# shepherdvovkes/sparse-matrix-multiplication-benchmark

Hardware: AMD Instinct MI355X
Metric: TCSC SpMM: effective G-add-ops/s + achieved HBM GB/s vs roofline, 1/2/4/8 GPU (higher is better)
Workload: dtype f32; 1 GPU; cfg4: M=4096 K=16384 N=16384, 98% ternary sparsity, fp32, tcsc_gemm_prelu; M=4096, K=16384, N=16384, variant=prelu_basic, columns_per_gpu=16384, nnz_per_gpu=5369271, parallelism=column-shard x1 (strong), no collective, rows_per_gpu=4096

## Files before the change

include/tcsc_gpu.h:

```cpp
#ifndef TCSC_AMD_TCSC_GPU_H
#define TCSC_AMD_TCSC_GPU_H

#include <stddef.h>
#include "sparse/tcsc.h"

#ifdef __cplusplus
extern "C" {
#endif

enum tcsc_variant {
    TCSC_VARIANT_BASIC = 0,
    TCSC_VARIANT_OPTIMIZED = 1,
    TCSC_VARIANT_PRELU_BASIC = 2,
    TCSC_VARIANT_PRELU_SEPARATE = 3,
    TCSC_VARIANT_PRELU_ONTHEGO = 4,
    TCSC_VARIANT_SPARSE_GEMM = 5
};

enum tcsc_status {
    TCSC_OK = 0,
    TCSC_E_ARG = 1,
    TCSC_E_HIP = 2,
    TCSC_E_NOMEM = 3,
    TCSC_E_NODEV = 4
};

enum tcsc_order {
    TCSC_ORDER_FAST = 0,
    TCSC_ORDER_REFERENCE = 1
};

typedef struct tcsc_gpu_plan tcsc_gpu_plan;

typedef struct {
    int device;
    int rows;
    int cols;
    int col_begin;
    long long nnz;
    long long n_pos, n_neg;
    int chunk_k;
    int n_chunks;
    size_t device_bytes;
    int order;
    int mfma_min_M;
} tcsc_gpu_plan_info;

int tcsc_gpu_device_count(void);

void tcsc_gpu_set_order(int order);
int tcsc_gpu_get_order(void);

int tcsc_gpu_plan_create(const tcsc_t *W, int col_begin, int col_end,
                         int device, void *stream, tcsc_gpu_plan **out);

int tcsc_gpu_plan_create_device(int rows, int cols,
                                const int *d_col_start_pos,
                                const int *d_col_start_neg,
                                const int *d_row_index_pos,
                                const int *d_row_index_neg,
                                int col_begin, int col_end, int device,
                                void *stream, tcsc_gpu_plan **out);

int tcsc_gpu_plan_get_info(const tcsc_gpu_plan *plan, tcsc_gpu_plan_info *info);

enum tcsc_path {
    TCSC_PATH_GATHER = 0,
    TCSC_PATH_FUSED = 1,
    TCSC_PATH_MFMA = 2,
    TCSC_PATH_SMALL = 3,
    TCSC_PATH_DECODE = 4
};
int tcsc_gpu_launch_info(const tcsc_gpu_plan *plan, int M, int *path, int *slices);

int tcsc_gpu_launch_combine(const tcsc_gpu_plan *plan, int M, int *in_launch);

int tcsc_gpu_launch_geometry(const tcsc_gpu_plan *plan, int M, int *cols_per_wave);
int tcsc_gpu_wide_pays(int M, int ncols, int num_cus);
int tcsc_gpu_plan_wide_stats(const tcsc_gpu_plan *plan, long long stats[4], unsigned short *map,
                             size_t map_entries);

int tcsc_gpu_plan_reserve(tcsc_gpu_plan *plan, int max_M);
void tcsc_gpu_plan_destroy(tcsc_gpu_plan *plan);

#define TCSC_PATH_AUTO (-1)
int tcsc_gpu_plan_workspace(const tcsc_gpu_plan *plan, int M, int path, size_t *need, size_t *reserved);

int tcsc_gpu_sgemm(const tcsc_gpu_plan *plan, const float *dX, const float *dB,
                   float *dY, int M, int ldy, int variant, float a,
                   void *stream);

int tcsc_gpu_prepare_x(const tcsc_gpu_plan *plan, const float *dX, int M, void *stream);
int tcsc_gpu_sgemm_prepared(const tcsc_gpu_plan *plan, const float *dB, float *dY, int M, int ldy,
                            int variant, float a, void *stream);

int tcsc_gpu_sgemm_bf16(const tcsc_gpu_plan *plan, const void *dX_bf16, const float *dB,
                        float *dY, int M, int ldy, int variant, float a, void *stream);
int tcsc_gpu_launch_info_bf16(const tcsc_gpu_plan *plan, int M, int *path, int *slices);

int tcsc_gpu_plan_enable_i8(tcsc_gpu_plan *plan, void *stream);
int tcsc_gpu_plan_has_i8(const tcsc_gpu_plan *plan);
int tcsc_gpu_sgemm_i8(const tcsc_gpu_plan *plan, const void *dXq, const float *dScale,
                      const float *dB, float *dY, int M, int ldy, int variant, float a, void *stream);
int tcsc_gpu_launch_info_i8(const tcsc_gpu_plan *plan, int M, int *path, int *slices);
int tcsc_gpu_quantize_rows_i8(const float *dX, int M, int K, void *dXq, float *dScale, void *stream);
int tcsc_gpu_workspace_bound_i8(int M, int K, int N, size_t *i8_bytes, size_t *f32_bytes);

int tcsc_gpu_plan_enable_w2(tcsc_gpu_plan *plan, void *stream);
int tcsc_gpu_plan_has_w2(const tcsc_gpu_plan *plan);
int tcsc_gpu_w2_image_bytes(int K, int N, size_t *bytes);
int tcsc_gpu_decode_pays(int M, int K, int N, long long nnz);

int tcsc_gpu_plan_create_packed(const tcsc_t *W, int col_begin, int col_end,
                                int device, void *stream, tcsc_gpu_plan **out);
int tcsc_gpu_plan_create_packed_device(int rows, int cols,
                                       const int *d_col_start_pos,
                                       const int *d_col_start_neg,
                                       const int *d_row_index_pos,
                                       const int *d_row_index_neg,
                                       int col_begin, int col_end, int device,
                                       void *stream, tcsc_gpu_plan **out);
int tcsc_gpu_plan_is_packed(const tcsc_gpu_plan *plan);
int tcsc_gpu_plan_copy_w2(const tcsc_gpu_plan *plan, void *d_dst, size_t bytes, void *stream);

int tcsc_gpu_plan_create_packed_image(const void *image, size_t bytes, int rows, int cols,
                                      int col_begin, int device, void *stream, tcsc_gpu_plan **out);
int tcsc_gpu_plan_create_packed_image_device(const void *d_image, size_t bytes, int rows, int cols,
                                             int col_begin, int device, void *stream, tcsc_gpu_plan **out);
int tcsc_gpu_w2_to_tcsc(const void *d_image, size_t bytes, int rows, int cols,
                        int *d_col_start_pos, int *d_col_start_neg,
                        int *d_row_index_pos, int *d_row_index_neg,
                        int *n_pos, int *n_neg, void *stream);
int tcsc_gpu_w2_from_tcsc_host(const tcsc_t *W, int col_begin, int col_end, void *image, size_t bytes);
tcsc_t *tcsc_gpu_w2_to_tcsc_host(const void *image, size_t bytes, int rows, int cols);

enum tcsc_xtype { TCSC_X_F32 = 0, TCSC_X_BF16 = 1 };
int tcsc_gpu_quantize_rows_i8_bf16(const void *dX_bf16, int M, int K, void *dXq, float *dScale, void *stream);
int tcsc_gpu_sgemm_q8(const tcsc_gpu_plan *plan, const void *dX, int xtype, void *dXq, float *dScale,
                      const float *dB, float *dY, int M, int ldy, int variant, float a, void *stream);
int tcsc_gpu_launch_info_q8(const tcsc_gpu_plan *plan, int M, int xtype, int *path, int *slices, int *fused);
int tcsc_gpu_quant_fuse_pays(int M, int K, int N, int xtype);

enum tcsc_ytype { TCSC_Y_F32 = 0, TCSC_Y_BF16 = 1 };
int tcsc_gpu_sgemm_i8_out(const tcsc_gpu_plan *plan, const void *dXq, const float *dScale,
                          const float *dColScale, const float *dB, void *dY, int ytype,
                          int M, int ldy, int variant, float a, void *stream);
int tcsc_gpu_sgemm_q8_out(const tcsc_gpu_plan *plan, const void *dX, int xtype, void *dXq,
                          float *dScale, const float *dColScale, const float *dB, void *dY,
                          int ytype, int M, int ldy, int variant, float a, void *stream);

int tcsc_gpu_from_dense(const float *d_dense, int rows, int cols,
                        int *d_col_start_pos, int *d_col_start_neg,
                        int *d_row_index_pos, int *d_row_index_neg,
                        int *n_pos, int *n_neg, void *stream);

int tcsc_gpu_dense_sgemm(const float *dX, const float *dW, const float *dB,
                         float *dY, int M, int N, int K, int ldy, int variant,
                         float a, void *stream);


int tcsc_gpu_transpose_index(int rows, int cols,
                             const int *d_col_start_pos, const int *d_col_start_neg,
                             const int *d_row_index_pos, const int *d_row_index_neg,
                             int col_begin, int col_end,
                             int *d_t_col_start_pos, int *d_t_col_start_neg,
                             int *d_t_row_index_pos, int *d_t_row_index_neg,
                             void *stream);

int tcsc_gpu_plan_create_transposed(const tcsc_t *W, int col_begin, int col_end,
                                    int device, void *stream, tcsc_gpu_plan **out);

int tcsc_gpu_plan_create_transposed_device(int rows, int cols,
                                           const int *d_col_start_pos,
                                           const int *d_col_start_neg,
                                           const int *d_row_index_pos,
                                           const int *d_row_index_neg,
                                           int col_begin, int col_end, int device,
                                           void *stream, tcsc_gpu_plan **out);

int tcsc_gpu_sgemm_t(const tcsc_gpu_plan *tplan, const float *dG, float *dDX,
                     int M, int ldx, void *stream);

int tcsc_gpu_prelu_backward(const float *dG, int ldg, const float *dY, int ldy, float a,
                            float *dDZ, int lddz, float *dDB, int M, int N, void *stream);

const char *tcsc_gpu_last_error(void);

void tcsc_gpu_cache_clear(void);

int tcsc_gpu_num_shards(void);
void tcsc_gpu_set_num_shards(int shards);


int tcsc_gpu_build_flags(void);

#ifdef __cplusplus
}
#endif

#endif
```

sparse-matrix-multiplication-benchmark_amd/csrc/tcsc_api.cpp:

```cpp
#include <hip/hip_runtime.h>
#include <rocblas/rocblas.h>

#include <algorithm>
#include <cstdarg>
#include <cstdint>
#include <cstdio>
#include <cstdlib>
#include <cstring>
#include <memory>
#include <mutex>
#include <string>
#include <unordered_map>
#include <vector>

#include "../../include/sparse/tcsc.h"
#include "../../include/tcsc_gpu.h"
#include "tcsc_plan.h"

struct tcsc_gpu_plan {
    int device = 0;
    int rows = 0, cols = 0, col_begin = 0;
    long long n_pos = 0, n_neg = 0;
    int n_chunks = 0, n_groups = 0;
    long long n_entries = 0;
// ... 319 lines not shown
              bool allow_mfma, hipStream_t st) {
    if (p->cols == 0 || p->rows >= (1 << 27) - 4) return TCSC_OK;
    if (!tcsc::small_m_fits(1, p->rows) && !mfma_wanted(p, allow_mfma)) return TCSC_OK;
    const int nc = p->cols, ng = tcsc::csc_groups(nc);
    size_t tb = 0;
    DevBuf tcp, tcn, trp, trn, gq, tmp;
    if (tcsc::plan_scan_tmp_bytes(ng + 1, &tb) != hipSuccess || hipMalloc(&p->ccq, (size_t)(ng + 1) * sizeof(int)) != hipSuccess ||
        tcp.alloc((size_t)(nc + 1) * sizeof(int)) != hipSuccess || tcn.alloc((size_t)(nc + 1) * sizeof(int)) != hipSuccess ||
        gq.alloc((size_t)(ng + 1) * sizeof(int)) != hipSuccess || tmp.alloc(tb) != hipSuccess ||
        trp.alloc((size_t)(p->n_pos > 0 ? p->n_pos : 1) * sizeof(int)) != hipSuccess ||
        trn.alloc((size_t)(p->n_neg > 0 ? p->n_neg : 1) * sizeof(int)) != hipSuccess) {
        (void)hipGetLastError();
        free_csc(p);
        return TCSC_OK;
    }
    HIP_TRY(tcsc::csc_prepare(csp, csn, rip, rin, col_begin, nc, p->n_pos, p->n_neg, tcp.as<int>(), tcn.as<int>(),
                              trp.as<int>(), trn.as<int>(), gq.as<int>(), tmp.p, tb, p->ccq, st));
    int quads = 0;
    HIP_TRY(hipMemcpyAsync(&quads, p->ccq + ng, sizeof(int), hipMemcpyDeviceToHost, st));
    HIP_TRY(hipStreamSynchronize(st));
    const size_t ent = tcsc::csc_quad_entries(quads);
    const double nnz = (double)(p->n_pos + p->n_neg);
    if ((double)ent > kCscMaxPad * nnz + (double)tcsc::csc_quad_entries(16LL * ng)) {
        free_csc(p);
        return TCSC_OK;
    }
    if (hipMalloc(&p->crq, ent * sizeof(int)) != hipSuccess) {
        (void)hipGetLastError();
        free_csc(p);
        return TCSC_OK;
    }
    p->csc_bytes = (size_t)(ng + 1) * sizeof(int) + ent * sizeof(int);
    HIP_TRY(tcsc::csc_fill(tcp.as<int>(), tcn.as<int>(), trp.as<int>(), trn.as<int>(), p->ccq, nc, p->rows, p->crq,
                           ent, st));
    HIP_TRY(hipStreamSynchronize(st));
    return TCSC_OK;
}

constexpr int kSmallMaxM = 4;
int small_max_m() {
    const char* e = std::getenv("TCSC_SMALL_M");
    if (!e) return kSmallMaxM;
    return std::max(0, std::min(kSmallMaxM, std::atoi(e)));
}

bool has_small(const tcsc_gpu_plan* p, int M) {
    return p->crq && p->rows > 0 && M >= 1 && M <= small_max_m() && tcsc::small_m_fits(M, p->rows);
}
bool use_small(const tcsc_gpu_plan* p, int M, int dt = kF32) { return has_small(p, M) && !use_mfma(p, M, dt); }

bool decode_pays(int M, int K, int N, long long nnz) {
    if (M < 1 || M > tcsc::kDecodeMaxM) return false;
    return M > kSmallMaxM || !tcsc::small_m_fits(M, K) || 16 * nnz > (long long)K * N;
}
int decode_knob() {
    const char* e = std::getenv("TCSC_DECODE");
    if (!e || !*e) return -1;
    return std::atoi(e) != 0 ? 1 : 0;
}
bool w2gemm_knob() {
    const char* e = std::getenv("TCSC_W2GEMM");
    return e && std::atoi(e) != 0;
}
bool has_decode(const tcsc_gpu_plan* p, int M, int dt) {
    return dt == kI8 && p->w2 && M >= 1 && M <= tcsc::kDecodeMaxM;
}
bool use_decode(const tcsc_gpu_plan* p, int M, int dt) {
    if (!has_decode(p, M, dt)) return false;
    if (p->packed) return true;
    const int knob = decode_knob();
    return knob >= 0 ? knob == 1 : decode_pays(M, p->rows, p->cols, p->n_pos + p->n_neg);
}

int maybe_build_mfma(tcsc_gpu_plan* p, const int* csp, const int* csn, const int* rip, const int* rin, int col_begin,
                     bool allow_mfma, hipStream_t st) {
    const int mode = path_mode();
    if (!mfma_wanted(p, allow_mfma)) return TCSC_OK;
    if (!p->crq) return TCSC_OK;
    const size_t n = (size_t)p->rows * p->cols;
    DevBuf wf, bad;
    if (wf.alloc(n * sizeof(float)) != hipSuccess || bad.alloc(sizeof(int)) != hipSuccess) {
        (void)hipGetLastError();
        return TCSC_OK;
    }
    const int ldw = tcsc::mfma_ldw(p->rows);
    const size_t wtb = (size_t)p->cols * ldw * sizeof(uint16_t);
    if (hipMalloc(&p->wt, wtb) != hipSuccess) {
        (void)hipGetLastError();
        free_mfma(p);
        return TCSC_OK;
    }
    p->mfma_bytes = wtb;
    HIP_TRY(hipMemsetAsync(bad.p, 0, sizeof(int), st));
    HIP_TRY(tcsc::mfma_build_wt(csp, csn, rip, rin, col_begin, p->rows, p->cols, wf.as<float>(), p->wt, ldw,
                                p->n_pos, p->n_neg, bad.as<int>(), st));
    int hbad = 0;
    HIP_TRY(hipMemcpyAsync(&hbad, bad.p, sizeof(int), hipMemcpyDeviceToHost, st));
    HIP_TRY(hipStreamSynchronize(st));
    if (hbad) free_mfma(p);
    p->mfma_min_M = mode == 2 ? 1 : kMfmaMinM;
    return TCSC_OK;
}

int build_plan_ordered(int rows, int col_begin, int ncols, long long n_pos, long long n_neg, const int* csp,
                       const int* csn, const int* rip, const int* rin, int device, hipStream_t st, int order,
                       tcsc_gpu_plan** out, bool allow_mfma = true) {
    int rc = build_plan(rows, col_begin, ncols, n_pos, n_neg, csp, csn, rip, rin, device, st, out);
    if (rc != TCSC_OK) return rc;
    if (order != TCSC_ORDER_REFERENCE) {
        rc = build_csc(*out, csp, csn, rip, rin, col_begin, allow_mfma, st);
        if (rc == TCSC_OK) rc = maybe_build_mfma(*out, csp, csn, rip, rin, col_begin, allow_mfma, st);
        if (rc != TCSC_OK) {
            tcsc_gpu_plan_destroy(*out);
            *out = nullptr;
        }
        return rc;
    }
    tcsc_gpu_plan* p = *out;
    p->order = order;
    DevBuf zeros;
    const size_t zb = (size_t)(col_begin + ncols + 1) * sizeof(int);
    if (zeros.alloc(zb) != hipSuccess || hipMemsetAsync(zeros.p, 0, zb, st) != hipSuccess) {
        tcsc_gpu_plan_destroy(p);
        *out = nullptr;
        set_error("tcsc_gpu_plan_create: cannot allocate the reference-order chains");
        return TCSC_E_HIP;
    }
    rc = build_plan(rows, col_begin, ncols, n_pos, 0, csp, zeros.as<int>(), rip, rip, device, st, &p->chain_pos);
    if (rc == TCSC_OK)
        rc = build_plan(rows, col_begin, ncols, 0, n_neg, zeros.as<int>(), csn, rin, rin, device, st, &p->chain_neg);
    if (rc != TCSC_OK) {
        tcsc_gpu_plan_destroy(p);
        *out = nullptr;
    }
    return rc;
}

int slices_override() {
    const char* s = std::getenv("TCSC_SLICES");
    return s ? std::atoi(s) : 0;
}

int combine_giveup_knob() {
    const char* s = std::getenv("TCSC_COMBINE_GIVEUP");
    return s && std::atoi(s) != 0 ? 1 : 0;
}

size_t path_ws_bytes(const tcsc_gpu_plan* p, int M, int path) {
    if (M <= 0 || p->cols == 0) return 0;
    RoutePins pin;
    pin.path = path;
    return route_call(p, M, p->packed ? kI8 : kF32, kUnbounded, pin).ws_bytes;
}

int launch_path(const tcsc_gpu_plan* p, int M, int dt = kF32) {
    if (use_decode(p, M, dt)) return TCSC_PATH_DECODE;
    return use_mfma(p, M, dt) ? TCSC_PATH_MFMA : use_small(p, M, dt) ? TCSC_PATH_SMALL : TCSC_PATH_GATHER;
}

size_t wanted_workspace(const tcsc_gpu_plan* p, int M, int dt = kF32) {
    if (M <= 0 || p->cols == 0) return 0;
    return route_call(p, M, dt, kUnbounded, RoutePins()).ws_bytes;
}

constexpr long long kNoSplitBase = 40 * 256;
size_t reserve_bytes(const tcsc_gpu_plan* p, int max_M) {
    if (max_M <= 0 || p->cols == 0) return 0;
    if (p->packed) {
        const int top = std::min(max_M, kMaxLaunchRows);
        size_t want = path_ws_bytes(p, top, TCSC_PATH_MFMA);
        for (int M = 64; M < top; M += 64) want = std::max(want, path_ws_bytes(p, M, TCSC_PATH_MFMA));
        return want;
    }
    const long long cb = std::max(1, (p->n_groups + tcsc::kWaves - 1) / tcsc::kWaves);
    const int every = (int)std::min<long long>(max_M, (kNoSplitBase + cb - 1) / cb * tcsc::kTM);
    size_t want = 0;
    auto all_paths = [&](int M) {
        for (int path : {TCSC_PATH_GATHER, TCSC_PATH_MFMA, TCSC_PATH_SMALL})
            want = std::max(want, path_ws_bytes(p, M, path));
    };
    for (int M = 1; M <= every; ++M) all_paths(M);
    if (p->wt)
        for (long long M = ((long long)every / 64 + 1) * 64; M < max_M; M += 64)
            want = std::max(want, path_ws_bytes(p, (int)M, TCSC_PATH_MFMA));
    all_paths(max_M);
    return want;
}

int check_index_host(const int* cs, const int* ri, int c0, int c1, int rows, int n_elem, const char* sign,
                     std::vector<int>& sorted) {
    sorted.clear();
    bool in_order = true;
    for (int j = c0; j < c1; ++j) {
        const int a = cs[j], b = cs[j + 1];
        if (a < 0 || b < a || b > n_elem) {
            set_error("tcsc_gpu_plan_create: col_start_%s[%d..%d] = %d, %d is not a range inside [0, %d]", sign, j,
                      j + 1, a, b, n_elem);
            return TCSC_E_ARG;
        }
        for (int i = a; i < b; ++i) {
            const int k = ri[i];
            if (k < 0 || k >= rows) {
                set_error("tcsc_gpu_plan_create: row_index_%s[%d] = %d outside [0, %d) (column %d)", sign, i, k, rows,
                          j);
                return TCSC_E_ARG;
            }
            if (i > a && k < ri[i - 1]) in_order = false;
        }
    }
    if (in_order) return TCSC_OK;
    const int base = cs[c0];
    sorted.assign(ri + base, ri + cs[c1]);
    for (int j = c0; j < c1; ++j) std::sort(sorted.begin() + (cs[j] - base), sorted.begin() + (cs[j + 1] - base));
    return TCSC_OK;
}

}

namespace tcsc {

uint64_t fmix64(uint64_t h) {
    h ^= h >> 33;
    h *= 0xff51afd7ed558ccdull;
    h ^= h >> 33;
    h *= 0xc4ceb9fe1a85ec53ull;
    return h ^ (h >> 33);
}

constexpr uint32_t kHashA[4] = {0x9e3779b9u, 0x85ebca6bu, 0xc2b2ae35u, 0x27d4eb2fu};
constexpr uint32_t kHashB[4] = {0x165667b1u, 0xd3a2646cu, 0xfd7046c5u, 0xb55a4f09u};

void hash_groups(const uint32_t* u, long long i0, long long i1, uint64_t acc[4]) {
    for (long long i = i0; i < i1; i += 8) {
        const uint32_t pos = (uint32_t)i;
        for (int j = 0; j < 4; ++j)
            acc[j] += (uint64_t)(u[i + 2 * j] + kHashA[j] + pos) * (uint64_t)(u[i + 2 * j + 1] + kHashB[j]);
    }
}

uint64_t hash_finish(const uint32_t* u, long long n, uint64_t h, uint64_t acc[4]) {
    for (long long i = n & ~7LL; i < n; ++i)
        acc[i & 3] += (uint64_t)(u[i] + kHashA[i & 3] + (uint32_t)i) * (uint64_t)(kHashB[i & 3] | 1u);
    for (int j = 0; j < 4; ++j) h = fmix64(h ^ acc[j]) + (uint64_t)j;
    return h;
}

uint64_t hash_ints(const int* p, long long n, uint64_t h) {
    h = fmix64(h ^ (uint64_t)n);
    if (!p || n <= 0) return h;
    const uint32_t* u = reinterpret_cast<const uint32_t*>(p);
    uint64_t acc[4] = {0, 0, 0, 0};
    hash_groups(u, 0, n & ~7LL, acc);
    return hash_finish(u, n, h, acc);
}

uint64_t tcsc_fingerprint(const tcsc_t* W) {
    uint64_t h = fmix64(((uint64_t)(uint32_t)W->rows << 32) | (uint32_t)W->cols);
    h = hash_ints(W->col_start_pos, (long long)W->cols + 1, h);
    h = hash_ints(W->col_start_neg, (long long)W->cols + 1, h);
    h = hash_ints(W->row_index_pos, W->n_elem_pos, h);
    return hash_ints(W->row_index_neg, W->n_elem_neg, h);
}

}

namespace {

constexpr double kWideAlpha = 0.92;
bool wide_pays(int M, int ncols, int num_cus) {
    if (M <= 0 || ncols <= 0 || num_cus <= 0) return false;
    const long long rt = ((long long)M + tcsc::kTM - 1) / tcsc::kTM;
    auto rounds = [&](int w) { return (rt * ((ncols + w - 1) / w) + num_cus - 1) / num_cus; };
    return (double)(rounds(tcsc::kWideWgCols) * tcsc::kWideWgCols) * kWideAlpha <
           (double)(rounds(tcsc::kWgCols) * tcsc::kWgCols);
}

int geo_override() {
    const char* s = std::getenv("TCSC_GEO");
    const int v = s ? std::atoi(s) : 0;
    return v == tcsc::kCW || v == tcsc::kWideCW ? v : 0;
}

bool wide_wanted(const tcsc_gpu_plan* p, int max_M) {
    if (p->order != TCSC_ORDER_FAST || p->tbias || p->rows <= 0 || p->cols <= 0 || max_M <= 0 || !p->ent || !p->sptr)
        return false;
    const int f = geo_override();
    if (f == tcsc::kWideCW) return true;
    if (f == tcsc::kCW) return false;
    const int top = std::min(max_M, kMaxLaunchRows);
    for (long long M = tcsc::kTM; M < top + tcsc::kTM; M += tcsc::kTM)
        if (wide_pays((int)std::min<long long>(M, top), p->cols, p->num_cus)) return true;
    return false;
}

int build_wide(tcsc_gpu_plan* p) {
    if (p->ent_w) return TCSC_OK;
    DeviceGuard dg(p->device);
    hipStream_t st = nullptr;
    const int nch = p->n_chunks, G = p->n_groups, ncols = p->cols, Gw = tcsc::wide_groups_for(ncols);
    const long long nc = (long long)nch * ncols, ng = (long long)nch * Gw;
    if (nch <= 0 || ng + 1 > 0x7fffffffLL) return TCSC_OK;
    const char* bal_s = std::getenv("TCSC_WIDE_BALANCE");
    const int balance = bal_s && std::atoi(bal_s) == 0 ? 0 : 1;
    const size_t nmap = (size_t)tcsc::wide_blocks_for(ncols) * tcsc::kWideWgCols;
    DevBuf cnt, cptr, gcnt, tmp, loads, winv, wstats;
    size_t tb1 = 0, tb2 = 0;
    HIP_TRY(tcsc::plan_scan_tmp_bytes(nc + 1, &tb1));
    HIP_TRY(tcsc::plan_scan_tmp_bytes(ng + 1, &tb2));
    const size_t tb = std::max(tb1, tb2);
    int* sptr_w = nullptr;
    unsigned short* wperm = nullptr;
    if (cnt.alloc((size_t)(nc + 1) * sizeof(int)) != hipSuccess || cptr.alloc((size_t)(nc + 1) * sizeof(int)) != hipSuccess ||
        gcnt.alloc((size_t)(ng + 1) * sizeof(int)) != hipSuccess || tmp.alloc(tb) != hipSuccess ||
        loads.alloc(nmap / tcsc::kWideCW * nch * sizeof(int)) != hipSuccess ||
        winv.alloc((size_t)ncols * sizeof(unsigned short)) != hipSuccess ||
        wstats.alloc(4 * sizeof(unsigned long long)) != hipSuccess ||
        hipMalloc(&sptr_w, (size_t)(ng + 1) * sizeof(int)) != hipSuccess) {
        (void)hipGetLastError();
        return TCSC_OK;
    }
    std::unique_ptr<int, void (*)(int*)> sptr_guard(sptr_w, [](int* q) { (void)hipFree(q); });
    if (hipMalloc(&wperm, nmap * sizeof(unsigned short)) != hipSuccess) {
        (void)hipGetLastError();
        return TCSC_OK;
    }
    std::unique_ptr<unsigned short, void (*)(unsigned short*)> wperm_guard(wperm, [](unsigned short* q) { (void)hipFree(q); });
    HIP_TRY(hipDeviceSynchronize());
    HIP_TRY(tcsc::wide_counts(p->ent, p->sptr, G, nch, ncols, Gw, balance, cnt.as<int>(), cptr.as<int>(), gcnt.as<int>(),
                              sptr_w, loads.as<int>(), wperm, winv.as<unsigned short>(), wstats.as<unsigned long long>(),
                              tmp.p, tb, st));
    int total = 0;
    unsigned long long stats[4] = {0, 0, 0, 0};
    HIP_TRY(hipMemcpyAsync(&total, sptr_w + ng, sizeof(int), hipMemcpyDeviceToHost, st));
    HIP_TRY(hipMemcpyAsync(stats, wstats.p, sizeof stats, hipMemcpyDeviceToHost, st));
    HIP_TRY(hipStreamSynchronize(st));
    int2* ent_w = nullptr;
    if (hipMalloc(&ent_w, (size_t)(total + tcsc::kEntGuard) * sizeof(int2)) != hipSuccess) {
        (void)hipGetLastError();
        return TCSC_OK;
    }
    hipError_t e = tcsc::wide_fill(p->ent, p->sptr, G, nch, ncols, Gw, cptr.as<int>(), winv.as<unsigned short>(), sptr_w,
                                   ent_w, total, st);
    if (e == hipSuccess) e = hipStreamSynchronize(st);
    if (e != hipSuccess) {
        (void)hipFree(ent_w);
        return hip_fail(e, "build_wide");
    }
    p->ent_w = ent_w;
    p->sptr_w = sptr_guard.release();
    p->wperm = wperm_guard.release();
    for (int i = 0; i < 4; ++i) p->wide_stats[i] = (long long)stats[i];
    p->n_entries_w = total;
    p->n_groups_w = Gw;
    p->wide_bytes = (size_t)(ng + 1) * sizeof(int) + (size_t)(total + tcsc::kEntGuard) * sizeof(int2) +
                    nmap * sizeof(unsigned short);
    return TCSC_OK;
}

int launch_geo(const tcsc_gpu_plan* p, int M, int slices, int forced_slices, const char* who) {
    const int f = geo_override();
    if (f == tcsc::kWideCW) {
        if (p->order != TCSC_ORDER_FAST || forced_slices > 1) {
            if (who)
                set_error("%s: TCSC_GEO=22 needs the fast order and an unsplit K (order %s, %d slices forced)", who,
                          p->order == TCSC_ORDER_FAST ? "fast" : "reference", forced_slices);
            return -1;
        }
        if (p->rows <= 0) return tcsc::kCW;
        if (!p->ent_w) {
            if (who)
                set_error("%s: TCSC_GEO=22 but the plan has no wide streams (tcsc_gpu_plan_reserve builds them)", who);
            return -1;
        }
        return tcsc::kWideCW;
    }
    if (f == tcsc::kCW || !p->ent_w || p->order != TCSC_ORDER_FAST) return tcsc::kCW;
    if (slices != 1) return tcsc::kCW;
    return wide_pays(M, p->cols, p->num_cus) ? tcsc::kWideCW : tcsc::kCW;
}

}

Route tcsc::route_call(const tcsc_gpu_plan* p, int M, int dt, size_t ws_avail, const RoutePins& pin, const char* who) {
    const XType& d = kXTypes[dt];
    const int K = p->rows, N = p->cols;
    Route r;
    r.path = pin.path != TCSC_PATH_AUTO ? pin.path : launch_path(p, M, dt);
    r.rows = std::min(M, kMaxLaunchRows);
    if (p->packed) {
        if (pin.path == TCSC_PATH_AUTO) r.path = M <= tcsc::kDecodeMaxM ? TCSC_PATH_DECODE : TCSC_PATH_MFMA;
        if (r.path != TCSC_PATH_MFMA || !has_mfma(p, r.rows, dt)) return r;
        r.slices = d.slices(r.rows, N, K);
        r.ws_bytes = mfma_ws(dt, r.rows, K, N).bytes;
        return r;
    }
    if (r.path == TCSC_PATH_MFMA) {
        if (!has_mfma(p, M, dt)) return r;
        r.slices = d.slices(M, N, K);
        r.ws_bytes = mfma_ws(dt, M, K, N).bytes;
        return r;
    }
    if (r.path == TCSC_PATH_DECODE) return r;
    if (r.path == TCSC_PATH_SMALL) {
        if (has_small(p, M) && dt == kF32) r.ws_bytes = align256((size_t)M * K * sizeof(float));
        return r;
    }
    const size_t xtb = tcsc::xt_bytes(r.rows, K);
    const int force = pin.slices > 0 ? pin.slices : M > kMaxLaunchRows ? 1 : slices_override();
    int chosen = 1;
    if (p->order != TCSC_ORDER_REFERENCE)
        chosen = tcsc::choose_slices(r.rows, N, K, p->n_pos + p->n_neg, p->n_groups, ws_avail > xtb ? ws_avail - xtb : 0,
                                     force);
    r.slices = tcsc::normalized_slices(K, chosen);
    r.ws_bytes = xtb + tcsc::workspace_bytes(r.rows, N, chosen);
    r.geo = launch_geo(p, r.rows, r.slices, force, who);
    if (r.slices > 1) {
        const long long cb = (p->n_groups + tcsc::kWaves - 1) / tcsc::kWaves, rt = (r.rows + tcsc::kTM - 1) / tcsc::kTM;
        const bool words = pin.plan_ws && p->csync != nullptr;
        r.combine = tcsc::combine_mode(r.slices, cb * rt * r.slices, cb * rt, (long long)r.rows * N,
                                       words ? p->num_cus : 0, words, pin.vec && N % 4 == 0);
    }
    return r;
}

namespace {
int sgemm_mfma(const tcsc_gpu_plan* p, const void* dX, int dt, const float* dScale, const float* dB, const YOut& y,
               int M, int ldy, int variant, float a, void* stream, float* ws, size_t ws_bytes, int stage) {
    const XType& d = kXTypes[dt];
    float* dY = static_cast<float*>(y.Y);
    const int K = p->rows, N = p->cols, ldx = d.ldx(K), ldw = d.ldw(K);
    const MfmaWs w = mfma_ws(dt, M, K, N);
    if (!ws || ws_bytes < w.bytes) {
        set_error("%s: workspace of %zu bytes < %zu needed for M=%d", d.sgemm, ws ? ws_bytes : (size_t)0, w.bytes, M);
        return TCSC_E_ARG;
    }
    hipStream_t st = static_cast<hipStream_t>(stream);
    char* base = reinterpret_cast<char*>(ws);
    uint16_t* xp = reinterpret_cast<uint16_t*>(base);
    int* flags = reinterpret_cast<int*>(base + w.flags_off);
    void* slabs = base + w.slabs_off;
    const size_t slab_bytes = ws_bytes - w.slabs_off;
    const bool prelu = is_prelu(variant);
    switch (dt) {
        case kF32:
            if (stage != 2) HIP_TRY(tcsc::mfma_split_x(static_cast<const float*>(dX), M, K, xp, ldx, flags, st));
            if (stage == 1) return TCSC_OK;
            HIP_TRY(tcsc::mfma_gemm3(xp, ldx, p->wt, ldw, K, M, N, dB, dY, ldy, prelu, a, static_cast<float*>(slabs),
                                     slab_bytes, flags, p->ccq, p->crq, st));
            break;
        case kBf16:
            HIP_TRY(tcsc::mfma_pack_x(static_cast<const uint16_t*>(dX), M, K, xp, ldx, flags, st));
            HIP_TRY(tcsc::mfma_gemm1(xp, ldx, p->wt, ldw, K, M, N, dB, dY, ldy, prelu, a, static_cast<float*>(slabs),
                                     slab_bytes, flags, p->ccq, p->crq, st));
            break;
        case kI8:
            HIP_TRY(tcsc::mfma8_pack_x(static_cast<const int8_t*>(dX), M, K, reinterpret_cast<int8_t*>(base), ldx, st));
            if (p->packed || (p->w2 && w2gemm_knob()))
                HIP_TRY(tcsc::mfma8_gemm_w2(reinterpret_cast<const int8_t*>(base), p->w2, ldx, K, M, N, dScale, dB, y,
                                            ldy, prelu, a, static_cast<int*>(slabs), slab_bytes, st));
            else
                HIP_TRY(tcsc::mfma8_gemm(reinterpret_cast<const int8_t*>(base), p->w8, ldx, K, M, N, dScale, dB, y,
                                         ldy, prelu, a, static_cast<int*>(slabs), slab_bytes, st));
            break;
    }
    if (d.flags && d.slices(M, N, K) <= 1) {
        const auto fixup = dt == kF32 ? tcsc::mfma_fixup : tcsc::mfma_fixup1;
        HIP_TRY(fixup(xp, M, K, ldx, p->ccq, p->crq, N, dB, dY, ldy, false, prelu, a, flags, st));
    }
    return TCSC_OK;
}

}

static const char* path_name(int path) {
    switch (path) {
        case TCSC_PATH_GATHER: return "gather";
        case TCSC_PATH_MFMA: return "MFMA";
        case TCSC_PATH_SMALL: return "small-M";
        case TCSC_PATH_DECODE: return "decode";
        default: return "unknown";
    }
}
static bool refuse_out(const char* who, int path, const YOut& y, int M) {
    if (y.plain() || path == TCSC_PATH_DECODE || path == TCSC_PATH_MFMA) return false;
    set_error("%s: %s%s%s needs the decode or the MFMA path, and M=%d routes to the %s path (%d), which writes an fp32 Y "
              "without column scales", who, y.ytype == kYBf16 ? "a bf16 Y" : "", y.ytype == kYBf16 && y.cscale ? " with " : "",
              y.cscale ? "a column scale" : "", M, path_name(path), path);
    return true;
}

int tcsc::sgemm_ws(const tcsc_gpu_plan* p, const void* dX, const float* dB, float* dY, int M, int ldy, int variant,
                   float a, void* stream, float* ws, size_t ws_bytes, int stage, const RoutePins& pin, Route* ran,
                   int dt, const float* dScale, const YOut* out, const char* as) {
    const XType& d = kXTypes[dt];
    const char* who = as ? as : d.sgemm;
    const YOut y = out ? *out : YOut{dY, kYF32, nullptr};
    if (out) dY = y.plain() ? static_cast<float*>(y.Y) : nullptr;
    if (dt != kI8 && !y.plain()) {
        set_error("%s: only the int8 call has a typed Y and column scales", who);
        return TCSC_E_ARG;
    }
    if (dt != kF32 && stage != 0) {
        set_error("%s: no staged form", who);
        return TCSC_E_ARG;
    }
    if (!p || M < 0 || (stage != 1 && (ldy < p->cols || !valid_variant(variant)))) {
        set_error("%s: bad arguments (M=%d ldy=%d variant=%d)", who, M, ldy, variant);
        return TCSC_E_ARG;
    }
    if (p->packed && dt != kI8) {
        set_error("%s: a packed plan holds the 2-bit image only and runs tcsc_gpu_sgemm_i8 alone", who);
        return TCSC_E_ARG;
    }
    if (M == 0 || p->cols == 0) return TCSC_OK;
    if ((stage != 1 && (!y.Y || !dB)) || (stage != 2 && !dX && p->rows > 0)) {
        set_error("%s: NULL device pointer", who);
        return TCSC_E_ARG;
    }
    if (p->packed && M > kMaxLaunchRows) {
        for (int r0 = 0; r0 < M; r0 += kMaxLaunchRows) {
            const YOut piece = y.rows_on((size_t)r0, ldy);
            const int rc = sgemm_ws(p, static_cast<const char*>(dX) + (size_t)r0 * p->rows * d.elem, dB, nullptr,
                                    std::min(kMaxLaunchRows, M - r0), ldy, variant, a, stream, ws, ws_bytes, 0, pin,
                                    nullptr, dt, dScale ? dScale + r0 : nullptr, &piece, as);
            if (rc != TCSC_OK) return rc;
        }
        if (ran) *ran = route_call(p, M, dt, ws ? ws_bytes : 0, pin);
        return TCSC_OK;
    }
    const size_t xtb = tcsc::xt_bytes(std::min(M, kMaxLaunchRows), p->rows);
    tcsc::GemmArgs g;
    g.ncols = p->cols;
    g.B = dB;
    g.Y = dY;
    g.ldy = ldy;
    g.ws = (ws && ws_bytes > xtb) ? reinterpret_cast<float*>(reinterpret_cast<char*>(ws) + xtb) : nullptr;
    g.ws_bytes = g.ws ? ws_bytes - xtb : 0;
    RoutePins pins = pin;
    pins.plan_ws = ws == p->ws;
    pins.vec = tcsc::stores16(g);
    const Route r = route_call(p, M, dt, ws ? ws_bytes : 0, pins, stage != 1 ? who : nullptr);
    if (ran) *ran = r;
    if ((r.path == TCSC_PATH_MFMA && !has_mfma(p, M, dt)) || (r.path == TCSC_PATH_SMALL && !has_small(p, M)) ||
        (r.path == TCSC_PATH_DECODE && !has_decode(p, M, dt)) ||
        (p->packed && r.path != TCSC_PATH_MFMA && r.path != TCSC_PATH_DECODE)) {
        set_error("%s: the plan cannot run M=%d on the pinned path %d", who, M, r.path);
        return TCSC_E_ARG;
    }
    if (refuse_out(who, r.path, y, M)) return TCSC_E_ARG;
    if (r.path == TCSC_PATH_DECODE) {
        HIP_TRY(tcsc::decode_gemm(static_cast<const int8_t*>(dX), p->w2, p->rows, M, p->cols, dScale, dB, y, ldy,
                                  is_prelu(variant), a, p->num_cus, static_cast<hipStream_t>(stream)));
        return TCSC_OK;
    }
    if (r.path == TCSC_PATH_MFMA)
        return sgemm_mfma(p, dX, dt, dScale, dB, y, M, ldy, variant, a, stream, ws, ws_bytes, stage);
    if (r.path == TCSC_PATH_SMALL) {
        hipStream_t st = static_cast<hipStream_t>(stream);
        const size_t xb = (size_t)M * p->rows * sizeof(float);
        if (stage != 0 && (!ws || ws_bytes < xb)) {
            set_error("tcsc_gpu_sgemm: workspace of %zu bytes < %zu needed for M=%d", ws ? ws_bytes : (size_t)0, xb,
                      M);
            return TCSC_E_ARG;
        }
        if (stage == 1) {
            HIP_TRY(hipMemcpyAsync(ws, dX, xb, hipMemcpyDeviceToDevice, st));
            return TCSC_OK;
        }
        HIP_TRY(tcsc::launch_small_m(stage == 2 ? ws : dX, dt, dScale, M, p->rows, p->ccq, p->crq, p->cols, dB, dY, ldy,
                                     false, is_prelu(variant), a, st));
        return TCSC_OK;
    }
    if (M > kMaxLaunchRows) {
        if (stage != 0) {
            set_error("tcsc_gpu_sgemm: M=%d rows staged at once (at most %d; split the rows)", M, kMaxLaunchRows);
            return TCSC_E_ARG;
        }
        RoutePins piece = pin;
        piece.path = TCSC_PATH_GATHER;
        piece.slices = r.slices;
        for (int r0 = 0; r0 < M; r0 += kMaxLaunchRows) {
            const int rows = std::min(kMaxLaunchRows, M - r0);
            const void* xr = static_cast<const char*>(dX) + (size_t)r0 * p->rows * d.elem;
            const int rc = sgemm_ws(p, xr, dB, dY + (size_t)r0 * ldy, rows, ldy, variant, a, stream, ws, ws_bytes, 0,
                                    piece, nullptr, dt, dScale ? dScale + r0 : nullptr, nullptr, as);
            if (rc != TCSC_OK) return rc;
        }
        return TCSC_OK;
    }
    if (p->rows > 0 && (!ws || ws_bytes < xtb)) {
        set_error("%s: workspace of %zu bytes < %zu needed for M=%d", who, ws ? ws_bytes : (size_t)0, xtb, M);
        return TCSC_E_ARG;
    }
    g.X = dX;
    g.xtype = dt;
    g.Xscale = dScale;
    g.XT = p->rows > 0 ? ws : nullptr;
    g.M = M;
    g.K = p->rows;
    g.ent = p->ent;
    g.sptr = p->sptr;
    g.n_entries = p->n_entries;
    if (p->order == TCSC_ORDER_REFERENCE && p->chain_pos && p->chain_neg) {
        g.order = (variant == TCSC_VARIANT_BASIC || variant == TCSC_VARIANT_PRELU_BASIC ||
                   variant == TCSC_VARIANT_SPARSE_GEMM)
                      ? 1
                      : 2;
        g.ent = p->chain_pos->ent;
        g.sptr = p->chain_pos->sptr;
        g.n_entries = p->chain_pos->n_entries;
        g.ent2 = p->chain_neg->ent;
        g.sptr2 = p->chain_neg->sptr;
        g.n_entries2 = p->chain_neg->n_entries;
    }
    g.n_groups = p->n_groups;
    g.a = a;
    g.slices = r.slices;
    g.combine = r.combine;
    g.stage = stage;
    if (stage != 1) {
        if (r.geo < 0) return TCSC_E_ARG;
        if (r.geo == tcsc::kWideCW) {
            g.geo = r.geo;
            g.ent = p->ent_w;
            g.sptr = p->sptr_w;
            g.wperm = p->wperm;
            g.n_entries = p->n_entries_w;
            g.n_groups = p->n_groups_w;
            g.slices = 1;
            g.combine = 0;
        }
    }
    if (pins.plan_ws && p->csync) {
        if (p->csync_dirty) {
            HIP_TRY(hipMemsetAsync(p->csync, 0, tcsc::kCombineBytes, static_cast<hipStream_t>(stream)));
            p->csync_dirty = false;
        }
        g.ccnt = p->csync;
        g.combine_giveup = combine_giveup_knob();
    }
    g.bias_first = (g.order == 1 && variant == TCSC_VARIANT_BASIC);
    g.prelu = is_prelu(variant);
    hipError_t e = tcsc::launch_gemm(g, static_cast<hipStream_t>(stream));
    if (e != hipSuccess) {
        if (g.ccnt) p->csync_dirty = true;
// ... 266 lines not shown
int tcsc_gpu_plan_create_packed(const tcsc_t* W, int col_begin, int col_end, int device, void* stream,
                                tcsc_gpu_plan** out) {
    const char* who = "tcsc_gpu_plan_create_packed";
    if (!W || !out || col_begin < 0 || col_end > W->cols || col_begin > col_end) {
        set_error("%s: bad arguments", who);
        return TCSC_E_ARG;
    }
    *out = nullptr;
    int rc = packed_args_ok(who, W->rows);
    if (rc != TCSC_OK) return rc;
    std::vector<int> unused;
    rc = check_index_host(W->col_start_pos, W->row_index_pos, col_begin, col_end, W->rows, W->n_elem_pos, "pos", unused);
    if (rc == TCSC_OK)
        rc = check_index_host(W->col_start_neg, W->row_index_neg, col_begin, col_end, W->rows, W->n_elem_neg, "neg",
                              unused);
    if (rc != TCSC_OK) return rc;
    DeviceGuard dg(device);
    if (!dg.ok()) {
        set_error("%s: cannot select device %d", who, device);
        return TCSC_E_NODEV;
    }
    hipStream_t st = static_cast<hipStream_t>(stream);
    const int nc = col_end - col_begin;
    const int p0 = W->col_start_pos[col_begin], p1 = W->col_start_pos[col_end];
    const int q0 = W->col_start_neg[col_begin], q1 = W->col_start_neg[col_end];
    std::vector<int> csp(nc + 1), csn(nc + 1);
    for (int j = 0; j <= nc; ++j) {
        csp[j] = W->col_start_pos[col_begin + j] - p0;
        csn[j] = W->col_start_neg[col_begin + j] - q0;
    }
    DevBuf dcsp, dcsn, drip, drin;
    HIP_TRY(dcsp.alloc((nc + 1) * sizeof(int)));
    HIP_TRY(dcsn.alloc((nc + 1) * sizeof(int)));
    HIP_TRY(drip.alloc((size_t)(p1 - p0) * sizeof(int)));
    HIP_TRY(drin.alloc((size_t)(q1 - q0) * sizeof(int)));
    HIP_TRY(hipMemcpyAsync(dcsp.p, csp.data(), (nc + 1) * sizeof(int), hipMemcpyHostToDevice, st));
    HIP_TRY(hipMemcpyAsync(dcsn.p, csn.data(), (nc + 1) * sizeof(int), hipMemcpyHostToDevice, st));
    if (p1 > p0)
        HIP_TRY(hipMemcpyAsync(drip.p, W->row_index_pos + p0, (size_t)(p1 - p0) * sizeof(int), hipMemcpyHostToDevice, st));
    if (q1 > q0)
        HIP_TRY(hipMemcpyAsync(drin.p, W->row_index_neg + q0, (size_t)(q1 - q0) * sizeof(int), hipMemcpyHostToDevice, st));
    rc = build_packed(who, W->rows, 0, nc, p1 - p0, q1 - q0, dcsp.as<int>(), dcsn.as<int>(), drip.as<int>(),
                      drin.as<int>(), device, st, out);
    if (rc == TCSC_OK) (*out)->col_begin = col_begin;
    return rc;
}

int tcsc_gpu_plan_create_packed_device(int rows, int cols, const int* d_csp, const int* d_csn, const int* d_rip,
                                       const int* d_rin, int col_begin, int col_end, int device, void* stream,
                                       tcsc_gpu_plan** out) {
    const char* who = "tcsc_gpu_plan_create_packed_device";
    if (!out || !d_csp || !d_csn || col_begin < 0 || col_end > cols || col_begin > col_end) {
        set_error("%s: bad arguments", who);
        return TCSC_E_ARG;
    }
    *out = nullptr;
    const int rc = packed_args_ok(who, rows);
    if (rc != TCSC_OK) return rc;
    DeviceGuard dg(device);
    if (!dg.ok()) {
        set_error("%s: cannot select device %d", who, device);
        return TCSC_E_NODEV;
    }
    hipStream_t st = static_cast<hipStream_t>(stream);
    int ends[4];
    HIP_TRY(hipMemcpyAsync(&ends[0], d_csp + col_begin, sizeof(int), hipMemcpyDeviceToHost, st));
    HIP_TRY(hipMemcpyAsync(&ends[1], d_csp + col_end, sizeof(int), hipMemcpyDeviceToHost, st));
    HIP_TRY(hipMemcpyAsync(&ends[2], d_csn + col_begin, sizeof(int), hipMemcpyDeviceToHost, st));
    HIP_TRY(hipMemcpyAsync(&ends[3], d_csn + col_end, sizeof(int), hipMemcpyDeviceToHost, st));
    HIP_TRY(hipStreamSynchronize(st));
    const int nc = col_end - col_begin;
    DevBuf flag;
    HIP_TRY(flag.alloc(sizeof(int)));
    HIP_TRY(hipMemsetAsync(flag.p, 0, sizeof(int), st));
    HIP_TRY(tcsc::check_index_device(d_csp, d_rip, col_begin, nc, rows, ends[1], flag.as<int>(), st));
    HIP_TRY(tcsc::check_index_device(d_csn, d_rin, col_begin, nc, rows, ends[3], flag.as<int>(), st));
    int hflag = 0;
    HIP_TRY(hipMemcpyAsync(&hflag, flag.p, sizeof(int), hipMemcpyDeviceToHost, st));
    HIP_TRY(hipStreamSynchronize(st));
    if (hflag & 1) {
        set_error("%s: a col_start range or a row index outside [0, %d)", who, rows);
        return TCSC_E_ARG;
    }
    return build_packed(who, rows, col_begin, nc, ends[1] - ends[0], ends[3] - ends[2], d_csp, d_csn, d_rip, d_rin,
                        device, st, out);
}

int tcsc_gpu_plan_is_packed(const tcsc_gpu_plan* p) {
    if (!p) {
        set_error("tcsc_gpu_plan_is_packed: NULL plan");
        return 0;
    }
    return p->packed ? 1 : 0;
}

int tcsc_gpu_plan_copy_w2(const tcsc_gpu_plan* p, void* d_dst, size_t bytes, void* stream) {
    if (!p) {
        set_error("tcsc_gpu_plan_copy_w2: NULL plan");
        return TCSC_E_ARG;
    }
    if (!p->w2 || bytes != p->w2_bytes || !d_dst) {
        set_error("tcsc_gpu_plan_copy_w2: %s", !p->w2 ? "the plan has no 2-bit image"
                                                      : !d_dst ? "NULL destination" : "bytes is not the image's size");
        return TCSC_E_ARG;
    }
    DeviceGuard dg(p->device);
    HIP_TRY(hipMemcpyAsync(d_dst, p->w2, bytes, hipMemcpyDeviceToDevice, static_cast<hipStream_t>(stream)));
    return TCSC_OK;
}

int tcsc_gpu_plan_create_packed_image(const void* image, size_t bytes, int rows, int cols, int col_begin, int device,
                                      void* stream, tcsc_gpu_plan** out) {
    return packed_from_image("tcsc_gpu_plan_create_packed_image", image, hipMemcpyHostToDevice, bytes, rows, cols,
                             col_begin, device, stream, out);
}

int tcsc_gpu_plan_create_packed_image_device(const void* d_image, size_t bytes, int rows, int cols, int col_begin,
                                             int device, void* stream, tcsc_gpu_plan** out) {
    return packed_from_image("tcsc_gpu_plan_create_packed_image_device", d_image, hipMemcpyDeviceToDevice, bytes, rows,
                             cols, col_begin, device, stream, out);
}

int tcsc_gpu_w2_to_tcsc(const void* d_image, size_t bytes, int rows, int cols, int* d_csp, int* d_csn, int* d_rip,
                        int* d_rin, int* n_pos, int* n_neg, void* stream) {
    const char* who = "tcsc_gpu_w2_to_tcsc";
    if (!d_csp || !d_csn || !n_pos || !n_neg) {
        set_error("%s: NULL col_start or count pointer", who);
        return TCSC_E_ARG;
    }
    int rc = image_args_ok(who, d_image, bytes, rows, cols);
    if (rc != TCSC_OK) return rc;
    if (!tcsc::w2_unpack_fits(cols, rows)) {
        set_error("%s: %d columns x %d k blocks do not fit 32-bit counters", who, cols, tcsc::w2_kblocks(rows));
        return TCSC_E_ARG;
    }
    hipStream_t st = static_cast<hipStream_t>(stream);
    const uint32_t* w2 = static_cast<const uint32_t*>(d_image);
    long long np = 0, nn = 0;
    rc = check_image(who, w2, rows, cols, &np, &nn, st);
    if (rc != TCSC_OK) return rc;
    if (np > 0x7fffffffLL || nn > 0x7fffffffLL) {
        set_error("%s: %lld +1 and %lld -1 entries: tcsc_t offsets are int (each sign below 2^31)", who, np, nn);
        return TCSC_E_ARG;
    }
    const size_t n = (size_t)cols * tcsc::w2_kblocks(rows) + 1;
    size_t tb = 0;
    HIP_TRY(tcsc::plan_scan_tmp_bytes((long long)n, &tb));
    const size_t arr = align256(n * sizeof(int));
    DevBuf scratch;
    HIP_TRY(scratch.alloc(align256(tb) + 4 * arr));
    char* base = scratch.as<char>() + align256(tb);
    int *cntp = reinterpret_cast<int*>(base), *cntn = reinterpret_cast<int*>(base + arr);
    int *offp = reinterpret_cast<int*>(base + 2 * arr), *offn = reinterpret_cast<int*>(base + 3 * arr);
    HIP_TRY(hipMemsetAsync(cntp + (n - 1), 0, sizeof(int), st));
    HIP_TRY(hipMemsetAsync(cntn + (n - 1), 0, sizeof(int), st));
    HIP_TRY(tcsc::w2_unpack_counts(w2, cols, rows, cntp, cntn, st));
    HIP_TRY(tcsc::exclusive_scan_i32(cntp, offp, (int)n, scratch.p, tb, st));
    HIP_TRY(tcsc::exclusive_scan_i32(cntn, offn, (int)n, scratch.p, tb, st));
    HIP_TRY(tcsc::w2_unpack_col_start(offp, offn, cols, rows, d_csp, d_csn, st));
    if (d_rip && d_rin) HIP_TRY(tcsc::w2_unpack_fill(w2, cols, rows, offp, offn, d_rip, d_rin, st));
    HIP_TRY(hipStreamSynchronize(st));
    *n_pos = (int)np;
    *n_neg = (int)nn;
    return TCSC_OK;
}

int tcsc_gpu_plan_get_info(const tcsc_gpu_plan* p, tcsc_gpu_plan_info* info) {
    if (!p || !info) {
        set_error("tcsc_gpu_plan_get_info: NULL");
        return TCSC_E_ARG;
    }
    info->device = p->device;
    info->rows = p->rows;
    info->cols = p->cols;
    info->col_begin = p->col_begin;
    info->nnz = p->n_pos + p->n_neg;
    info->n_pos = p->n_pos;
    info->n_neg = p->n_neg;
    info->chunk_k = tcsc::kTK;
    info->n_chunks = p->n_chunks;
    info->device_bytes = p->bytes + p->ws_bytes + p->mfma_bytes + p->i8_bytes + p->w2_bytes + p->csc_bytes + p->tbias_bytes + p->wide_bytes +
                         (p->chain_pos ? p->chain_pos->bytes : 0) + (p->chain_neg ? p->chain_neg->bytes : 0);
    info->order = p->order;
    info->mfma_min_M = (p->wt || p->packed) ? p->mfma_min_M : 0;
    return TCSC_OK;
}

void tcsc_gpu_set_order(int order) {
    std::lock_guard<std::mutex> lk(g_order_mu);
    g_order = order == TCSC_ORDER_REFERENCE ? TCSC_ORDER_REFERENCE : TCSC_ORDER_FAST;
}

int tcsc_gpu_get_order(void) { return current_order(); }

void tcsc_gpu_plan_destroy(tcsc_gpu_plan* p) {
    if (!p) return;
    DeviceGuard dg(p->device);
    if (p->ent) (void)hipFree(p->ent);
    if (p->sptr) (void)hipFree(p->sptr);
    if (p->ws) (void)hipFree(p->ws);
    if (p->csync) (void)hipFree(p->csync);
    if (p->tbias) (void)hipFree(p->tbias);
    if (p->ent_w) (void)hipFree(p->ent_w);
    if (p->sptr_w) (void)hipFree(p->sptr_w);
    if (p->wperm) (void)hipFree(p->wperm);
    free_mfma(p);
    free_csc(p);
    tcsc_gpu_plan_destroy(p->chain_pos);
    tcsc_gpu_plan_destroy(p->chain_neg);
    delete p;
}

int tcsc_gpu_plan_reserve(tcsc_gpu_plan* p, int max_M) {
    if (!p || max_M < 0) {
        set_error("tcsc_gpu_plan_reserve: bad arguments");
        return TCSC_E_ARG;
    }
    const size_t want = reserve_bytes(p, max_M);
    if (!p->csync && p->rows > 0 && p->order == TCSC_ORDER_FAST && !p->packed) {
        DeviceGuard dg(p->device);
        HIP_TRY(hipMalloc(&p->csync, tcsc::kCombineBytes));
        HIP_TRY(hipMemset(p->csync, 0, tcsc::kCombineBytes));
        HIP_TRY(hipDeviceSynchronize());
        if (!p->num_cus) HIP_TRY(hipDeviceGetAttribute(&p->num_cus, hipDeviceAttributeMultiprocessorCount, p->device));
    }
    if (!p->ent_w && wide_wanted(p, max_M)) {
        const int rc = build_wide(p);
        if (rc != TCSC_OK) return rc;
    }
    if (want <= p->ws_bytes) return TCSC_OK;
    DeviceGuard dg(p->device);
    if (p->ws) {
        HIP_TRY(hipDeviceSynchronize());
        (void)hipFree(p->ws);
    }
    p->ws = nullptr;
    p->ws_bytes = 0;
    p->staged_M = -1;
    HIP_TRY(hipMalloc(&p->ws, want));
    p->ws_bytes = want;
    return TCSC_OK;
}

int tcsc_gpu_plan_workspace(const tcsc_gpu_plan* p, int M, int path, size_t* need, size_t* reserved) {
    if (!p || M < 0 || (path != TCSC_PATH_AUTO && path != TCSC_PATH_GATHER && path != TCSC_PATH_MFMA &&
                        path != TCSC_PATH_SMALL && path != TCSC_PATH_DECODE)) {
        set_error("tcsc_gpu_plan_workspace: bad arguments (M=%d path=%d)", M, path);
        return TCSC_E_ARG;
    }
    if (need) *need = path_ws_bytes(p, M, path);
    if (reserved) *reserved = p->ws_bytes;
    return TCSC_OK;
}

static Route plan_route(const tcsc_gpu_plan* p, int M, int dt, const char* who = nullptr) {
    return route_call(p, M, dt, p->ws_bytes, RoutePins(), who);
}

static int launch_info_impl(const char* who, const tcsc_gpu_plan* p, int M, int* path, int* slices, int dt) {
    if (!p || M < 0 || !path || !slices) {
        set_error("%s: bad arguments", who);
        return TCSC_E_ARG;
    }
    if (dt != kI8 && refuse_packed(p, who)) return TCSC_E_ARG;
    const Route r = plan_route(p, M, dt);
    *path = r.path;
    *slices = r.slices;
    return TCSC_OK;
}

int tcsc_gpu_launch_info(const tcsc_gpu_plan* p, int M, int* path, int* slices) {
    return launch_info_impl("tcsc_gpu_launch_info", p, M, path, slices, kF32);
}

int tcsc_gpu_launch_info_bf16(const tcsc_gpu_plan* p, int M, int* path, int* slices) {
    return launch_info_impl("tcsc_gpu_launch_info_bf16", p, M, path, slices, kBf16);
}

int tcsc_gpu_launch_info_i8(const tcsc_gpu_plan* p, int M, int* path, int* slices) {
    return launch_info_impl("tcsc_gpu_launch_info_i8", p, M, path, slices, kI8);
}

int tcsc_gpu_wide_pays(int M, int ncols, int num_cus) { return wide_pays(M, ncols, num_cus) ? 1 : 0; }

int tcsc_gpu_plan_wide_stats(const tcsc_gpu_plan* p, long long stats[4], unsigned short* map, size_t map_entries) {
    if (!p || (!stats && !map)) {
        set_error("tcsc_gpu_plan_wide_stats: bad arguments");
        return TCSC_E_ARG;
    }
    if (!p->ent_w || !p->wperm) {
        set_error("tcsc_gpu_plan_wide_stats: the plan has no wide streams (tcsc_gpu_plan_reserve builds them)");
        return TCSC_E_ARG;
    }
    if (stats)
        for (int i = 0; i < 4; ++i) stats[i] = p->wide_stats[i];
    if (map) {
        const size_t nmap = (size_t)tcsc::wide_blocks_for(p->cols) * tcsc::kWideWgCols;
        if (map_entries != nmap) {
            set_error("tcsc_gpu_plan_wide_stats: the map has %zu entries, not %zu", nmap, map_entries);
            return TCSC_E_ARG;
        }
        DeviceGuard dg(p->device);
        HIP_TRY(hipMemcpy(map, p->wperm, nmap * sizeof(unsigned short), hipMemcpyDeviceToHost));
    }
    return TCSC_OK;
}

int tcsc_gpu_launch_geometry(const tcsc_gpu_plan* p, int M, int* cols_per_wave) {
    if (!p || M < 0 || !cols_per_wave) {
        set_error("tcsc_gpu_launch_geometry: bad arguments");
        return TCSC_E_ARG;
    }
    if (refuse_packed(p, "tcsc_gpu_launch_geometry")) return TCSC_E_ARG;
    *cols_per_wave = 0;
    const Route r = plan_route(p, M, kF32, "tcsc_gpu_launch_geometry");
    if (r.path != TCSC_PATH_GATHER) return TCSC_OK;
    if (r.geo < 0) return TCSC_E_ARG;
    *cols_per_wave = r.geo;
    return TCSC_OK;
}

int tcsc_gpu_launch_combine(const tcsc_gpu_plan* p, int M, int* in_launch) {
    if (!p || M < 0 || !in_launch) {
        set_error("tcsc_gpu_launch_combine: bad arguments");
        return TCSC_E_ARG;
    }
    if (refuse_packed(p, "tcsc_gpu_launch_combine")) return TCSC_E_ARG;
    *in_launch = plan_route(p, M, kF32).combine;
    return TCSC_OK;
}

static int sgemm_entry(const tcsc_gpu_plan* p, const void* dX, int dt, const float* dScale, const float* dB, float* dY,
                       int M, int ldy, int variant, float a, void* stream, const YOut* out = nullptr,
                       const char* as = nullptr) {
    if (dt != kI8 && refuse_packed(p, kXTypes[dt].sgemm)) return TCSC_E_ARG;
    if (out && !out->plain() && p && M > 0 && p->cols > 0 &&
        refuse_out(as ? as : kXTypes[dt].sgemm, route_call(p, M, dt, p->ws_bytes, RoutePins()).path, *out, M))
        return TCSC_E_ARG;
    if (p && M > 0 && p->cols > 0 && p->ws_bytes < wanted_workspace(p, M, dt)) {
        const int rc = tcsc_gpu_plan_reserve(const_cast<tcsc_gpu_plan*>(p), M);
        if (rc != TCSC_OK) return rc;
    }
    if (p) const_cast<tcsc_gpu_plan*>(p)->staged_M = -1;
    return sgemm_ws(p, dX, dB, dY, M, ldy, variant, a, stream, p ? p->ws : nullptr, p ? p->ws_bytes : 0, 0, RoutePins(),
                    nullptr, dt, dScale, out, as);
}

int tcsc_gpu_sgemm(const tcsc_gpu_plan* p, const float* dX, const float* dB, float* dY, int M, int ldy,
                   int variant, float a, void* stream) {
    return sgemm_entry(p, dX, kF32, nullptr, dB, dY, M, ldy, variant, a, stream);
}

int tcsc_gpu_sgemm_bf16(const tcsc_gpu_plan* p, const void* dX_bf16, const float* dB, float* dY, int M, int ldy,
                        int variant, float a, void* stream) {
    return sgemm_entry(p, dX_bf16, kBf16, nullptr, dB, dY, M, ldy, variant, a, stream);
}

int tcsc_gpu_plan_enable_i8(tcsc_gpu_plan* p, void* stream) {
    if (!p) {
        set_error("tcsc_gpu_plan_enable_i8: NULL plan");
        return TCSC_E_ARG;
    }
    if (p->w8 || !p->wt || p->order == TCSC_ORDER_REFERENCE || p->rows <= 0 || p->cols <= 0) return TCSC_OK;
    DeviceGuard dg(p->device);
    hipStream_t st = static_cast<hipStream_t>(stream);
    const int ld8 = tcsc::mfma8_ldw(p->rows);
    const size_t bytes = (size_t)p->cols * ld8;
    DevBuf bad;
    if (bad.alloc(sizeof(int)) != hipSuccess || hipMalloc(&p->w8, bytes) != hipSuccess) {
        (void)hipGetLastError();
        p->w8 = nullptr;
        set_error("tcsc_gpu_plan_enable_i8: cannot allocate the int8 image (%zu bytes)", bytes);
        return TCSC_E_NOMEM;
    }
    p->i8_bytes = bytes;
    int hbad = 0, rc = TCSC_OK;
    hipError_t e = hipMemsetAsync(bad.p, 0, sizeof(int), st);
    if (e == hipSuccess)
        e = tcsc::mfma8_build_w8(p->wt, p->cols, p->rows, tcsc::mfma_ldw(p->rows), p->w8, ld8, bad.as<int>(), st);
    if (e == hipSuccess) e = hipMemcpyAsync(&hbad, bad.p, sizeof(int), hipMemcpyDeviceToHost, st);
    if (e == hipSuccess) e = hipStreamSynchronize(st);
    if (e != hipSuccess) rc = hip_fail(e, "tcsc_gpu_plan_enable_i8");
    if (rc != TCSC_OK || hbad) free_i8(p);
    return rc;
}

int tcsc_gpu_plan_has_i8(const tcsc_gpu_plan* p) {
    if (!p) {
        set_error("tcsc_gpu_plan_has_i8: NULL plan");
        return 0;
    }
    return p->w8 ? 1 : 0;
}

int tcsc_gpu_plan_enable_w2(tcsc_gpu_plan* p, void* stream) {
    if (!p) {
        set_error("tcsc_gpu_plan_enable_w2: NULL plan");
        return TCSC_E_ARG;
    }
    if (p->w2 || !p->w8 || p->rows <= 0 || p->rows >= tcsc::kDecodeMaxK || p->cols <= 0) return TCSC_OK;
    DeviceGuard dg(p->device);
    hipStream_t st = static_cast<hipStream_t>(stream);
    const size_t bytes = tcsc::w2_image_bytes(p->rows, p->cols);
    DevBuf bad;
    if (bad.alloc(sizeof(int)) != hipSuccess || hipMalloc(&p->w2, bytes) != hipSuccess) {
        (void)hipGetLastError();
        p->w2 = nullptr;
        set_error("tcsc_gpu_plan_enable_w2: cannot allocate the 2-bit image (%zu bytes)", bytes);
        return TCSC_E_NOMEM;
    }
    p->w2_bytes = bytes;
    int hbad = 0, rc = TCSC_OK;
    hipError_t e = hipMemsetAsync(bad.p, 0, sizeof(int), st);
    if (e == hipSuccess)
        e = tcsc::decode_build_w2(p->w8, p->cols, p->rows, tcsc::mfma8_ldw(p->rows), p->w2, bad.as<int>(), st);
    if (e == hipSuccess) e = hipMemcpyAsync(&hbad, bad.p, sizeof(int), hipMemcpyDeviceToHost, st);
    if (e == hipSuccess) e = hipStreamSynchronize(st);
    if (e == hipSuccess && !p->num_cus)
        e = hipDeviceGetAttribute(&p->num_cus, hipDeviceAttributeMultiprocessorCount, p->device);
    if (e != hipSuccess) rc = hip_fail(e, "tcsc_gpu_plan_enable_w2");
    if (rc != TCSC_OK || hbad) free_w2(p);
    return rc;
}

int tcsc_gpu_plan_has_w2(const tcsc_gpu_plan* p) {
    if (!p) {
        set_error("tcsc_gpu_plan_has_w2: NULL plan");
        return 0;
    }
    return p->w2 ? 1 : 0;
}

int tcsc_gpu_w2_image_bytes(int K, int N, size_t* bytes) {
    if (K < 0 || N < 0 || !bytes) {
        set_error("tcsc_gpu_w2_image_bytes: bad arguments (K=%d N=%d)", K, N);
        return TCSC_E_ARG;
    }
    *bytes = tcsc::w2_image_bytes(K, N);
    return TCSC_OK;
}

int tcsc_gpu_decode_pays(int M, int K, int N, long long nnz) { return decode_pays(M, K, N, nnz) ? 1 : 0; }

int tcsc_gpu_sgemm_i8(const tcsc_gpu_plan* p, const void* dXq, const float* dScale, const float* dB, float* dY, int M,
                      int ldy, int variant, float a, void* stream) {
    const YOut y{dY, kYF32, nullptr};
    return sgemm_entry(p, dXq, kI8, dScale, dB, nullptr, M, ldy, variant, a, stream, &y);
}

static int out_args(const char* who, const tcsc_gpu_plan* p, const float* dB, const void* dY, int ytype) {
    if (ytype != TCSC_Y_F32 && ytype != TCSC_Y_BF16) {
        set_error("%s: ytype=%d is neither TCSC_Y_F32 (0) nor TCSC_Y_BF16 (1)", who, ytype);
        return TCSC_E_ARG;
    }
    if (!p) {
        set_error("%s: NULL plan", who);
        return TCSC_E_ARG;
    }
    if (!dY || !dB) {
        set_error("%s: NULL %s", who, !dY ? "dY" : "dB");
        return TCSC_E_ARG;
    }
    return TCSC_OK;
}

int tcsc_gpu_sgemm_i8_out(const tcsc_gpu_plan* p, const void* dXq, const float* dScale, const float* dColScale,
                          const float* dB, void* dY, int ytype, int M, int ldy, int variant, float a, void* stream) {
    const char* who = "tcsc_gpu_sgemm_i8_out";
    const int rc = out_args(who, p, dB, dY, ytype);
    if (rc != TCSC_OK) return rc;
    const YOut y{dY, ytype == TCSC_Y_BF16 ? kYBf16 : kYF32, dColScale};
    return sgemm_entry(p, dXq, kI8, dScale, dB, nullptr, M, ldy, variant, a, stream, &y, who);
}

int tcsc_gpu_quantize_rows_i8(const float* dX, int M, int K, void* dXq, float* dScale, void* stream) {
    if (M < 0 || K < 0) {
        set_error("tcsc_gpu_quantize_rows_i8: bad arguments (M=%d K=%d)", M, K);
        return TCSC_E_ARG;
    }
    if (M == 0) return TCSC_OK;
    if (!dScale || (K > 0 && (!dX || !dXq))) {
        set_error("tcsc_gpu_quantize_rows_i8: NULL device pointer");
        return TCSC_E_ARG;
    }
    HIP_TRY(tcsc::quantize_rows_i8(dX, M, K, static_cast<int8_t*>(dXq), dScale, static_cast<hipStream_t>(stream)));
    return TCSC_OK;
}

int tcsc_gpu_quantize_rows_i8_bf16(const void* dX_bf16, int M, int K, void* dXq, float* dScale, void* stream) {
    if (M < 0 || K < 0) {
        set_error("tcsc_gpu_quantize_rows_i8_bf16: bad arguments (M=%d K=%d)", M, K);
        return TCSC_E_ARG;
    }
    if (M == 0) return TCSC_OK;
    if (!dScale || (K > 0 && (!dX_bf16 || !dXq))) {
        set_error("tcsc_gpu_quantize_rows_i8_bf16: NULL device pointer");
        return TCSC_E_ARG;
    }
    HIP_TRY(tcsc::quantize_rows_i8_bf16(static_cast<const uint16_t*>(dX_bf16), M, K, static_cast<int8_t*>(dXq), dScale,
                                        static_cast<hipStream_t>(stream)));
    return TCSC_OK;
}

static constexpr int kQFuseMaxM = 4;
static constexpr long long kQFuseValues = 1LL << 23;
static bool quant_fuse_pays(int M, int K, int N, int xtype) {
    if (M < 1 || M > kQFuseMaxM || K < 1 || N < 1 || (xtype != TCSC_X_F32 && xtype != TCSC_X_BF16)) return false;
    const int T = tcsc::decode_tiles_per_wg(M, N, 0);
    const long long wgs = (tcsc::w2_col_tiles(N) + T - 1) / T;
    return wgs * M * K <= kQFuseValues;
}
static int qfuse_knob() {
    const char* e = std::getenv("TCSC_QFUSE");
    if (!e || !*e) return -1;
    return std::atoi(e) != 0 ? 1 : 0;
}
static Route route_q8(const tcsc_gpu_plan* p, int M, int xtype, bool* fused) {
    const Route r = route_call(p, M, kI8, p->ws_bytes, RoutePins());
    *fused = false;
    if (r.path == TCSC_PATH_DECODE && has_decode(p, M, kI8)) {
        const int knob = qfuse_knob();
        *fused = knob >= 0 ? knob == 1 : quant_fuse_pays(M, p->rows, p->cols, xtype);
    }
    return r;
}

int tcsc_gpu_quant_fuse_pays(int M, int K, int N, int xtype) { return quant_fuse_pays(M, K, N, xtype) ? 1 : 0; }

int tcsc_gpu_launch_info_q8(const tcsc_gpu_plan* p, int M, int xtype, int* path, int* slices, int* fused) {
    if (!p || M < 0 || !path || !slices || !fused || (xtype != TCSC_X_F32 && xtype != TCSC_X_BF16)) {
        set_error("tcsc_gpu_launch_info_q8: bad arguments (M=%d xtype=%d)", M, xtype);
        return TCSC_E_ARG;
    }
    bool f = false;
    const Route r = route_q8(p, M, xtype, &f);
    *path = r.path;
    *slices = r.slices;
    *fused = f ? 1 : 0;
    return TCSC_OK;
}

static int sgemm_q8_impl(const char* who, const char* inner, const tcsc_gpu_plan* p, const void* dX, int xtype, void* dXq,
                         float* dScale, const float* dB, const YOut& y, int M, int ldy, int variant, float a,
                         void* stream) {
    void* dY = y.Y;
    if (!p || M < 0 || ldy < p->cols || !valid_variant(variant) || (xtype != TCSC_X_F32 && xtype != TCSC_X_BF16)) {
        set_error("%s: bad arguments (M=%d ldy=%d variant=%d xtype=%d)", who, M, ldy, variant, xtype);
        return TCSC_E_ARG;
    }
    if (M == 0) return TCSC_OK;
    if (!dScale || !dB || !dY || (!dX && p->rows > 0)) {
        set_error("%s: NULL device pointer", who);
        return TCSC_E_ARG;
    }
    bool fused = false;
    if (p->cols > 0 && refuse_out(who, route_q8(p, M, xtype, &fused).path, y, M)) return TCSC_E_ARG;
    if (!fused) {
        if (!dXq && p->rows > 0) {
            set_error("%s: NULL dXq on a route that is not fused (M=%d)", who, M);
            return TCSC_E_ARG;
        }
        const int rc = xtype == TCSC_X_F32
                           ? tcsc_gpu_quantize_rows_i8(static_cast<const float*>(dX), M, p->rows, dXq, dScale, stream)
                           : tcsc_gpu_quantize_rows_i8_bf16(dX, M, p->rows, dXq, dScale, stream);
        if (rc != TCSC_OK) return rc;
        return sgemm_entry(p, dXq, kI8, dScale, dB, nullptr, M, ldy, variant, a, stream, &y, inner);
    }
    const_cast<tcsc_gpu_plan*>(p)->staged_M = -1;
    HIP_TRY(tcsc::decode_gemm_q(dX, xtype == TCSC_X_BF16, p->w2, p->rows, M, p->cols, dScale, dB, y, ldy,
                                is_prelu(variant), a, p->num_cus, static_cast<hipStream_t>(stream)));
    return TCSC_OK;
}

int tcsc_gpu_sgemm_q8(const tcsc_gpu_plan* p, const void* dX, int xtype, void* dXq, float* dScale, const float* dB,
                      float* dY, int M, int ldy, int variant, float a, void* stream) {
    return sgemm_q8_impl("tcsc_gpu_sgemm_q8", nullptr, p, dX, xtype, dXq, dScale, dB, YOut{dY, kYF32, nullptr}, M, ldy,
                         variant, a, stream);
}

int tcsc_gpu_sgemm_q8_out(const tcsc_gpu_plan* p, const void* dX, int xtype, void* dXq, float* dScale,
                          const float* dColScale, const float* dB, void* dY, int ytype, int M, int ldy, int variant,
                          float a, void* stream) {
    const char* who = "tcsc_gpu_sgemm_q8_out";
    const int rc = out_args(who, p, dB, dY, ytype);
    if (rc != TCSC_OK) return rc;
    return sgemm_q8_impl(who, who, p, dX, xtype, dXq, dScale, dB, YOut{dY, ytype == TCSC_Y_BF16 ? kYBf16 : kYF32, dColScale},
                         M, ldy, variant, a, stream);
}

int tcsc_gpu_workspace_bound_i8(int M, int K, int N, size_t* i8_bytes, size_t* f32_bytes) {
    if (M < 0 || K < 1 || N < 0) {
        set_error("tcsc_gpu_workspace_bound_i8: bad arguments (M=%d K=%d N=%d)", M, K, N);
        return TCSC_E_ARG;
    }
    if (i8_bytes) *i8_bytes = mfma_ws(kI8, M, K, N).bytes;
    if (f32_bytes) *f32_bytes = mfma_ws(kF32, M, K, N).bytes;
    return TCSC_OK;
}

static int ensure_workspace(const tcsc_gpu_plan* p, int M) {
    if (p && M > 0 && p->cols > 0 && p->ws_bytes < wanted_workspace(p, M))
        return tcsc_gpu_plan_reserve(const_cast<tcsc_gpu_plan*>(p), M);
    return TCSC_OK;
}

int tcsc_gpu_prepare_x(const tcsc_gpu_plan* p, const float* dX, int M, void* stream) {
// ... 363 lines not shown
```

sparse-matrix-multiplication-benchmark_amd/csrc/tcsc_internal.h:

```cpp
#pragma once
#include <hip/hip_runtime.h>
#include <stddef.h>
#include <stdint.h>

namespace tcsc {

constexpr int kTM = 256;
#ifndef TCSC_TK
#define TCSC_TK 48
#endif
#ifndef TCSC_NBUF
#define TCSC_NBUF 3
#endif
constexpr int kTK = TCSC_TK;
constexpr int kNBuf = TCSC_NBUF;
constexpr int kRowBytes = kTM * 4;
constexpr int kBufRows = kTK + 1;
#ifndef TCSC_WAVES
#define TCSC_WAVES 16
#endif
#ifndef TCSC_CW
#define TCSC_CW 16
#endif
#ifndef TCSC_BATCH
#define TCSC_BATCH 4
#endif
constexpr int kWaves = TCSC_WAVES;
constexpr int kCW = TCSC_CW;
constexpr int kBatch = TCSC_BATCH;
constexpr int kWavesPerSimd = kWaves / 4;
static_assert(kWaves % 4 == 0 && kWaves <= 16, "whole waves per SIMD");

#ifndef TCSC_WIDTHS
#define TCSC_WIDTHS 16, 16, 16, 16
#endif
struct ColLayout {
    int w[kWavesPerSimd];
};
constexpr ColLayout kRankCols{{TCSC_WIDTHS}};
__host__ __device__ constexpr int wave_cols(int w) { return kRankCols.w[w >> 2]; }
__host__ __device__ constexpr int wave_col0(int w) {
    int s = 0;
    for (int r = 0; r < (w >> 2); ++r) s += 4 * kRankCols.w[r];
    return s + (w & 3) * kRankCols.w[w >> 2];
}
constexpr int wg_cols() {
    int s = 0;
    for (int r = 0; r < kWavesPerSimd; ++r) s += 4 * kRankCols.w[r];
    return s;
}
constexpr int kWgCols = wg_cols();
constexpr bool widths_ok() {
    for (int r = 0; r < kWavesPerSimd; ++r)
        if (kRankCols.w[r] <= 0 || kRankCols.w[r] > kCW || kRankCols.w[r] % 4) return false;
    return true;
}
static_assert(widths_ok(), "TCSC_WIDTHS: one width per rank, multiples of 4, at most TCSC_CW");
__host__ __device__ constexpr int group_col0(int g) { return (g / kWaves) * kWgCols + wave_col0(g % kWaves); }
__host__ __device__ constexpr int group_cols(int g) { return wave_cols(g % kWaves); }
__host__ __device__ constexpr int groups_for(int ncols) {
    int g = (ncols / kWgCols) * kWaves;
    while (group_col0(g) < ncols) ++g;
    return g;
}
#ifndef TCSC_PF_S
#define TCSC_PF_S 1
#endif
constexpr bool kPfS = TCSC_PF_S != 0;
constexpr int kPfWindow = 1792;
constexpr int kEntGuard = kPfS ? kPfWindow / 8 + 8 : 64;
static_assert(kEntGuard <= 256, "k_fill_headers writes the guard with one block");
constexpr int kHdr = 2;
constexpr int kRingBytes = kNBuf * kBufRows * kRowBytes;
constexpr int kPfScratch = kPfS ? kWaves * 256 : 0;
constexpr int kEpiMinBytes = kWaves * 64 * (kCW * 4 + 16) + 64 * kRowBytes + 16;
constexpr int kLdsBytes = (kRingBytes + kPfScratch) > kEpiMinBytes ? (kRingBytes + kPfScratch) : kEpiMinBytes;
#ifndef TCSC_DMA_WAVES
#define TCSC_DMA_WAVES (TCSC_WAVES / 4)
#endif
#ifndef TCSC_DMA_EARLY
#define TCSC_DMA_EARLY 1
#endif
constexpr int kDmaWaves = TCSC_DMA_WAVES;
constexpr bool kDmaEarly = TCSC_DMA_EARLY != 0;
constexpr int kDmaPerWave = kTK / kDmaWaves;
static_assert(kDmaWaves <= kWaves && kTK % kDmaWaves == 0, "each DMA wave moves the same number of rows");
static_assert(kLdsBytes <= 160 * 1024, "LDS");
static_assert(kNBuf >= 2 && kNBuf <= 5, "ring of 2 (DMA(c+1) before gather(c)) or n >= 3 (DMA(c+n-1) after it)");

static_assert(4 * kCW <= 255, "slot index must fit the 8-bit gpr_idx field");
static_assert(64 * 16 <= 1024, "lane byte offset (16*lane) must fit the 10 low address bits");

constexpr int kWideCW = 22;
constexpr int kWideBatch = 3;
constexpr int kWideWgCols = kWaves * kWideCW;
__host__ __device__ constexpr int wide_group_col0(int g) { return (g / kWaves) * kWideWgCols + (g % kWaves) * kWideCW; }
__host__ __device__ constexpr int wide_groups_for(int ncols) {
    return (ncols / kWideWgCols) * kWaves + (ncols % kWideWgCols + kWideCW - 1) / kWideCW;
}
__host__ __device__ constexpr int wide_blocks_for(int ncols) { return (ncols + kWideWgCols - 1) / kWideWgCols; }

struct PlanDev {
    int rows = 0;
    int ncols = 0;
    int col_begin = 0;
    long long n_pos = 0, n_neg = 0;
    const int* csp = nullptr;
    const int* csn = nullptr;
    const int* rip = nullptr;
    const int* rin = nullptr;
};

struct PlanOut {
    int n_chunks = 0;
    int n_groups = 0;
    long long n_entries = 0;
    int2* ent = nullptr;
    int* sptr = nullptr;
    int* lbp = nullptr;
    int* lbn = nullptr;
    int* cnt = nullptr;
    int* cptr = nullptr;
    int* gcnt = nullptr;
    void* scan_tmp = nullptr;
    size_t scan_tmp_bytes = 0;
};

constexpr int kCombineTiles = 4096;
constexpr int kCombineWords = 32;
constexpr size_t kCombineBytes = (size_t)kCombineTiles * kCombineWords * 4;

enum { kF32 = 0, kBf16 = 1, kI8 = 2 };

enum { kYF32 = 0, kYBf16 = 1 };
struct YOut {
    void* Y = nullptr;
    int ytype = kYF32;
    const float* cscale = nullptr;
    size_t elem() const { return ytype == kYBf16 ? 2 : 4; }
    bool plain() const { return ytype == kYF32 && !cscale; }
    YOut rows_on(size_t r0, int ldy) const { return YOut{static_cast<char*>(Y) + r0 * ldy * elem(), ytype, cscale}; }
};

struct GemmArgs {
    const void* X = nullptr;
    int xtype = kF32;
    const float* Xscale = nullptr;
    float* XT = nullptr;
    int M = 0, K = 0;
    const int2* ent = nullptr;
    const int* sptr = nullptr;
    long long n_entries = 0;
    int order = 0;
    const int2* ent2 = nullptr;
    const int* sptr2 = nullptr;
    long long n_entries2 = 0;
    int n_groups = 0;
    int geo = kCW;
    const unsigned short* wperm = nullptr;
    int ncols = 0;
    const float* B = nullptr;
    float* Y = nullptr;
    int ldy = 0;
    float a = 0.f;
    bool bias_first = false;
    bool prelu = false;
    float* ws = nullptr;
    size_t ws_bytes = 0;
    int slices = 1;
    int combine = 0;
    int stage = 0;
    unsigned* ccnt = nullptr;
    int combine_giveup = 0;
};
inline bool stores16(const GemmArgs& g) {
    return g.ncols % 4 == 0 && g.ldy % 4 == 0 &&
           ((reinterpret_cast<uintptr_t>(g.Y) | reinterpret_cast<uintptr_t>(g.ws) | reinterpret_cast<uintptr_t>(g.B)) & 15) == 0;
}
constexpr int kMaxLaunchRows = 1 << 22;

hipError_t plan_scan_tmp_bytes(long long n, size_t* bytes);
hipError_t plan_counts(const PlanDev& in, PlanOut& out, hipStream_t st);
hipError_t plan_fill(const PlanDev& in, PlanOut& out, hipStream_t st);
int choose_slices(int M, int ncols, int K, long long nnz, int n_groups, size_t ws_bytes, int force);
int combine_mode(int slices, long long wgs, long long tiles, long long slab_floats, int num_cus, bool have_words,
                 bool vec);
int normalized_slices(int K, int slices);
void pf_stream_params(long long n_entries, int n_groups, int n_chunks, int* dist, int* lines);
size_t workspace_bytes(int M, int ncols, int slices);
size_t xt_bytes(int M, int K);
hipError_t launch_gemm(const GemmArgs& g, hipStream_t st);
hipError_t wide_counts(const int2* ent, const int* sptr, int G, int nch, int ncols, int Gw, int balance, int* cnt,
                       int* cptr, int* gcnt, int* sptr_w, int* loads, unsigned short* wperm, unsigned short* winv,
                       unsigned long long* wstats, void* tmp, size_t tmp_bytes, hipStream_t st);
hipError_t wide_fill(const int2* ent, const int* sptr, int G, int nch, int ncols, int Gw, const int* cptr,
                     const unsigned short* winv, const int* sptr_w, int2* ent_w, long long n_entries, hipStream_t st);
hipError_t launch_stream_wide(const GemmArgs& g, hipStream_t st);
int dense_tile_rows(int rows);
hipError_t dense_to_tcsc_counts(const float* D, int rows, int cols, int* cp, int* cn, int* totp, int* totn,
                                hipStream_t st);
hipError_t dense_to_tcsc_fill(const float* D, int rows, int cols, const int* csp, const int* csn, const int* op,
                              const int* on, int* rip, int* rin, hipStream_t st);
hipError_t launch_bias_act(float* Y, int M, int N, int ldy, const float* B, bool prelu, float a, hipStream_t st);
hipError_t exclusive_scan_i32(const int* in, int* out, int n, void* tmp, size_t tmp_bytes, hipStream_t st);
hipError_t check_index_device(const int* cs, const int* ri, int col_begin, int ncols, int rows, int n_total,
                              int* d_flag, hipStream_t st);
hipError_t rebase_offsets(const int* cs, int col_begin, int ncols, int* out, hipStream_t st);
hipError_t sort_columns_tmp_bytes(int n, int ncols, size_t* bytes);
hipError_t sort_columns(const int* in, int* out, int n, int ncols, const int* off, void* tmp, size_t tmp_bytes,
                        hipStream_t st);
int ldxt_for(int M);
hipError_t launch_transpose(const void* X, int M, int K, float* XT, int ldxt, hipStream_t st, int xtype = kF32,
                            const float* scale = nullptr);

constexpr int kCscGroup = 64;
constexpr int kCscGuardQuads = 48;
__host__ __device__ inline int csc_half(int K) { return (K + 4) & ~3; }
__host__ __device__ inline int csc_neg_base(int K) { return 4 * csc_half(K); }
__host__ __device__ inline int csc_groups(int ncols) { return (ncols + kCscGroup - 1) / kCscGroup; }
inline size_t csc_quad_entries(long long quads) { return (size_t)(quads + kCscGuardQuads) * kCscGroup * 4; }
hipError_t csc_prepare(const int* csp, const int* csn, const int* rip, const int* rin, int col_begin, int ncols,
                       long long n_pos, long long n_neg, int* cp, int* cn, int* crp, int* crn, int* gq, void* scan_tmp,
                       size_t scan_tmp_bytes, int* cq, hipStream_t st);
hipError_t csc_fill(const int* cp, const int* cn, const int* crp, const int* crn, const int* cq, int ncols, int rows,
                    int* crq, size_t crq_entries, hipStream_t st);
__host__ __device__ inline size_t csc_entry(const int* cq, int j, int i) {
    const int g = j / kCscGroup, l = j % kCscGroup;
    return ((size_t)(cq[g] + i / 4) * kCscGroup + l) * 4 + (i & 3);
}

constexpr int kMfmaBlk = 64;
__host__ __device__ inline int mfma_nblk(int K) { return (K + kMfmaBlk - 1) / kMfmaBlk; }
__host__ __device__ inline int mfma_ldk(int K) { return 3 * kMfmaBlk * mfma_nblk(K); }
__host__ __device__ inline int mfma_ldw(int K) { return kMfmaBlk * mfma_nblk(K); }
__host__ __device__ inline int x3_index(int k, int part) {
    return (k / kMfmaBlk) * (3 * kMfmaBlk) + part * kMfmaBlk + k % kMfmaBlk;
}
hipError_t mfma_build_wt(const int* csp, const int* csn, const int* rip, const int* rin, int col_begin, int rows,
                         int ncols, float* wf, uint16_t* wt, int ldw, long long n_pos, long long n_neg, int* bad,
                         hipStream_t st);
constexpr size_t small_m_lds_bytes_max() { return 160 * 1024; }
inline size_t small_m_lds_bytes(int M, int K) { return (size_t)M * 2 * (size_t)csc_half(K) * 4; }
inline bool small_m_fits(int M, int K) { return M >= 1 && M <= 4 && small_m_lds_bytes(M, K) <= small_m_lds_bytes_max(); }
hipError_t launch_small_m(const void* X, int xtype, const float* scale, int M, int K, const int* cq, const int* crq,
                          int ncols, const float* B, float* Y, int ldy, bool bias_first, bool prelu, float a,
                          hipStream_t st);
hipError_t mfma_split_x(const float* X, int M, int K, uint16_t* x3, int ldk, int* flags, hipStream_t st);
bool mfma_big_tiles(int M, int N);
bool mfma_narrow_tiles(int M, int N);
long long mfma_tiles(int M, int N);
int mfma_slices(int M, int N, int K);
size_t mfma_slab_bytes(int M, int N, int K);
hipError_t mfma_gemm3(const uint16_t* x3, int ldk, const uint16_t* wt, int ldw, int K, int M, int N, const float* B,
                      float* Y, int ldy, bool prelu, float a, float* slabs, size_t slab_bytes, const int* flags,
                      const int* cq, const int* crq, hipStream_t st);

hipError_t mfma_pack_x(const uint16_t* X, int M, int K, uint16_t* x1, int ldw, int* flags, hipStream_t st);
hipError_t mfma_gemm1(const uint16_t* x1, int ldk, const uint16_t* wt, int ldw, int K, int M, int N, const float* B,
                      float* Y, int ldy, bool prelu, float a, float* slabs, size_t slab_bytes, const int* flags,
                      const int* cq, const int* crq, hipStream_t st);
hipError_t mfma_fixup1(const uint16_t* x1, int M, int K, int ldk, const int* cq, const int* crq, int ncols,
                       const float* B, float* Y, int ldy, bool bias_first, bool prelu, float a, const int* flags,
                       hipStream_t st);

constexpr int kMfma8Blk = 128;
__host__ __device__ inline int mfma8_nblk(int K) { return (K + kMfma8Blk - 1) / kMfma8Blk; }
__host__ __device__ inline int mfma8_ldw(int K) { return kMfma8Blk * mfma8_nblk(K); }
int mfma8_slices(int M, int N, int K);
size_t mfma8_slab_bytes(int M, int N, int K);
hipError_t mfma8_pack_x(const int8_t* X, int M, int K, int8_t* x8, int ld8, hipStream_t st);
hipError_t mfma8_build_w8(const uint16_t* wt, int ncols, int K, int ldw, int8_t* w8, int ld8, int* bad,
                          hipStream_t st);
hipError_t mfma8_gemm(const int8_t* x8, const int8_t* w8, int ld8, int K, int M, int N, const float* scale,
                      const float* B, const YOut& y, int ldy, bool prelu, float a, int* slabs, size_t slab_bytes,
                      hipStream_t st);
hipError_t quantize_rows_i8(const float* X, int M, int K, int8_t* Xq, float* scale, hipStream_t st);
hipError_t quantize_rows_i8_bf16(const uint16_t* X, int M, int K, int8_t* Xq, float* scale, hipStream_t st);

constexpr int kW2Cols = 16;
constexpr int kW2Blk = 256;
constexpr int kW2TileBytes = 1024;
constexpr int kDecodeMaxM = 16;
constexpr int kDecodeMaxK = 1 << 22;
__host__ __device__ inline int w2_col_tiles(int N) { return (N + kW2Cols - 1) / kW2Cols; }
__host__ __device__ inline int w2_kblocks(int K) { return (K + kW2Blk - 1) / kW2Blk; }
inline size_t w2_image_bytes(int K, int N) { return (size_t)w2_col_tiles(N) * w2_kblocks(K) * kW2TileBytes; }
hipError_t decode_build_w2(const int8_t* w8, int ncols, int K, int ld8, uint32_t* w2, int* bad, hipStream_t st);
hipError_t w2_from_tcsc(const int* csp, const int* csn, const int* rip, const int* rin, int col_begin, int ncols, int K,
                        uint32_t* w2, int* bad, hipStream_t st);
constexpr int kW2BadCode = 1, kW2BadPad = 2;
hipError_t w2_check(const uint32_t* w2, int ncols, int K, unsigned long long* counts, int* bad, hipStream_t st);
bool w2_unpack_fits(int ncols, int K);
hipError_t w2_unpack_counts(const uint32_t* w2, int ncols, int K, int* cntp, int* cntn, hipStream_t st);
hipError_t w2_unpack_col_start(const int* offp, const int* offn, int ncols, int K, int* csp, int* csn, hipStream_t st);
hipError_t w2_unpack_fill(const uint32_t* w2, int ncols, int K, const int* offp, const int* offn, int* rip, int* rin,
                          hipStream_t st);
hipError_t mfma8_gemm_w2(const int8_t* x8, const uint32_t* w2, int ld8, int K, int M, int N, const float* scale,
                         const float* B, const YOut& y, int ldy, bool prelu, float a, int* slabs, size_t slab_bytes,
                         hipStream_t st);
int decode_tiles_per_wg(int M, int N, int num_cus);
hipError_t decode_gemm(const int8_t* X, const uint32_t* w2, int K, int M, int N, const float* scale, const float* B,
                       const YOut& y, int ldy, bool prelu, float a, int num_cus, hipStream_t st);
hipError_t decode_gemm_q(const void* X, bool bf16, const uint32_t* w2, int K, int M, int N, float* scale_out,
                         const float* B, const YOut& y, int ldy, bool prelu, float a, int num_cus, hipStream_t st);

hipError_t mfma_fixup(const uint16_t* x3, int M, int K, int ldk, const int* cq, const int* crq, int ncols,
                      const float* B, float* Y, int ldy, bool bias_first, bool prelu, float a, const int* flags,
                      hipStream_t st);

hipError_t transpose_sign(const int* cs, const int* ri, int col_begin, int ncols, int rows, int e0, int n, int* cnt,
                          int* cursor, int* unsorted, void* tmp, size_t tmp_bytes, int* t_cs, int* t_ri,
                          hipStream_t st);
hipError_t launch_prelu_bwd(const float* G, int ldg, const float* Y, int ldy, float a, float* DZ, int lddz, float* DB,
                            int M, int N, hipStream_t st);

void set_error_msg(const char* msg);
const char* error_msg();
void report_status(int rc);

struct BcsrArgs {
    const float* XT = nullptr;
    int ldxt = 0, M = 0, N = 0, ldy = 0;
    const int* colptr = nullptr;
    const int2* ent = nullptr;
    const float* vals = nullptr;
    int r = 1, c = 1, nbc = 0;
    const float* B = nullptr;
    float* Y = nullptr;
    float a = 0.f;
    bool fma = false;
    bool prelu = false;
};
hipError_t launch_bcsr(const BcsrArgs& g, hipStream_t st);

}
```

sparse-matrix-multiplication-benchmark_amd/csrc/tcsc_wide.hip:

```cpp
#include <hip/hip_runtime.h>
#include <hipcub/hipcub.hpp>
#include <stdint.h>

#include "tcsc_internal.h"

namespace tcsc {

#include "gather_asm_w22.inc"

static_assert(TCSCW_GEN_CW == kWideCW && TCSCW_GEN_BATCH == kWideBatch, "generated loop geometry");
static_assert(TCSCW_GEN_CAP + kHdr <= kEntGuard, "stream prefetch stays inside the entry guard");
static_assert(TCSCW_GEN_HDR == 2 * kHdr, "generated loop and plan agree on the chunk header");
static_assert(TCSCW_GEN_BUDGET == (512 / kWavesPerSimd) / 8 * 8, "generated loop VGPR budget");
static_assert(TCSCW_GEN_TAIL == 1, "the wide streams are unpadded");
static_assert(TCSCW_GEN_TOUCH == 0 && TCSCW_GEN_PF == 0, "no scalar-cache touches in the wide loop");
static_assert(4 * kWideCW <= 255, "slot index must fit the 8-bit gpr_idx field");
static_assert(kWaves == 16 && kTK % 16 == 0 && kNBuf >= 3, "the wide kernel's DMA split and ring");

namespace {

typedef float f32x32_t __attribute__((ext_vector_type(32)));
typedef float f32x16_t __attribute__((ext_vector_type(16)));
typedef float f32x8_t __attribute__((ext_vector_type(8)));
constexpr int kAccWidths[] = {TCSCW_ACC_WIDTHS};
static_assert(sizeof(kAccWidths) == 4 * sizeof(int) && kAccWidths[0] == 32 && kAccWidths[1] == 32 &&
                  kAccWidths[2] == 16 && kAccWidths[3] == 8,
              "AccW mirrors the generated operand tuples");
struct AccW {
    f32x32_t v0, v1;
    f32x16_t v2;
    f32x8_t v3;
};
__device__ __forceinline__ float acc_get(const AccW& a, int i) {
    return i < 32 ? a.v0[i] : i < 64 ? a.v1[i - 32] : i < 80 ? a.v2[i - 64] : a.v3[i - 80];
}
__device__ __forceinline__ void acc_set(AccW& a, int i, float v) {
    if (i < 32) a.v0[i] = v;
    else if (i < 64) a.v1[i - 32] = v;
    else if (i < 80) a.v2[i - 64] = v;
    else a.v3[i - 80] = v;
}
__device__ __forceinline__ void acc_zero(AccW& a) {
#pragma unroll
    for (int i = 0; i < 4 * kWideCW; ++i) acc_set(a, i, 0.f);
}

typedef int i32x16 __attribute__((ext_vector_type(16)));
typedef __attribute__((address_space(4))) const i32x16 const_i32x16;
typedef int sbuf_tail_t __attribute__((ext_vector_type(TCSCW_SBUF_TAIL ? TCSCW_SBUF_TAIL : 4)));
typedef __attribute__((address_space(4))) const sbuf_tail_t const_sbuf_tail;

__device__ __forceinline__ void gather_stream_w(i32x16 (&sb)[TCSCW_SBUF_VECS], sbuf_tail_t& sbt,
                                                unsigned long long& ptr, unsigned lane16, unsigned mask, AccW& acc) {
    (void)sbt;
    unsigned m0sv;
    asm volatile(TCSCW_GATHER_ASM
                 : TCSCW_ACC_OPERANDS(acc), TCSCW_SBUF_OPERANDS(sb, sbt), TCSCW_PTR_OPERAND(ptr), [m0sv] "=&s"(m0sv)
                 : [lane] "v"(lane16), [mask] "v"(mask)
                 : TCSCW_GATHER_CLOBBERS);
}

__device__ __forceinline__ void load_stream_w(i32x16 (&sb)[TCSCW_SBUF_VECS], sbuf_tail_t& sbt, const char* p) {
    const_i32x16* q = reinterpret_cast<const_i32x16*>(reinterpret_cast<uintptr_t>(p));
#pragma unroll
    for (int i = 0; i < TCSCW_SBUF_VECS; ++i) sb[i] = q[i];
#if TCSCW_SBUF_TAIL
    sbt = *reinterpret_cast<const_sbuf_tail*>(reinterpret_cast<uintptr_t>(p + 64 * TCSCW_SBUF_VECS));
#endif
}

struct DmaW {
    const char* next;
    unsigned lds_wave;
    unsigned chunk_bytes;
    unsigned row_bytes;
};
static_assert(kDmaPerWave % 2 == 0, "whole pairs of DMA rows");

__device__ __forceinline__ void dma_next_chunk_w(DmaW& d, int buf, unsigned lane16) {
    const unsigned m0base = d.lds_wave + (unsigned)(buf * (kBufRows * kRowBytes));
    const char* row = d.next;
#pragma unroll
    for (int i0 = 0; i0 < kDmaPerWave; i0 += 2) {
        const char* s0 = row;
        const char* s1 = row + (d.row_bytes - 1 * kRowBytes);
        unsigned sv;
        asm volatile("s_mov_b32 %[sv], m0\n\ts_mov_b32 m0, %1\n\ts_nop 0\n\tglobal_load_lds_dwordx4 %2, %3\n\t"
                     "global_load_lds_dwordx4 %2, %4 offset:1024\n\ts_mov_b32 m0, %[sv]"
                     : [sv] "=&s"(sv)
                     : "s"(m0base + i0 * kRowBytes), "v"(lane16), "s"(s0), "s"(s1)
                     : "memory");
        row += 2u * d.row_bytes;
    }
    d.next += d.chunk_bytes;
}
static_assert(kRowBytes == 1024, "the DMA's instruction offsets are whole 1-KiB rows");

__device__ __forceinline__ void pf_touch_w(unsigned m0, unsigned voff, const char* base) {
    unsigned sv;
    asm volatile("s_mov_b32 %[sv], m0\n\ts_mov_b32 m0, %1\n\ts_nop 0\n\tglobal_load_lds_dword %2, %3\n\t"
                 "s_mov_b32 m0, %[sv]"
                 : [sv] "=&s"(sv)
                 : "s"(m0), "v"(voff), "s"(base)
                 : "memory");
}

__device__ __forceinline__ void xcd_tile_w(int bx, int by, int ncb, int nrt, int& cb, int& rt) {
    const int T = ncb * nrt;
    const int L = bx + ncb * by;
    const int q = T >> 3, r = T & 7, x = L & 7;
    const int Lg = (x < r ? x * (q + 1) : r * (q + 1) + (x - r) * q) + (L >> 3);
    cb = Lg % ncb;
    rt = Lg / ncb;
}

constexpr int kEpiRowsW = 64;
constexpr int kStrideW = kWideWgCols * 4 + 16;
constexpr int kLdsBytesW = kRingBytes + kPfScratch;
static_assert(kEpiRowsW * kStrideW <= kRingBytes, "the epilogue staging fits below the ring's end");
static_assert(kLdsBytesW <= 160 * 1024, "LDS");
static_assert(kWideCW <= 64 && kWideWgCols <= 65535, "one lane per slot reads its 16-bit column position");
static_assert(kWideWgCols % 4 == 0 && kWideWgCols / 4 > 64 && kWideWgCols / 4 <= 128,
              "a tile row is 64 quads plus a second, partial set");

}

struct WideArgs {
    const float* XT;
    const int2* ent;
    const int* sptr;
    const float* Bias;
    float* Y;
    const unsigned short* wperm;
    long long n_entries;
    int ldxt, M, G, ncols, nch, ldy;
    float a;
    int pf_dist, pf_lines;
};

template <bool BIAS_FIRST, bool PRELU>
__global__ void __launch_bounds__(kWaves * 64, kWavesPerSimd)
k_stream_w(const float* __restrict__ XT, const int2* __restrict__ ent, const int* __restrict__ sptr,
           const float* __restrict__ Bias0, float* __restrict__ Y0, const unsigned short* __restrict__ wperm0,
           long long n_entries, int ldxt, int M0, int G, int ncols0, int nch, int ldy0, float a0, int pf_dist,
           int pf_lines) {
    __shared__ __attribute__((aligned(16))) char lds[kLdsBytesW];
    const int lane = threadIdx.x & 63;
    const unsigned lane16 = 16u * lane;
    const int wave = __builtin_amdgcn_readfirstlane(threadIdx.x >> 6);
    int tcb, trt;
    xcd_tile_w(blockIdx.x, blockIdx.y, gridDim.x, gridDim.y, tcb, trt);
    const int g = tcb * kWaves + wave;
    const int m0 = trt * kTM;
    const bool active = g < G;

    AccW acc;
    acc_zero(acc);
    if (BIAS_FIRST && active) {
        const int cb = lane < kWideCW ? tcb * kWideWgCols + wperm0[tcb * kWideWgCols + wave * kWideCW + lane] : ncols0;
        const float bv = cb < ncols0 ? Bias0[cb] : 0.f;
#pragma unroll
        for (int j = 0; j < kWideCW; ++j) {
            const float b = __shfl(bv, j);
#pragma unroll
            for (int r = 0; r < 4; ++r) acc_set(acc, 4 * j + r, b);
        }
    }

    if (threadIdx.x < 64 * kNBuf) {
        const int b = threadIdx.x >> 6;
        reinterpret_cast<float4*>(lds + (b * kBufRows + kTK) * kRowBytes)[lane] = make_float4(-0.f, -0.f, -0.f, -0.f);
    }

    if (nch > 0) {
        DmaW dma;
        dma.row_bytes = (unsigned)ldxt * 4u;
        dma.chunk_bytes = (unsigned)kTK * (unsigned)ldxt * 4u;
        dma.next = reinterpret_cast<const char*>(XT + m0) + (size_t)(wave * kDmaPerWave) * dma.row_bytes;
        dma.lds_wave = (unsigned)reinterpret_cast<uintptr_t>(lds) + (unsigned)(wave * kDmaPerWave * kRowBytes);
        const bool dma_wave = wave < kDmaWaves;
        const unsigned pf_m0 = (unsigned)reinterpret_cast<uintptr_t>(lds) + kRingBytes + 256u * wave;
        const unsigned pf_s_off = (unsigned)pf_dist + 128u * (unsigned)(lane * pf_lines >> 6);
        auto pf_issue = [&](unsigned long long p) {
            if (kPfS) pf_touch_w(pf_m0, pf_s_off, reinterpret_cast<const char*>(p));
        };
        if (dma_wave) dma_next_chunk_w(dma, 0, lane16);
        unsigned long long cur =
            reinterpret_cast<unsigned long long>(ent + (active ? (long long)sptr[(long long)g * nch] : n_entries));
        i32x16 sb[TCSCW_SBUF_VECS];
        sbuf_tail_t sbt;
        load_stream_w(sb, sbt, reinterpret_cast<const char*>(cur));
        pf_issue(cur);
#pragma unroll
        for (int i = 1; i + 1 < kNBuf; ++i) {
            if (dma_wave) dma_next_chunk_w(dma, i % kNBuf, lane16);
            pf_issue(cur);
        }
        asm volatile("s_waitcnt lgkmcnt(0)" ::: "memory");
        const unsigned mask = 0x3ffu;
        int dbuf = kNBuf - 1;
        for (int c = 0; c < nch; ++c) {
            asm volatile("s_waitcnt vmcnt(%0)" ::"n"((kNBuf - 2) * kDmaPerWave + (kPfS ? 2 : 0)) : "memory");
            __builtin_amdgcn_s_barrier();
            if (dma_wave) dma_next_chunk_w(dma, dbuf, lane16);
            gather_stream_w(sb, sbt, cur, lane16, mask, acc);
            load_stream_w(sb, sbt, reinterpret_cast<const char*>(cur));
            pf_issue(cur);
            dbuf = dbuf == kNBuf - 1 ? 0 : dbuf + 1;
        }
        asm volatile("s_waitcnt vmcnt(0) lgkmcnt(0)" ::: "memory");
    }

    __syncthreads();
    typedef __attribute__((address_space(4))) const WideArgs const_args;
    const_args* E = reinterpret_cast<const_args*>(reinterpret_cast<uintptr_t>(__builtin_amdgcn_kernarg_segment_ptr()));
    asm volatile("" : "+s"(E)::"memory");
    const float* __restrict__ Bias = E->Bias;
    float* __restrict__ Y = E->Y;
    const int M = E->M, ncols = E->ncols, ldy = E->ldy;
    const float a = E->a;
    int bx = blockIdx.x, by = blockIdx.y, gx = gridDim.x, gy = gridDim.y;
    asm volatile("" : "+s"(bx), "+s"(by), "+s"(gx), "+s"(gy));
    const int wave_e = __builtin_amdgcn_readfirstlane(threadIdx.x >> 6);
    int tcb_e, trt_e;
    xcd_tile_w(bx, by, gx, gy, tcb_e, trt_e);
    const bool active_e = tcb_e * kWaves + wave_e < E->G;
    const int m0_e = trt_e * kTM;
    static_assert(kEpiRowsW == 64 && kTM == 4 * kEpiRowsW, "a pass parks one of each lane's four rows");
    constexpr int kQuads = kWideWgCols / 4;
    const unsigned short* __restrict__ wperm = E->wperm;
    const int posv = lane < kWideCW ? wperm[tcb_e * kWideWgCols + wave_e * kWideCW + lane] : 0;
    int pos[kWideCW];
#pragma unroll
    for (int j = 0; j < kWideCW; ++j) pos[j] = __builtin_amdgcn_readlane(posv, j);
    const bool vec_ok = (ldy & 3) == 0 && ((reinterpret_cast<uintptr_t>(Y) & 15) == 0);
    float4 bq[2];
#pragma unroll
    for (int s = 0; s < 2; ++s) {
        const int col = tcb_e * kWideWgCols + 4 * (lane + 64 * s);
        const bool in = lane + 64 * s < kQuads;
        bq[s].x = (!BIAS_FIRST && in && col + 0 < ncols) ? Bias[col + 0] : 0.f;
        bq[s].y = (!BIAS_FIRST && in && col + 1 < ncols) ? Bias[col + 1] : 0.f;
        bq[s].z = (!BIAS_FIRST && in && col + 2 < ncols) ? Bias[col + 2] : 0.f;
        bq[s].w = (!BIAS_FIRST && in && col + 3 < ncols) ? Bias[col + 3] : 0.f;
    }
#pragma unroll
    for (int h = 0; h < kTM / kEpiRowsW; ++h) {
        if (active_e) {
#pragma unroll
            for (int j = 0; j < kWideCW; ++j)
                *reinterpret_cast<float*>(lds + lane * kStrideW + pos[j] * 4) = acc_get(acc, 4 * j + h);
        }
        __syncthreads();
#pragma unroll
        for (int i = 0; i < kEpiRowsW / kWaves; ++i) {
            const int R = wave_e + kWaves * i;
            const int row = m0_e + 4 * R + h;
#pragma unroll
            for (int s = 0; s < 2; ++s) {
                const int q = lane + 64 * s;
                const int col = tcb_e * kWideWgCols + 4 * q;
                if (q < kQuads && row < M && col < ncols) {
                    float4 v = *reinterpret_cast<const float4*>(lds + R * kStrideW + q * 16);
                    if (!BIAS_FIRST) {
                        v.x += bq[s].x;
                        v.y += bq[s].y;
                        v.z += bq[s].z;
                        v.w += bq[s].w;
                    }
                    if (PRELU) {
                        v.x = (v.x < 0.0f) ? a * v.x : v.x;
                        v.y = (v.y < 0.0f) ? a * v.y : v.y;
                        v.z = (v.z < 0.0f) ? a * v.z : v.z;
                        v.w = (v.w < 0.0f) ? a * v.w : v.w;
                    }
                    float* dst = Y + (size_t)row * ldy + col;
                    if (vec_ok && col + 3 < ncols) {
                        typedef float nt4 __attribute__((ext_vector_type(4)));
                        nt4 w = {v.x, v.y, v.z, v.w};
                        __builtin_nontemporal_store(w, reinterpret_cast<nt4*>(dst));
                    } else {
                        dst[0] = v.x;
                        if (col + 1 < ncols) dst[1] = v.y;
                        if (col + 2 < ncols) dst[2] = v.z;
                        if (col + 3 < ncols) dst[3] = v.w;
                    }
                }
            }
        }
        if (h + 1 < kTM / kEpiRowsW) __syncthreads();
    }
}


namespace {

__device__ __forceinline__ int stream_range(const int* __restrict__ sptr, long long i, int* first) {
    const int s0 = sptr[i], s1 = sptr[i + 1];
    *first = s0 + kHdr;
    return s1 - s0 - kHdr;
}
__device__ __forceinline__ bool is_pad(int word) { return ((word >> 10) % kBufRows) == kTK; }

__global__ void k_wide_col_counts(const int2* __restrict__ ent, const int* __restrict__ sptr, int G, int nch, int ncols,
                                  int* __restrict__ cnt) {
    const long long total = (long long)G * nch;
    for (long long i = blockIdx.x * (long long)blockDim.x + threadIdx.x; i < total;
         i += (long long)gridDim.x * blockDim.x) {
        const int g = (int)(i / nch), c = (int)(i % nch);
        int first;
        const int n = stream_range(sptr, i, &first);
        const int n0 = group_col0(g);
        int run = 0, slot = -1;
        for (int e = 0; e < n; ++e) {
            const int w = ent[first + e].y;
            if (is_pad(w)) continue;
            const int s = (w & 0x3ff) >> 2;
            if (s != slot) {
                if (run) cnt[(long long)c * ncols + n0 + slot] = run;
                slot = s;
                run = 0;
            }
            ++run;
        }
        if (run) cnt[(long long)c * ncols + n0 + slot] = run;
    }
}

template <typename T>
__device__ __forceinline__ T wave_sum(T v) {
#pragma unroll
    for (int o = 32; o > 0; o >>= 1) v += __shfl_xor(v, o);
    return v;
}

__global__ void __launch_bounds__(kWaves * 64)
k_wide_balance(const int* __restrict__ cnt, int ncols, int nch, int balance, int* L0, unsigned short* __restrict__ wperm,
               unsigned short* __restrict__ winv) {
    __shared__ int tot[kWideWgCols];
    __shared__ unsigned short order[kWideWgCols], cand[kWideWgCols];
    __shared__ int nslot[kWaves];
    __shared__ unsigned long long score[kWaves], red[2][kWaves];
    __shared__ int best_s, keep_s;
    const int tid = threadIdx.x, nt = blockDim.x, lane = tid & 63, wave = tid >> 6;
    const int c0 = blockIdx.x * kWideWgCols;
    unsigned short* perm = wperm + (size_t)blockIdx.x * kWideWgCols;
    if (!balance || c0 + kWideWgCols > ncols) {
        for (int i = tid; i < kWideWgCols; i += nt) {
            perm[i] = (unsigned short)i;
            if (c0 + i < ncols) winv[c0 + i] = (unsigned short)i;
        }
        return;
    }
    const int* blk = cnt + c0;
    int* L = L0 + (size_t)blockIdx.x * kWaves * nch;
    for (int col = tid; col < kWideWgCols; col += nt) {
        int s = 0;
        for (int c = 0; c < nch; ++c) s += blk[(size_t)c * ncols + col];
        tot[col] = s;
    }
    for (int i = tid; i < kWaves * nch; i += nt) L[i] = 0;
    if (tid < kWaves) nslot[tid] = 0;
    __syncthreads();
    for (int i = tid; i < kWideWgCols; i += nt) {
        int r = 0;
        for (int j = 0; j < kWideWgCols; ++j) r += (tot[j] > tot[i] || (tot[j] == tot[i] && j < i)) ? 1 : 0;
        order[r] = (unsigned short)i;
    }
    __syncthreads();
    for (int step = 0; step < kWideWgCols; ++step) {
        const int col = order[step];
        const int* cc = blk + col;
        unsigned long long s = 0;
        if (nslot[wave] < kWideCW)
            for (int c = lane; c < nch; c += 64)
                s += (unsigned long long)L[(size_t)wave * nch + c] * (unsigned long long)cc[(size_t)c * ncols];
        s = wave_sum(s);
        if (lane == 0) score[wave] = s;
        __syncthreads();
        if (tid == 0) {
            int best = -1;
            for (int w = 0; w < kWaves; ++w)
                if (nslot[w] < kWideCW && (best < 0 || score[w] < score[best])) best = w;
            cand[best * kWideCW + nslot[best]++] = (unsigned short)col;
            best_s = best;
        }
        __syncthreads();
        const int bw = best_s;
        for (int c = tid; c < nch; c += nt) L[(size_t)bw * nch + c] += cc[(size_t)c * ncols];
        __syncthreads();
    }
    unsigned long long sg = 0, si = 0;
    for (int c = tid; c < nch; c += nt) {
        int mg = 0, mi = 0;
        for (int w = 0; w < kWaves; ++w) {
            mg = max(mg, L[(size_t)w * nch + c]);
            int s = 0;
            for (int j = 0; j < kWideCW; ++j) s += blk[(size_t)c * ncols + w * kWideCW + j];
            mi = max(mi, s);
        }
        sg += (unsigned long long)mg;
        si += (unsigned long long)mi;
    }
    sg = wave_sum(sg);
    si = wave_sum(si);
    if (lane == 0) {
        red[0][wave] = sg;
        red[1][wave] = si;
    }
    __syncthreads();
    if (tid == 0) {
        unsigned long long g = 0, i = 0;
        for (int w = 0; w < kWaves; ++w) {
            g += red[0][w];
            i += red[1][w];
        }
        keep_s = g < i ? 1 : 0;
    }
    __syncthreads();
    const bool keep = keep_s != 0;
    for (int i = tid; i < kWideWgCols; i += nt) {
        const int v = keep ? cand[i] : i;
        perm[i] = (unsigned short)v;
        winv[c0 + v] = (unsigned short)i;
    }
}

__global__ void k_wide_permute_counts(const int* __restrict__ cnt, const unsigned short* __restrict__ wperm, int ncols,
                                      int nch, int* __restrict__ cntp) {
    const long long total = (long long)nch * ncols;
    for (long long i = blockIdx.x * (long long)blockDim.x + threadIdx.x; i <= total;
         i += (long long)gridDim.x * blockDim.x) {
        if (i == total) {
            cntp[i] = 0;
            continue;
        }
        const int q = (int)(i % ncols), b0 = q / kWideWgCols * kWideWgCols;
        cntp[i] = cnt[i - q + b0 + wperm[q]];
    }
}

__global__ void k_wide_stats(const int* __restrict__ cnt, const unsigned short* __restrict__ wperm, int ncols, int nch,
                             unsigned long long* __restrict__ st) {
    const int c0 = blockIdx.x * kWideWgCols;
    const unsigned short* perm = wperm + (size_t)blockIdx.x * kWideWgCols;
    unsigned long long v[4] = {0, 0, 0, 0};
    for (int c = threadIdx.x; c < nch; c += blockDim.x) {
        const int* row = cnt + (size_t)c * ncols + c0;
        int mi = 0, mp = 0;
        for (int w = 0; w < kWaves; ++w) {
            int si = 0, sp = 0;
            for (int j = 0; j < kWideCW; ++j) {
                const int ci = w * kWideCW + j, cp = perm[ci];
                si += c0 + ci < ncols ? row[ci] : 0;
                sp += c0 + cp < ncols ? row[cp] : 0;
            }
            mi = max(mi, si);
            mp = max(mp, sp);
            v[2] += si > TCSCW_GEN_CAP ? 1 : 0;
            v[3] += sp > TCSCW_GEN_CAP ? 1 : 0;
        }
        v[0] += (unsigned long long)mi;
        v[1] += (unsigned long long)mp;
    }
#pragma unroll
    for (int k = 0; k < 4; ++k) {
        const unsigned long long s = wave_sum(v[k]);
        if ((threadIdx.x & 63) == 0 && s) atomicAdd(st + k, s);
    }
}

__global__ void k_wide_group_counts(const int* __restrict__ cptr, int ncols, int nch, int Gw, int* __restrict__ gcnt) {
    const long long total = (long long)nch * Gw;
    for (long long i = blockIdx.x * (long long)blockDim.x + threadIdx.x; i < total;
         i += (long long)gridDim.x * blockDim.x) {
        const int g = (int)(i / nch), c = (int)(i % nch);
        const int n0 = wide_group_col0(g), n1 = min(n0 + kWideCW, ncols);
        gcnt[i] = kHdr + cptr[(long long)c * ncols + n1] - cptr[(long long)c * ncols + n0];
    }
}

__global__ void k_wide_scatter(const int2* __restrict__ ent, const int* __restrict__ sptr, int G, int nch, int ncols,
                               const int* __restrict__ cptr, const unsigned short* __restrict__ winv,
                               const int* __restrict__ sptr_w, int2* __restrict__ ent_w) {
    const long long total = (long long)G * nch;
    for (long long i = blockIdx.x * (long long)blockDim.x + threadIdx.x; i < total;
         i += (long long)gridDim.x * blockDim.x) {
        const int g = (int)(i / nch), c = (int)(i % nch);
        int first;
        const int n = stream_range(sptr, i, &first);
        const int n0 = group_col0(g);
        int rank = 0, slot = -1, base = 0, jw = 0;
        for (int e = 0; e < n; ++e) {
            const int2 v = ent[first + e];
            if (is_pad(v.y)) continue;
            const int s = (v.y & 0x3ff) >> 2;
            if (s != slot) {
                slot = s;
                rank = 0;
                const int col = n0 + s;
                const int p = col / kWideWgCols * kWideWgCols + winv[col];
                const int gw = (p / kWideWgCols) * kWaves + (p % kWideWgCols) / kWideCW;
                jw = p - wide_group_col0(gw);
                base = sptr_w[(long long)gw * nch + c] + kHdr +
                       (cptr[(long long)c * ncols + p] - cptr[(long long)c * ncols + wide_group_col0(gw)]);
            }
            ent_w[base + rank++] = make_int2(v.x, (v.y & ~0x3ff) | (4 * jw));
        }
    }
}

__global__ void k_wide_headers(const int* __restrict__ sptr_w, int nch, int Gw, int2* __restrict__ ent_w,
                               long long n_entries) {
    const long long total = (long long)nch * Gw;
    for (long long i = blockIdx.x * (long long)blockDim.x + threadIdx.x; i < total;
         i += (long long)gridDim.x * blockDim.x) {
        const int s0 = sptr_w[i], s1 = sptr_w[i + 1];
        const int n = s1 - s0 - kHdr;
        ent_w[s0] = make_int2(n / kWideBatch, n % kWideBatch);
        ent_w[s0 + 1] = make_int2((s1 - s0) * (int)sizeof(int2), 0);
    }
    if (blockIdx.x == 0)
        for (int i = threadIdx.x; i < kEntGuard; i += blockDim.x)
            ent_w[n_entries + i] = i < kHdr ? make_int2(0, 0) : make_int2(0x3f800000, kTK << 10);
}

inline int grid_for(long long n, int block) {
    long long g = (n + block - 1) / block;
    if (g < 1) g = 1;
    if (g > 65535LL * 16) g = 65535LL * 16;
    return (int)g;
}

}

hipError_t wide_counts(const int2* ent, const int* sptr, int G, int nch, int ncols, int Gw, int balance, int* cnt,
                       int* cptr, int* gcnt, int* sptr_w, int* loads, unsigned short* wperm, unsigned short* winv,
                       unsigned long long* wstats, void* tmp, size_t tmp_bytes, hipStream_t st) {
    hipError_t e;
    const long long nc = (long long)nch * ncols, ng = (long long)nch * Gw;
    const int nblk = wide_blocks_for(ncols);
    if ((e = hipMemsetAsync(cnt, 0, (size_t)(nc + 1) * sizeof(int), st)) != hipSuccess) return e;
    if ((e = hipMemsetAsync(gcnt + ng, 0, sizeof(int), st)) != hipSuccess) return e;
    if ((e = hipMemsetAsync(wstats, 0, 4 * sizeof(unsigned long long), st)) != hipSuccess) return e;
    hipLaunchKernelGGL(k_wide_col_counts, dim3(grid_for((long long)G * nch, 128)), dim3(128), 0, st, ent, sptr, G, nch,
                       ncols, cnt);
    if ((e = hipGetLastError()) != hipSuccess) return e;
    hipLaunchKernelGGL(k_wide_balance, dim3(nblk), dim3(kWaves * 64), 0, st, cnt, ncols, nch, balance, loads, wperm,
                       winv);
    if ((e = hipGetLastError()) != hipSuccess) return e;
    hipLaunchKernelGGL(k_wide_stats, dim3(nblk), dim3(256), 0, st, cnt, wperm, ncols, nch, wstats);
    if ((e = hipGetLastError()) != hipSuccess) return e;
    hipLaunchKernelGGL(k_wide_permute_counts, dim3(grid_for(nc + 1, 256)), dim3(256), 0, st, cnt, wperm, ncols, nch,
                       cptr);
    if ((e = hipGetLastError()) != hipSuccess) return e;
    size_t tb = tmp_bytes;
    if ((e = hipcub::DeviceScan::ExclusiveSum(tmp, tb, cptr, cptr, (int)(nc + 1), st)) != hipSuccess) return e;
    hipLaunchKernelGGL(k_wide_group_counts, dim3(grid_for(ng, 256)), dim3(256), 0, st, cptr, ncols, nch, Gw, gcnt);
    if ((e = hipGetLastError()) != hipSuccess) return e;
    tb = tmp_bytes;
    return hipcub::DeviceScan::ExclusiveSum(tmp, tb, gcnt, sptr_w, (int)(ng + 1), st);
}

hipError_t wide_fill(const int2* ent, const int* sptr, int G, int nch, int ncols, int Gw, const int* cptr,
                     const unsigned short* winv, const int* sptr_w, int2* ent_w, long long n_entries, hipStream_t st) {
    hipLaunchKernelGGL(k_wide_scatter, dim3(grid_for((long long)G * nch, 128)), dim3(128), 0, st, ent, sptr, G, nch,
                       ncols, cptr, winv, sptr_w, ent_w);
    hipError_t e = hipGetLastError();
    if (e != hipSuccess) return e;
    hipLaunchKernelGGL(k_wide_headers, dim3(grid_for((long long)nch * Gw, 256)), dim3(256), 0, st, sptr_w, nch, Gw,
                       ent_w, n_entries);
    return hipGetLastError();
}

hipError_t launch_stream_wide(const GemmArgs& g, hipStream_t st) {
    if (g.order != 0 || g.ent == nullptr || g.wperm == nullptr) return hipErrorInvalidValue;
    const int nch = (g.K + kTK - 1) / kTK;
    const int ldxt = ldxt_for(g.M);
    dim3 grid((g.n_groups + kWaves - 1) / kWaves, (g.M + kTM - 1) / kTM, 1);
    dim3 block(kWaves * 64);
    int pfd = 0, pfl = 1;
    pf_stream_params(g.n_entries, g.n_groups, nch, &pfd, &pfl);
#define TCSC_LAUNCH_W(BF, PR)                                                                                \
    hipLaunchKernelGGL((k_stream_w<BF, PR>), grid, block, 0, st, g.XT, g.ent, g.sptr, g.B, g.Y, g.wperm, g.n_entries, \
                       ldxt, g.M, g.n_groups, g.ncols, nch, g.ldy, g.a, pfd, pfl)
    if (g.bias_first) {
        if (g.prelu) TCSC_LAUNCH_W(true, true);
        else TCSC_LAUNCH_W(true, false);
    } else {
        if (g.prelu) TCSC_LAUNCH_W(false, true);
        else TCSC_LAUNCH_W(false, false);
    }
#undef TCSC_LAUNCH_W
    return hipGetLastError();
}

}
```

sparse-matrix-multiplication-benchmark_amd/tcsc_amd/__init__.py:

```python
from __future__ import annotations

import ctypes as C
import os
import subprocess

import numpy as np

PKG_DIR = os.path.dirname(os.path.dirname(os.path.abspath(__file__)))
LIB_PATH = os.environ.get("TCSC_AMD_LIB") or os.path.join(PKG_DIR, "lib", "libtcsc_amd.so")

VARIANTS = ("basic", "optimized", "prelu_basic", "prelu_separate", "prelu_onthego")
VARIANT_ID = {v: i for i, v in enumerate(VARIANTS)}
VARIANT_ID["sparse_gemm"] = 5
PRELU_VARIANTS = frozenset(VARIANTS[2:])

EXPORTED_SYMBOLS = (
    "tcsc_from_dense", "tcsc_sgemm_basic", "tcsc_sgemm_optimized", "tcsc_sgemm_prelu_basic",
    "tcsc_sgemm_prelu_optimized_separate", "tcsc_sgemm_prelu_optimized_onthego", "tcsc_free",
    "dense_random", "init_rand_dense", "init_rand_sparse", "compare", "gemm_basic", "gemm_prelu_basic",
    "tcsc_set_seed",
    "tcsc_gpu_device_count", "tcsc_gpu_plan_create", "tcsc_gpu_plan_create_device", "tcsc_gpu_plan_get_info",
    "tcsc_gpu_plan_reserve", "tcsc_gpu_plan_destroy", "tcsc_gpu_sgemm", "tcsc_gpu_prepare_x",
    "tcsc_gpu_sgemm_prepared", "tcsc_gpu_from_dense", "tcsc_gpu_dense_sgemm", "tcsc_gpu_last_error",
    "tcsc_gpu_cache_clear", "tcsc_gpu_num_shards", "tcsc_gpu_set_num_shards", "tcsc_gpu_set_order",
    "tcsc_gpu_get_order", "tcsc_gpu_launch_info", "tcsc_gpu_launch_combine", "tcsc_gpu_build_flags",
    "tcsc_gpu_plan_workspace", "tcsc_gpu_transpose_index", "tcsc_gpu_plan_create_transposed",
    "tcsc_gpu_plan_create_transposed_device", "tcsc_gpu_sgemm_t", "tcsc_gpu_prelu_backward",
    "tcsc_gpu_sgemm_bf16", "tcsc_gpu_launch_info_bf16",
    "tcsc_gpu_plan_enable_i8", "tcsc_gpu_plan_has_i8", "tcsc_gpu_sgemm_i8", "tcsc_gpu_launch_info_i8",
    "tcsc_gpu_quantize_rows_i8", "tcsc_gpu_workspace_bound_i8",
    "tcsc_gpu_plan_enable_w2", "tcsc_gpu_plan_has_w2", "tcsc_gpu_w2_image_bytes", "tcsc_gpu_decode_pays",
    "tcsc_gpu_launch_geometry", "tcsc_gpu_wide_pays", "tcsc_gpu_plan_wide_stats",
    "tcsc_gpu_plan_create_packed", "tcsc_gpu_plan_create_packed_device", "tcsc_gpu_plan_is_packed",
    "tcsc_gpu_plan_copy_w2",
    "tcsc_gpu_plan_create_packed_image", "tcsc_gpu_plan_create_packed_image_device", "tcsc_gpu_w2_to_tcsc",
    "tcsc_gpu_w2_from_tcsc_host", "tcsc_gpu_w2_to_tcsc_host",
    "tcsc_gpu_quantize_rows_i8_bf16", "tcsc_gpu_sgemm_q8", "tcsc_gpu_launch_info_q8", "tcsc_gpu_quant_fuse_pays",
    "tcsc_gpu_sgemm_i8_out", "tcsc_gpu_sgemm_q8_out",
    "bcsr_from_dense", "bcsr_sgemm_basic", "bcsr_sgemm_prelu_basic", "bcsr_sgemm_avx", "bcsr_sgemm_prelu_avx",
    "bcsr_sgemm_avx2", "bcsr_free",
    "bcsr_gpu_plan_create", "bcsr_gpu_plan_stats", "bcsr_gpu_plan_reserve", "bcsr_gpu_plan_destroy",
    "bcsr_gpu_sgemm", "bcsr_gpu_prepare_x", "bcsr_gpu_sgemm_prepared",
    "tcsc_sparse_format", "tcsc_sparse_gemm", "tcsc_sparse_gemm_prelu", "tcsc_dense_gemm", "tcsc_dense_gemm_prelu",
)


class TcscError(RuntimeError):
    pass


class tcsc_t(C.Structure):

    _fields_ = [
        ("rows", C.c_int), ("cols", C.c_int), ("n_elem_pos", C.c_int), ("n_elem_neg", C.c_int),
        ("col_start_pos", C.POINTER(C.c_int)), ("col_start_neg", C.POINTER(C.c_int)),
        ("row_index_pos", C.POINTER(C.c_int)), ("row_index_neg", C.POINTER(C.c_int)),
    ]


class plan_info_t(C.Structure):
    _fields_ = [
        ("device", C.c_int), ("rows", C.c_int), ("cols", C.c_int), ("col_begin", C.c_int),
        ("nnz", C.c_longlong), ("n_pos", C.c_longlong), ("n_neg", C.c_longlong),
        ("chunk_k", C.c_int), ("n_chunks", C.c_int), ("device_bytes", C.c_size_t), ("order", C.c_int),
        ("mfma_min_M", C.c_int),
    ]


_f32p = np.ctypeslib.ndpointer(dtype=np.float32, flags="C_CONTIGUOUS")
_i32p = np.ctypeslib.ndpointer(dtype=np.int32, flags="C_CONTIGUOUS")
_lib = None


def build(force: bool = False) -> str:
    if force or not os.path.exists(LIB_PATH):
        subprocess.check_call(["make", "-s", "-C", PKG_DIR, "-j8"])
    return LIB_PATH


def lib():
    global _lib
    if _lib is not None:
        return _lib
    if not os.path.exists(LIB_PATH):
        raise TcscError(f"{LIB_PATH} missing: build it with `make -C {PKG_DIR}`")
    try:
        import torch
    except ImportError:
        pass
    L = C.CDLL(LIB_PATH)
    L.tcsc_gpu_build_flags.restype = C.c_int
    flags = int(L.tcsc_gpu_build_flags())
    if flags and os.environ.get("TCSC_ALLOW_DIAG") != "1":
        raise TcscError(f"{LIB_PATH} is a diagnostic build (flags {flags:#x}: ablation/no-DMA/stamps/trace, "
                        "results wrong by design); set TCSC_ALLOW_DIAG=1 to load it anyway")
    vp, i, f = C.c_void_p, C.c_int, C.c_float
    P = C.POINTER(tcsc_t)
    L.tcsc_from_dense.argtypes = [_f32p, i, i]
    L.tcsc_from_dense.restype = P
    for n in ("tcsc_sgemm_basic", "tcsc_sgemm_optimized"):
        getattr(L, n).argtypes = [_f32p, P, _f32p, _f32p, i, i, i]
        getattr(L, n).restype = None
    for n in ("tcsc_sgemm_prelu_basic", "tcsc_sgemm_prelu_optimized_separate",
              "tcsc_sgemm_prelu_optimized_onthego"):
        getattr(L, n).argtypes = [_f32p, P, _f32p, f, _f32p, i, i, i]
        getattr(L, n).restype = None
    L.tcsc_free.argtypes = [P]
    L.tcsc_free.restype = None
    L.tcsc_set_seed.argtypes = [C.c_ulonglong]
    L.tcsc_gpu_device_count.restype = i
    L.tcsc_gpu_last_error.restype = C.c_char_p
    L.tcsc_gpu_plan_create.argtypes = [P, i, i, i, vp, C.POINTER(vp)]
    L.tcsc_gpu_plan_create_device.argtypes = [i, i, vp, vp, vp, vp, i, i, i, vp, C.POINTER(vp)]
    L.tcsc_gpu_plan_get_info.argtypes = [vp, C.POINTER(plan_info_t)]
    L.tcsc_gpu_launch_info.argtypes = [vp, i, C.POINTER(i), C.POINTER(i)]
    L.tcsc_gpu_launch_combine.argtypes = [vp, i, C.POINTER(i)]
    L.tcsc_gpu_launch_geometry.argtypes = [vp, i, C.POINTER(i)]
    L.tcsc_gpu_wide_pays.argtypes = [i, i, i]
    L.tcsc_gpu_plan_wide_stats.argtypes = [vp, C.POINTER(C.c_longlong), vp, C.c_size_t]
    L.tcsc_gpu_plan_reserve.argtypes = [vp, i]
    L.tcsc_gpu_plan_workspace.argtypes = [vp, i, i, C.POINTER(C.c_size_t), C.POINTER(C.c_size_t)]
    L.tcsc_gpu_plan_destroy.argtypes = [vp]
    L.tcsc_gpu_plan_destroy.restype = None
    L.tcsc_gpu_sgemm.argtypes = [vp, vp, vp, vp, i, i, i, f, vp]
    L.tcsc_gpu_sgemm_bf16.argtypes = [vp, vp, vp, vp, i, i, i, f, vp]
    L.tcsc_gpu_launch_info_bf16.argtypes = [vp, i, C.POINTER(i), C.POINTER(i)]
    L.tcsc_gpu_plan_enable_i8.argtypes = [vp, vp]
    L.tcsc_gpu_plan_has_i8.argtypes = [vp]
    L.tcsc_gpu_sgemm_i8.argtypes = [vp, vp, vp, vp, vp, i, i, i, f, vp]
    L.tcsc_gpu_launch_info_i8.argtypes = [vp, i, C.POINTER(i), C.POINTER(i)]
    L.tcsc_gpu_quantize_rows_i8.argtypes = [vp, i, i, vp, vp, vp]
    L.tcsc_gpu_workspace_bound_i8.argtypes = [i, i, i, C.POINTER(C.c_size_t), C.POINTER(C.c_size_t)]
    L.tcsc_gpu_plan_enable_w2.argtypes = [vp, vp]
    L.tcsc_gpu_plan_has_w2.argtypes = [vp]
    L.tcsc_gpu_w2_image_bytes.argtypes = [i, i, C.POINTER(C.c_size_t)]
    L.tcsc_gpu_decode_pays.argtypes = [i, i, i, C.c_longlong]
    L.tcsc_gpu_plan_create_packed.argtypes = [P, i, i, i, vp, C.POINTER(vp)]
    L.tcsc_gpu_plan_create_packed_device.argtypes = [i, i, vp, vp, vp, vp, i, i, i, vp, C.POINTER(vp)]
    L.tcsc_gpu_plan_is_packed.argtypes = [vp]
    L.tcsc_gpu_plan_copy_w2.argtypes = [vp, vp, C.c_size_t, vp]
    L.tcsc_gpu_plan_create_packed_image.argtypes = [vp, C.c_size_t, i, i, i, i, vp, C.POINTER(vp)]
    L.tcsc_gpu_plan_create_packed_image_device.argtypes = [vp, C.c_size_t, i, i, i, i, vp, C.POINTER(vp)]
    L.tcsc_gpu_w2_to_tcsc.argtypes = [vp, C.c_size_t, i, i, vp, vp, vp, vp, C.POINTER(i), C.POINTER(i), vp]
    L.tcsc_gpu_w2_from_tcsc_host.argtypes = [P, i, i, vp, C.c_size_t]
    L.tcsc_gpu_w2_to_tcsc_host.argtypes = [vp, C.c_size_t, i, i]
    L.tcsc_gpu_w2_to_tcsc_host.restype = P
    L.tcsc_gpu_quantize_rows_i8_bf16.argtypes = [vp, i, i, vp, vp, vp]
    L.tcsc_gpu_sgemm_q8.argtypes = [vp, vp, i, vp, vp, vp, vp, i, i, i, f, vp]
    L.tcsc_gpu_launch_info_q8.argtypes = [vp, i, i, C.POINTER(i), C.POINTER(i), C.POINTER(i)]
    L.tcsc_gpu_quant_fuse_pays.argtypes = [i, i, i, i]
    L.tcsc_gpu_sgemm_i8_out.argtypes = [vp, vp, vp, vp, vp, vp, i, i, i, i, f, vp]
    L.tcsc_gpu_sgemm_q8_out.argtypes = [vp, vp, i, vp, vp, vp, vp, vp, i, i, i, i, f, vp]
    L.tcsc_gpu_prepare_x.argtypes = [vp, vp, i, vp]
    L.tcsc_gpu_sgemm_prepared.argtypes = [vp, vp, vp, i, i, i, f, vp]
    L.tcsc_gpu_from_dense.argtypes = [vp, i, i, vp, vp, vp, vp, C.POINTER(i), C.POINTER(i), vp]
    L.tcsc_gpu_dense_sgemm.argtypes = [vp, vp, vp, vp, i, i, i, i, i, f, vp]
    L.tcsc_gpu_transpose_index.argtypes = [i, i, vp, vp, vp, vp, i, i, vp, vp, vp, vp, vp]
    L.tcsc_gpu_plan_create_transposed.argtypes = [P, i, i, i, vp, C.POINTER(vp)]
    L.tcsc_gpu_plan_create_transposed_device.argtypes = [i, i, vp, vp, vp, vp, i, i, i, vp, C.POINTER(vp)]
    L.tcsc_gpu_sgemm_t.argtypes = [vp, vp, vp, i, i, vp]
    L.tcsc_gpu_prelu_backward.argtypes = [vp, i, vp, i, f, vp, i, vp, i, i, vp]
    L.tcsc_gpu_num_shards.restype = i
    L.tcsc_gpu_set_num_shards.argtypes = [i]
    L.tcsc_gpu_set_num_shards.restype = None
    L.tcsc_gpu_cache_clear.restype = None
    L.tcsc_gpu_set_order.argtypes = [i]
    L.tcsc_gpu_set_order.restype = None
    L.tcsc_gpu_get_order.restype = i
    ip = C.POINTER(i)
    L.tcsc_sparse_format.argtypes = [_i32p, i, i, _i32p, _i32p, vp, vp, ip, ip]
    L.tcsc_sparse_format.restype = i
    L.tcsc_sparse_gemm.argtypes = [_f32p, _i32p, _i32p, _i32p, _i32p, _f32p, _f32p, i, i, i]
    L.tcsc_sparse_gemm.restype = None
    L.tcsc_sparse_gemm_prelu.argtypes = L.tcsc_sparse_gemm.argtypes + [f]
    L.tcsc_sparse_gemm_prelu.restype = None
    L.tcsc_dense_gemm.argtypes = [_f32p, _f32p, _f32p, _f32p, i, i, i]
    L.tcsc_dense_gemm.restype = None
    L.tcsc_dense_gemm_prelu.argtypes = L.tcsc_dense_gemm.argtypes + [f]
    L.tcsc_dense_gemm_prelu.restype = None
    from . import bcsr as _bcsr

    _bcsr.bind(L)
    _lib = L
    return L


def last_error() -> str:
    return lib().tcsc_gpu_last_error().decode(errors="replace")


def _check(rc: int, what: str) -> None:
    if rc != 0:
        raise TcscError(f"{what} failed (status {rc}): {last_error()}")


def device_count() -> int:
    return int(lib().tcsc_gpu_device_count())


def require_gpu() -> None:
    if device_count() <= 0:
        raise TcscError("no HIP device visible: the TCSC kernels need a gfx950 (MI355X) GPU")


class TcscMatrix:

    def __init__(self, ptr):
        if not ptr:
            raise TcscError("tcsc_from_dense returned NULL")
        self.ptr = ptr

    @classmethod
    def from_dense(cls, dense: np.ndarray) -> "TcscMatrix":
        dense = np.ascontiguousarray(dense, dtype=np.float32)
        rows, cols = dense.shape
        buf = dense.reshape(-1) if dense.size else np.zeros(1, np.float32)
        return cls(lib().tcsc_from_dense(buf, rows, cols))

    @classmethod
    def from_arrays(cls, rows: int, cols: int, col_start_pos, col_start_neg, row_index_pos,
                    row_index_neg) -> "TcscMatrix":
        libc = C.CDLL(None)
        libc.malloc.restype = C.c_void_p
        libc.malloc.argtypes = [C.c_size_t]

        def put(a):
            a = np.ascontiguousarray(a, dtype=np.int32).reshape(-1)
            p = libc.malloc(max(a.nbytes, 4))
            if not p:
                raise MemoryError("malloc failed")
            if a.size:
                C.memmove(p, a.ctypes.data, a.nbytes)
            return C.cast(p, C.POINTER(C.c_int)), a.size

        t = libc.malloc(C.sizeof(tcsc_t))
        if not t:
            raise MemoryError("malloc failed")
        s = C.cast(t, C.POINTER(tcsc_t))
        s.contents.rows, s.contents.cols = int(rows), int(cols)
        s.contents.col_start_pos, _ = put(col_start_pos)
        s.contents.col_start_neg, _ = put(col_start_neg)
        s.contents.row_index_pos, s.contents.n_elem_pos = put(row_index_pos)
        s.contents.row_index_neg, s.contents.n_elem_neg = put(row_index_neg)
        return cls(s)

    def row_index(self, sign: str) -> np.ndarray:
        t = self.ptr.contents
        p, n = (t.row_index_pos, t.n_elem_pos) if sign == "pos" else (t.row_index_neg, t.n_elem_neg)
        return np.ctypeslib.as_array(p, shape=(n,)) if n > 0 else np.zeros(0, np.int32)

    @property
    def rows(self) -> int:
        return self.ptr.contents.rows

    @property
    def cols(self) -> int:
        return self.ptr.contents.cols

    @property
    def nnz(self) -> int:
        t = self.ptr.contents
        return t.n_elem_pos + t.n_elem_neg

    def arrays(self):
        t = self.ptr.contents

        def take(p, n):
            return np.ctypeslib.as_array(p, shape=(n,)).copy() if n > 0 else np.zeros(0, np.int32)

        return (take(t.col_start_pos, t.cols + 1), take(t.col_start_neg, t.cols + 1),
                take(t.row_index_pos, t.n_elem_pos), take(t.row_index_neg, t.n_elem_neg))

    def free(self) -> None:
        if self.ptr:
            lib().tcsc_free(self.ptr)
            self.ptr = None

    def __del__(self):
        try:
            self.free()
        except Exception:
            pass


def sgemm(variant: str, X: np.ndarray, W: TcscMatrix, B: np.ndarray, a: float = 0.2,
          Y: np.ndarray | None = None) -> np.ndarray:
    if variant not in VARIANTS:
        raise TcscError(f"unknown variant {variant!r} (one of {', '.join(VARIANTS)})")
    if not getattr(W, "ptr", None):
        raise TcscError("W is freed or not a TcscMatrix")
    X = np.ascontiguousarray(X, dtype=np.float32)
    if X.ndim != 2:
        raise TcscError(f"X must be 2-D (M x K), got shape {X.shape}")
    M, K = X.shape
    N = W.cols
    if K != W.rows:
        raise TcscError(f"X has K={K} columns but W has {W.rows} rows")
    B = np.ascontiguousarray(B, dtype=np.float32).reshape(-1)
    if B.size != N:
        raise TcscError(f"B has {B.size} elements, W has N={N} columns")
    if Y is None:
        Y = np.empty((M, N), np.float32)
    elif (not isinstance(Y, np.ndarray) or Y.shape != (M, N) or Y.dtype != np.float32
          or not Y.flags["C_CONTIGUOUS"]):
        raise TcscError(f"Y must be a C-contiguous float32 array of shape ({M}, {N})")
    L = lib()
    nz = lambda a_: a_.reshape(-1) if a_.size else np.zeros(1, np.float32)
    if variant in PRELU_VARIANTS:
        name = "tcsc_sgemm_prelu_basic" if variant == "prelu_basic" else "tcsc_sgemm_" + variant.replace(
            "prelu_", "prelu_optimized_")
        getattr(L, name)(nz(X), W.ptr, nz(B), a, nz(Y), M, N, K)
    else:
        getattr(L, "tcsc_sgemm_" + variant)(nz(X), W.ptr, nz(B), nz(Y), M, N, K)
    return Y



def sparse_format(matrix: np.ndarray):
    m = np.ascontiguousarray(matrix, dtype=np.int32)
    if m.ndim != 2:
        raise TcscError(f"matrix must be 2-D (K x N), got shape {m.shape}")
    K, N = m.shape
    flat = m.reshape(-1) if m.size else np.zeros(1, np.int32)
    csp, csn = np.zeros(N + 1, np.int32), np.zeros(N + 1, np.int32)
    p, q = C.c_int(0), C.c_int(0)
    L = lib()
    _check(L.tcsc_sparse_format(flat, K, N, csp, csn, None, None, C.byref(p), C.byref(q)), "tcsc_sparse_format")
    rip, rin = np.zeros(max(p.value, 1), np.int32), np.zeros(max(q.value, 1), np.int32)
    _check(L.tcsc_sparse_format(flat, K, N, csp, csn, rip.ctypes.data, rin.ctypes.data, C.byref(p), C.byref(q)),
           "tcsc_sparse_format")
    return csp, csn, rip[:p.value].copy(), rin[:q.value].copy()


def sparse_gemm(X: np.ndarray, col_start_pos, col_start_neg, row_index_pos, row_index_neg, b: np.ndarray,
                a: float | None = None, Y: np.ndarray | None = None) -> np.ndarray:
    X = np.ascontiguousarray(X, dtype=np.float32)
    if X.ndim != 2:
        raise TcscError(f"X must be 2-D (M x K), got shape {X.shape}")
    M, K = X.shape
    arrs = [np.ascontiguousarray(v, dtype=np.int32).reshape(-1)
            for v in (col_start_pos, col_start_neg, row_index_pos, row_index_neg)]
    csp, csn, rip, rin = arrs
    N = csp.size - 1
    if N < 0 or csn.size != N + 1:
        raise TcscError("col_start_pos / col_start_neg must both have N+1 entries")
    if rip.size < csp[-1] or rin.size < csn[-1]:
        raise TcscError("row_index arrays shorter than col_start[N]")
    b = np.ascontiguousarray(b, dtype=np.float32).reshape(-1)
    if b.size != N:
        raise TcscError(f"b has {b.size} elements, W has N={N} columns")
    if Y is None:
        Y = np.empty((M, N), np.float32)
    elif Y.shape != (M, N) or Y.dtype != np.float32 or not Y.flags["C_CONTIGUOUS"]:
        raise TcscError(f"Y must be a C-contiguous float32 array of shape ({M}, {N})")
    nz = lambda v, t: v if v.size else np.zeros(1, t)
    args = [nz(X.reshape(-1), np.float32), csp, csn, nz(rip, np.int32), nz(rin, np.int32), nz(b, np.float32),
            nz(Y.reshape(-1), np.float32), M, N, K]
    if a is None:
        lib().tcsc_sparse_gemm(*args)
    else:
        lib().tcsc_sparse_gemm_prelu(*args, float(a))
    return Y


def dense_gemm(X: np.ndarray, W: np.ndarray, b: np.ndarray, a: float | None = None) -> np.ndarray:
    X = np.ascontiguousarray(X, dtype=np.float32)
    W = np.ascontiguousarray(W, dtype=np.float32)
    if X.ndim != 2 or W.ndim != 2 or X.shape[1] != W.shape[0]:
        raise TcscError(f"X {X.shape} and W {W.shape} do not chain")
    M, K = X.shape
    N = W.shape[1]
    b = np.ascontiguousarray(b, dtype=np.float32).reshape(-1)
    if b.size != N:
        raise TcscError(f"b has {b.size} elements, W has N={N} columns")
    Y = np.empty((M, N), np.float32)
    nz = lambda v: v.reshape(-1) if v.size else np.zeros(1, np.float32)
    if a is None:
        lib().tcsc_dense_gemm(nz(X), nz(W), nz(b), nz(Y), M, N, K)
    else:
        lib().tcsc_dense_gemm_prelu(nz(X), nz(W), nz(b), nz(Y), M, N, K, float(a))
    return Y


ORDERS = {"fast": 0, "reference": 1}


def set_order(order: str) -> None:
    lib().tcsc_gpu_set_order(ORDERS[order])


def get_order() -> str:
    return {v: k for k, v in ORDERS.items()}[int(lib().tcsc_gpu_get_order())]


def set_num_shards(n: int) -> None:
    lib().tcsc_gpu_set_num_shards(int(n))


def num_shards() -> int:
    return int(lib().tcsc_gpu_num_shards())


def cache_clear() -> None:
    lib().tcsc_gpu_cache_clear()


def _ptr(x) -> int:
    if x is None:
        return 0
    if isinstance(x, int):
        return x
    if hasattr(x, "data_ptr"):
        return int(x.data_ptr())
    raise TypeError(f"expected a device pointer or tensor, got {type(x)}")


class Plan:

    def __init__(self, W: TcscMatrix, col_begin: int = 0, col_end: int | None = None, device: int = 0,
                 stream: int = 0):
        col_end = W.cols if col_end is None else col_end
        h = C.c_void_p()
        _check(lib().tcsc_gpu_plan_create(W.ptr, col_begin, col_end, device, C.c_void_p(stream), C.byref(h)),
               "tcsc_gpu_plan_create")
        self.handle = h

    @classmethod
    def from_device(cls, rows, cols, csp, csn, rip, rin, col_begin=0, col_end=None, device=0, stream=0):
        self = cls.__new__(cls)
        col_end = cols if col_end is None else col_end
        h = C.c_void_p()
        _check(lib().tcsc_gpu_plan_create_device(rows, cols, C.c_void_p(_ptr(csp)), C.c_void_p(_ptr(csn)),
                                                 C.c_void_p(_ptr(rip)), C.c_void_p(_ptr(rin)), col_begin,
                                                 col_end, device, C.c_void_p(stream), C.byref(h)),
               "tcsc_gpu_plan_create_device")
        self.handle = h
        return self

    @classmethod
    def transposed(cls, W: TcscMatrix, col_begin: int = 0, col_end: int | None = None, device: int = 0,
                   stream: int = 0) -> "Plan":
        if not getattr(W, "ptr", None):
            raise TcscError("W is freed or not a TcscMatrix")
        self = cls.__new__(cls)
        col_end = W.cols if col_end is None else col_end
        h = C.c_void_p()
        _check(lib().tcsc_gpu_plan_create_transposed(W.ptr, col_begin, col_end, device, C.c_void_p(stream),
                                                     C.byref(h)), "tcsc_gpu_plan_create_transposed")
        self.handle = h
        return self

    @classmethod
    def transposed_from_device(cls, rows, cols, csp, csn, rip, rin, col_begin=0, col_end=None, device=0,
                               stream=0) -> "Plan":
        self = cls.__new__(cls)
        col_end = cols if col_end is None else col_end
        h = C.c_void_p()
        _check(lib().tcsc_gpu_plan_create_transposed_device(rows, cols, C.c_void_p(_ptr(csp)), C.c_void_p(_ptr(csn)),
                                                            C.c_void_p(_ptr(rip)), C.c_void_p(_ptr(rin)), col_begin,
                                                            col_end, device, C.c_void_p(stream), C.byref(h)),
               "tcsc_gpu_plan_create_transposed_device")
        self.handle = h
        return self

    @classmethod
    def packed(cls, W: TcscMatrix, col_begin: int = 0, col_end: int | None = None, device: int = 0,
               stream: int = 0) -> "Plan":
        if not getattr(W, "ptr", None):
            raise TcscError("W is freed or not a TcscMatrix")
        self = cls.__new__(cls)
        col_end = W.cols if col_end is None else col_end
        h = C.c_void_p()
        _check(lib().tcsc_gpu_plan_create_packed(W.ptr, col_begin, col_end, device, C.c_void_p(stream), C.byref(h)),
               "tcsc_gpu_plan_create_packed")
        self.handle = h
        return self

    @classmethod
    def packed_from_device(cls, rows, cols, csp, csn, rip, rin, col_begin=0, col_end=None, device=0,
                           stream=0) -> "Plan":
        self = cls.__new__(cls)
        col_end = cols if col_end is None else col_end
        h = C.c_void_p()
        _check(lib().tcsc_gpu_plan_create_packed_device(rows, cols, C.c_void_p(_ptr(csp)), C.c_void_p(_ptr(csn)),
                                                        C.c_void_p(_ptr(rip)), C.c_void_p(_ptr(rin)), col_begin,
                                                        col_end, device, C.c_void_p(stream), C.byref(h)),
               "tcsc_gpu_plan_create_packed_device")
        self.handle = h
        return self

    @classmethod
    def packed_from_image(cls, image, rows: int, cols: int, col_begin: int = 0, device: int = 0,
                          stream: int = 0) -> "Plan":
        self = cls.__new__(cls)
        h = C.c_void_p()
        if isinstance(image, np.ndarray):
            if image.dtype != np.uint8:
                raise TcscError(f"Plan.packed_from_image: a host image must be uint8, got {image.dtype}")
            host = np.ascontiguousarray(image).reshape(-1)
            ptr, nbytes, name = host.ctypes.data, host.size, "tcsc_gpu_plan_create_packed_image"
        else:
            if hasattr(image, "is_contiguous") and not image.is_contiguous():
                raise TcscError("Plan.packed_from_image: the device image must be contiguous")
            nbytes = image.numel() * image.element_size() if hasattr(image, "numel") else w2_image_bytes(rows, cols)
            ptr, name = _ptr(image), "tcsc_gpu_plan_create_packed_image_device"
        _check(getattr(lib(), name)(C.c_void_p(ptr), int(nbytes), int(rows), int(cols), int(col_begin), int(device),
                                    C.c_void_p(stream), C.byref(h)), name)
        self.handle = h
        return self

    @property
    def is_packed(self) -> bool:
        return bool(lib().tcsc_gpu_plan_is_packed(self.handle))

    def w2_image(self, stream: int = 0):
        import torch

        inf = self.info()
        img = torch.empty(w2_image_bytes(inf["rows"], inf["cols"]), dtype=torch.uint8,
                          device=torch.device("cuda", inf["device"]))
        self.copy_w2(img, stream=stream)
        return img

    def copy_w2(self, dst, nbytes: int | None = None, stream: int = 0) -> None:
        if nbytes is None:
            nbytes = dst.numel() * dst.element_size() if hasattr(dst, "numel") else 0
        _check(lib().tcsc_gpu_plan_copy_w2(self.handle, C.c_void_p(_ptr(dst)), int(nbytes), C.c_void_p(stream)),
               "tcsc_gpu_plan_copy_w2")

    def info(self) -> dict:
        inf = plan_info_t()
        _check(lib().tcsc_gpu_plan_get_info(self.handle, C.byref(inf)), "tcsc_gpu_plan_get_info")
        return {k: getattr(inf, k) for k, _ in plan_info_t._fields_}

    def _launch_info(self, name: str, M: int) -> tuple[str, int]:
        path, slices = C.c_int(), C.c_int()
        _check(getattr(lib(), name)(self.handle, int(M), C.byref(path), C.byref(slices)), name)
        return ("gather", "fused", "mfma", "small", "decode")[path.value], slices.value

    def launch_info(self, M: int) -> tuple[str, int]:
        return self._launch_info("tcsc_gpu_launch_info", M)

    def launch_info_bf16(self, M: int) -> tuple[str, int]:
        return self._launch_info("tcsc_gpu_launch_info_bf16", M)

    def launch_combine(self, M: int) -> bool:
        return self.combine_mode(M) is not None

    def combine_mode(self, M: int):
        v = C.c_int()
        _check(lib().tcsc_gpu_launch_combine(self.handle, int(M), C.byref(v)), "tcsc_gpu_launch_combine")
        return {2: "bands", 3: "pairwise", 4: "pairwise-split"}.get(v.value)

    def launch_geometry(self, M: int) -> int:
        v = C.c_int()
        _check(lib().tcsc_gpu_launch_geometry(self.handle, int(M), C.byref(v)), "tcsc_gpu_launch_geometry")
        return v.value

    def wide_stats(self) -> dict:
        st = (C.c_longlong * 4)()
        nblk = (self.info()["cols"] + 351) // 352
        m = np.empty((nblk, 16, 22), np.uint16)
        _check(lib().tcsc_gpu_plan_wide_stats(self.handle, st, C.c_void_p(m.ctypes.data), m.size),
               "tcsc_gpu_plan_wide_stats")
        return dict(max_identity=st[0], max_balanced=st[1], long_identity=st[2], long_balanced=st[3], map=m)

    def reserve(self, max_M: int) -> None:
        _check(lib().tcsc_gpu_plan_reserve(self.handle, int(max_M)), "tcsc_gpu_plan_reserve")

    PATH_ID = {None: -1, "gather": 0, "mfma": 2, "small": 3, "decode": 4}

    def workspace(self, M: int, path: str | None = None) -> tuple[int, int]:
        need, reserved = C.c_size_t(), C.c_size_t()
        _check(lib().tcsc_gpu_plan_workspace(self.handle, int(M), self.PATH_ID[path], C.byref(need),
                                             C.byref(reserved)), "tcsc_gpu_plan_workspace")
        return need.value, reserved.value

    def sgemm(self, X, B, Y, M: int, ldy: int, variant: str = "prelu_basic", a: float = 0.2,
              stream: int = 0) -> None:
        _check(lib().tcsc_gpu_sgemm(self.handle, C.c_void_p(_ptr(X)), C.c_void_p(_ptr(B)), C.c_void_p(_ptr(Y)),
                                    int(M), int(ldy), VARIANT_ID[variant], float(a), C.c_void_p(stream)),
               "tcsc_gpu_sgemm")

    def sgemm_bf16(self, X, B, Y, M: int, ldy: int, variant: str = "prelu_basic", a: float = 0.2,
                   stream: int = 0) -> None:
        _check(lib().tcsc_gpu_sgemm_bf16(self.handle, C.c_void_p(_ptr(X)), C.c_void_p(_ptr(B)), C.c_void_p(_ptr(Y)),
                                         int(M), int(ldy), VARIANT_ID[variant], float(a), C.c_void_p(stream)),
               "tcsc_gpu_sgemm_bf16")

    def enable_i8(self, stream: int = 0) -> bool:
        _check(lib().tcsc_gpu_plan_enable_i8(self.handle, C.c_void_p(stream)), "tcsc_gpu_plan_enable_i8")
        return self.has_i8

    @property
    def has_i8(self) -> bool:
        return bool(lib().tcsc_gpu_plan_has_i8(self.handle))

    def launch_info_i8(self, M: int) -> tuple[str, int]:
        return self._launch_info("tcsc_gpu_launch_info_i8", M)

    def enable_w2(self, stream: int = 0) -> bool:
        _check(lib().tcsc_gpu_plan_enable_w2(self.handle, C.c_void_p(stream)), "tcsc_gpu_plan_enable_w2")
        return self.has_w2

    @property
    def has_w2(self) -> bool:
        return bool(lib().tcsc_gpu_plan_has_w2(self.handle))

    def sgemm_i8(self, Xq, scale, B, Y, M: int, ldy: int, variant: str = "prelu_basic", a: float = 0.2,
                 stream: int = 0, col_scale=None, ytype=None) -> None:
        yt = _ytype_of(Y) if ytype is None else _ytype(ytype)
        _check(lib().tcsc_gpu_sgemm_i8_out(self.handle, C.c_void_p(_ptr(Xq)), C.c_void_p(_ptr(scale)),
                                           C.c_void_p(_ptr(col_scale)), C.c_void_p(_ptr(B)), C.c_void_p(_ptr(Y)), yt,
                                           int(M), int(ldy), VARIANT_ID[variant], float(a), C.c_void_p(stream)),
               "tcsc_gpu_sgemm_i8_out")

    def sgemm_q8(self, X, Xq, scale, B, Y, M: int, ldy: int, variant: str = "prelu_basic", a: float = 0.2,
                 stream: int = 0, xtype=None, col_scale=None, ytype=None) -> None:
        xt = _xtype_of(X) if xtype is None else _xtype(xtype)
        yt = _ytype_of(Y) if ytype is None else _ytype(ytype)
        _check(lib().tcsc_gpu_sgemm_q8_out(self.handle, C.c_void_p(_ptr(X)), xt, C.c_void_p(_ptr(Xq)),
                                           C.c_void_p(_ptr(scale)), C.c_void_p(_ptr(col_scale)), C.c_void_p(_ptr(B)),
                                           C.c_void_p(_ptr(Y)), yt, int(M), int(ldy), VARIANT_ID[variant], float(a),
                                           C.c_void_p(stream)), "tcsc_gpu_sgemm_q8_out")

    def launch_info_q8(self, M: int, dtype="f32") -> tuple[str, int, bool]:
        path, slices, fused = C.c_int(), C.c_int(), C.c_int()
        _check(lib().tcsc_gpu_launch_info_q8(self.handle, int(M), _xtype(dtype), C.byref(path), C.byref(slices),
                                             C.byref(fused)), "tcsc_gpu_launch_info_q8")
        return ("gather", "fused", "mfma", "small", "decode")[path.value], slices.value, bool(fused.value)

    def sgemm_t(self, G, DX, M: int, ldx: int, stream: int = 0) -> None:
        _check(lib().tcsc_gpu_sgemm_t(self.handle, C.c_void_p(_ptr(G)), C.c_void_p(_ptr(DX)), int(M), int(ldx),
                                      C.c_void_p(stream)), "tcsc_gpu_sgemm_t")

    def prepare_x(self, X, M: int, stream: int = 0) -> None:
        _check(lib().tcsc_gpu_prepare_x(self.handle, C.c_void_p(_ptr(X)), int(M), C.c_void_p(stream)),
               "tcsc_gpu_prepare_x")

    def sgemm_prepared(self, B, Y, M: int, ldy: int, variant: str = "prelu_basic", a: float = 0.2,
                       stream: int = 0) -> None:
        _check(lib().tcsc_gpu_sgemm_prepared(self.handle, C.c_void_p(_ptr(B)), C.c_void_p(_ptr(Y)), int(M), int(ldy),
                                             VARIANT_ID[variant], float(a), C.c_void_p(stream)),
               "tcsc_gpu_sgemm_prepared")

    def destroy(self) -> None:
        if getattr(self, "handle", None):
            lib().tcsc_gpu_plan_destroy(self.handle)
            self.handle = None

    def __del__(self):
        try:
            self.destroy()
        except Exception:
            pass


def dense_sgemm(X, Wd, B, Y, M: int, N: int, K: int, ldy: int, variant: str = "prelu_basic", a: float = 0.2,
                stream: int = 0) -> None:
    _check(lib().tcsc_gpu_dense_sgemm(C.c_void_p(_ptr(X)), C.c_void_p(_ptr(Wd)), C.c_void_p(_ptr(B)),
                                      C.c_void_p(_ptr(Y)), int(M), int(N), int(K), int(ldy), VARIANT_ID[variant],
                                      float(a), C.c_void_p(stream)), "tcsc_gpu_dense_sgemm")


def gpu_from_dense(d_dense, rows: int, cols: int, d_csp, d_csn, d_rip=None, d_rin=None, stream: int = 0):
    p, q = C.c_int(), C.c_int()
    _check(lib().tcsc_gpu_from_dense(C.c_void_p(_ptr(d_dense)), rows, cols, C.c_void_p(_ptr(d_csp)),
                                     C.c_void_p(_ptr(d_csn)), C.c_void_p(_ptr(d_rip)), C.c_void_p(_ptr(d_rin)),
                                     C.byref(p), C.byref(q), C.c_void_p(stream)), "tcsc_gpu_from_dense")
    return p.value, q.value


def gpu_transpose_index(rows: int, cols: int, d_csp, d_csn, d_rip, d_rin, col_begin: int, col_end: int, d_t_csp,
                        d_t_csn, d_t_rip, d_t_rin, stream: int = 0) -> None:
    _check(lib().tcsc_gpu_transpose_index(int(rows), int(cols), C.c_void_p(_ptr(d_csp)), C.c_void_p(_ptr(d_csn)),
                                          C.c_void_p(_ptr(d_rip)), C.c_void_p(_ptr(d_rin)), int(col_begin),
                                          int(col_end), C.c_void_p(_ptr(d_t_csp)), C.c_void_p(_ptr(d_t_csn)),
                                          C.c_void_p(_ptr(d_t_rip)), C.c_void_p(_ptr(d_t_rin)), C.c_void_p(stream)),
           "tcsc_gpu_transpose_index")


XTYPE_ID = {"f32": 0, "bf16": 1}


def _xtype(spec) -> int:
    if isinstance(spec, int):
        return spec
    if isinstance(spec, str) and spec in XTYPE_ID:
        return XTYPE_ID[spec]
    name = str(spec)
    if name in ("torch.float32", "torch.bfloat16"):
        return int(name == "torch.bfloat16")
    raise TcscError(f"activations must be fp32 or bf16 ('f32', 'bf16' or the torch dtype), got {spec!r}")


def _xtype_of(X) -> int:
    dt = getattr(X, "dtype", None)
    return 0 if dt is None else _xtype(dt)


YTYPE_ID = {"f32": 0, "bf16": 1}


def _ytype(spec) -> int:
    if isinstance(spec, int):
        return spec
    if isinstance(spec, str) and spec in YTYPE_ID:
        return YTYPE_ID[spec]
    name = str(spec)
    if name in ("torch.float32", "torch.bfloat16"):
        return int(name == "torch.bfloat16")
    raise TcscError(f"Y must be fp32 or bf16 ('f32', 'bf16' or the torch dtype), got {spec!r}")


def _ytype_of(Y) -> int:
    dt = getattr(Y, "dtype", None)
    return 0 if dt is None else _ytype(dt)


def ternarize_absmean(Wf):
    W = np.ascontiguousarray(Wf, dtype=np.float32)
    beta = np.float32(np.mean(np.abs(W), dtype=np.float32)) if W.size else np.float32(0.0)
    if not beta > 0:
        return np.zeros(W.shape, dtype=np.int8), np.float32(0.0)
    return np.clip(np.rint(W / beta), -1, 1).astype(np.int8), beta


def quantize_rows_i8(X, Xq, scale, M: int, K: int, stream: int = 0) -> None:
    name = "tcsc_gpu_quantize_rows_i8_bf16" if _xtype_of(X) else "tcsc_gpu_quantize_rows_i8"
    _check(getattr(lib(), name)(C.c_void_p(_ptr(X)), int(M), int(K), C.c_void_p(_ptr(Xq)),
                                C.c_void_p(_ptr(scale)), C.c_void_p(stream)), name)


def quant_fuse_pays(M: int, K: int, N: int, dtype="f32") -> bool:
    return bool(lib().tcsc_gpu_quant_fuse_pays(int(M), int(K), int(N), _xtype(dtype)))


def w2_image_bytes(K: int, N: int) -> int:
    b = C.c_size_t()
    _check(lib().tcsc_gpu_w2_image_bytes(int(K), int(N), C.byref(b)), "tcsc_gpu_w2_image_bytes")
    return b.value


def decode_pays(M: int, K: int, N: int, nnz: int) -> bool:
    return bool(lib().tcsc_gpu_decode_pays(int(M), int(K), int(N), int(nnz)))


def w2_to_tcsc(image, rows: int, cols: int, stream: int = 0):
    import torch

    if not torch.is_tensor(image) or not image.is_cuda or not image.is_contiguous():
        raise TcscError("w2_to_tcsc: image must be a contiguous CUDA tensor")
    nbytes = image.numel() * image.element_size()
    rows, cols = int(rows), int(cols)
    L, p, q = lib(), C.c_int(), C.c_int()
    with torch.cuda.device(image.device):
        csp = torch.empty(max(cols, 0) + 1, dtype=torch.int32, device=image.device)
        csn = torch.empty_like(csp)

        def call(rip, rin):
            _check(L.tcsc_gpu_w2_to_tcsc(C.c_void_p(_ptr(image)), nbytes, rows, cols, C.c_void_p(_ptr(csp)),
                                         C.c_void_p(_ptr(csn)), C.c_void_p(_ptr(rip)), C.c_void_p(_ptr(rin)),
                                         C.byref(p), C.byref(q), C.c_void_p(stream)), "tcsc_gpu_w2_to_tcsc")

        call(None, None)
        rip = torch.empty(max(p.value, 1), dtype=torch.int32, device=image.device)
        rin = torch.empty(max(q.value, 1), dtype=torch.int32, device=image.device)
        call(rip, rin)
    return csp, csn, rip[:p.value], rin[:q.value]


def w2_pack_host(W: TcscMatrix, col_begin: int = 0, col_end: int | None = None) -> np.ndarray:
    if not getattr(W, "ptr", None):
        raise TcscError("W is freed or not a TcscMatrix")
    col_end = W.cols if col_end is None else col_end
    nbytes = _w2_bytes(W.rows, col_end - col_begin)
    if nbytes is None:
        raise TcscError(f"w2_pack_host: no image for K={W.rows} and columns [{col_begin}, {col_end})")
    image = np.empty(nbytes, np.uint8)
    _check(lib().tcsc_gpu_w2_from_tcsc_host(W.ptr, int(col_begin), int(col_end), C.c_void_p(image.ctypes.data),
                                            nbytes), "tcsc_gpu_w2_from_tcsc_host")
    return image


def w2_unpack_host(image: np.ndarray, rows: int, cols: int) -> TcscMatrix:
    if not isinstance(image, np.ndarray) or image.dtype != np.uint8:
        raise TcscError("w2_unpack_host: image must be a numpy uint8 array")
    host = np.ascontiguousarray(image).reshape(-1)
    ptr = lib().tcsc_gpu_w2_to_tcsc_host(C.c_void_p(host.ctypes.data), host.size, int(rows), int(cols))
    if not ptr:
        raise TcscError(f"tcsc_gpu_w2_to_tcsc_host failed: {last_error()}")
    return TcscMatrix(ptr)


PACKED_FORMAT_VERSION = 1


def _w2_bytes(rows: int, cols: int):
    if not (1 <= rows < 1 << 22) or cols < 1:
        return None
    return ((cols + 15) // 16) * ((rows + 255) // 256) * 1024


def save_packed(plan: Plan, path) -> None:
    inf = plan.info()
    img = plan.w2_image()
    np.savez(path, image=img.cpu().numpy(), rows=np.int64(inf["rows"]), cols=np.int64(inf["cols"]),
             col_begin=np.int64(inf["col_begin"]), version=np.int64(PACKED_FORMAT_VERSION))


def load_packed(path, device: int = 0, stream: int = 0) -> Plan:
    with np.load(path, allow_pickle=False) as z:
        missing = [k for k in ("image", "rows", "cols", "col_begin", "version") if k not in z.files]
        if missing:
            raise TcscError(f"load_packed: {path}: missing {', '.join(missing)}")
        version, image = z["version"], z["image"]
        if version.shape != () or version.dtype.kind not in "iu" or int(version) != PACKED_FORMAT_VERSION:
            raise TcscError(f"load_packed: {path}: format version {version!r}, this library reads "
                            f"{PACKED_FORMAT_VERSION}")
        dims = [z[k] for k in ("rows", "cols", "col_begin")]
    if any(d.shape != () or d.dtype.kind not in "iu" for d in dims):
        raise TcscError(f"load_packed: {path}: rows, cols and col_begin must be integer scalars")
    rows, cols, col_begin = (int(d) for d in dims)
    if image.dtype != np.uint8:
        raise TcscError(f"load_packed: {path}: image has dtype {image.dtype}, expected uint8")
    want = _w2_bytes(rows, cols)
    if want is None or col_begin < 0 or image.size != want:
        raise TcscError(f"load_packed: {path}: image has {image.size} bytes, rows={rows} cols={cols} "
                        f"col_begin={col_begin} need {want}")
    return Plan.packed_from_image(image, rows, cols, col_begin, device, stream)


def prelu_backward(G, Y, a: float, DZ, DB, M: int, N: int, ldg: int | None = None, ldy: int | None = None,
                   lddz: int | None = None, stream: int = 0) -> None:
    N = int(N)
    _check(lib().tcsc_gpu_prelu_backward(C.c_void_p(_ptr(G)), N if ldg is None else int(ldg), C.c_void_p(_ptr(Y)),
                                         N if ldy is None else int(ldy), float(a), C.c_void_p(_ptr(DZ)),
                                         N if lddz is None else int(lddz), C.c_void_p(_ptr(DB)), int(M), N,
                                         C.c_void_p(stream)), "tcsc_gpu_prelu_backward")
```

Measured before the change: 19310 G-add-ops/s.

## Use a continuous LDS ring in the wide kernel and defer tail-row entries to the next chunk

The wide gather kernel's fixed per-buffer LDS layout becomes a continuous ring of TCSC_WIDE_RING_ROWS rows, with DMA offsets wrapping modulo the ring. Because the ring holds extra rows, entries that touch the last rows of a chunk can be moved into the next chunk's stream. New plan-time kernels (level, defer_cols, apply_defer) pick which columns to defer so the per-wave maximum stream length across the 16 waves is evened out, which should shorten the critical wave per chunk. In exchange, plan building gets more complex and uses extra buffers. LDS use changes, and a debug stats API is added.

```diff
diff --git a/include/tcsc_gpu.h b/include/tcsc_gpu.h
--- a/include/tcsc_gpu.h
+++ b/include/tcsc_gpu.h
@@ -79,6 +79,8 @@
 int tcsc_gpu_wide_pays(int M, int ncols, int num_cus);
 int tcsc_gpu_plan_wide_stats(const tcsc_gpu_plan *plan, long long stats[4], unsigned short *map,
                              size_t map_entries);
+int tcsc_gpu_plan_wide_defer_stats(const tcsc_gpu_plan *plan, long long stats[4], int *periods,
+                                   size_t period_entries);
 
 int tcsc_gpu_plan_reserve(tcsc_gpu_plan *plan, int max_M);
 void tcsc_gpu_plan_destroy(tcsc_gpu_plan *plan);
diff --git a/sparse-matrix-multiplication-benchmark_amd/csrc/tcsc_api.cpp b/sparse-matrix-multiplication-benchmark_amd/csrc/tcsc_api.cpp
--- a/sparse-matrix-multiplication-benchmark_amd/csrc/tcsc_api.cpp
+++ b/sparse-matrix-multiplication-benchmark_amd/csrc/tcsc_api.cpp
@@ -645,8 +645,10 @@
     if (nch <= 0 || ng + 1 > 0x7fffffffLL) return TCSC_OK;
     const char* bal_s = std::getenv("TCSC_WIDE_BALANCE");
     const int balance = bal_s && std::atoi(bal_s) == 0 ? 0 : 1;
+    const char* def_s = std::getenv("TCSC_WIDE_DEFER");
+    const int defer = def_s && std::atoi(def_s) == 0 ? 0 : 1;
     const size_t nmap = (size_t)tcsc::wide_blocks_for(ncols) * tcsc::kWideWgCols;
-    DevBuf cnt, cptr, gcnt, tmp, loads, winv, wstats;
+    DevBuf cnt, cptr, gcnt, tmp, loads, winv, wstats, tail, lev, defc;
     size_t tb1 = 0, tb2 = 0;
     HIP_TRY(tcsc::plan_scan_tmp_bytes(nc + 1, &tb1));
     HIP_TRY(tcsc::plan_scan_tmp_bytes(ng + 1, &tb2));
@@ -658,6 +660,9 @@
         loads.alloc(nmap / tcsc::kWideCW * nch * sizeof(int)) != hipSuccess ||
         winv.alloc((size_t)ncols * sizeof(unsigned short)) != hipSuccess ||
         wstats.alloc(4 * sizeof(unsigned long long)) != hipSuccess ||
+        tail.alloc((size_t)nc * sizeof(unsigned short)) != hipSuccess ||
+        lev.alloc(3 * (nmap / tcsc::kWideCW) * nch * sizeof(int)) != hipSuccess ||
+        defc.alloc((size_t)nc * sizeof(int)) != hipSuccess ||
         hipMalloc(&sptr_w, (size_t)(ng + 1) * sizeof(int)) != hipSuccess) {
         (void)hipGetLastError();
         return TCSC_OK;
@@ -669,8 +674,9 @@
     }
     std::unique_ptr<unsigned short, void (*)(unsigned short*)> wperm_guard(wperm, [](unsigned short* q) { (void)hipFree(q); });
     HIP_TRY(hipDeviceSynchronize());
-    HIP_TRY(tcsc::wide_counts(p->ent, p->sptr, G, nch, ncols, Gw, balance, cnt.as<int>(), cptr.as<int>(), gcnt.as<int>(),
-                              sptr_w, loads.as<int>(), wperm, winv.as<unsigned short>(), wstats.as<unsigned long long>(),
+    HIP_TRY(tcsc::wide_counts(p->ent, p->sptr, G, nch, ncols, Gw, balance, defer, cnt.as<int>(), cptr.as<int>(),
+                              gcnt.as<int>(), sptr_w, loads.as<int>(), wperm, winv.as<unsigned short>(),
+                              wstats.as<unsigned long long>(), tail.as<unsigned short>(), lev.as<int>(), defc.as<int>(),
                               tmp.p, tb, st));
     int total = 0;
     unsigned long long stats[4] = {0, 0, 0, 0};
@@ -682,8 +688,8 @@
         (void)hipGetLastError();
         return TCSC_OK;
     }
-    hipError_t e = tcsc::wide_fill(p->ent, p->sptr, G, nch, ncols, Gw, cptr.as<int>(), winv.as<unsigned short>(), sptr_w,
-                                   ent_w, total, st);
+    hipError_t e = tcsc::wide_fill(p->ent, p->sptr, G, nch, ncols, Gw, cnt.as<int>(), defc.as<int>(), cptr.as<int>(),
+                                   winv.as<unsigned short>(), sptr_w, ent_w, total, st);
     if (e == hipSuccess) e = hipStreamSynchronize(st);
     if (e != hipSuccess) {
         (void)hipFree(ent_w);
@@ -1556,6 +1562,49 @@
         }
         DeviceGuard dg(p->device);
         HIP_TRY(hipMemcpy(map, p->wperm, nmap * sizeof(unsigned short), hipMemcpyDeviceToHost));
+    }
+    return TCSC_OK;
+}
+
+int tcsc_gpu_plan_wide_defer_stats(const tcsc_gpu_plan* p, long long stats[4], int* periods, size_t period_entries) {
+    if (!p || (!stats && !periods)) {
+        set_error("tcsc_gpu_plan_wide_defer_stats: bad arguments");
+        return TCSC_E_ARG;
+    }
+    if (!p->ent_w || !p->sptr_w) {
+        set_error("tcsc_gpu_plan_wide_defer_stats: the plan has no wide streams (tcsc_gpu_plan_reserve builds them)");
+        return TCSC_E_ARG;
+    }
+    const int nch = p->n_chunks, Gw = p->n_groups_w, nblk = tcsc::wide_blocks_for(p->cols);
+    const size_t np = (size_t)nblk * nch * tcsc::kWaves;
+    if (periods && period_entries != np) {
+        set_error("tcsc_gpu_plan_wide_defer_stats: the periods have %zu entries, not %zu", np, period_entries);
+        return TCSC_E_ARG;
+    }
+    std::vector<int> sp((size_t)Gw * nch + 1);
+    {
+        DeviceGuard dg(p->device);
+        HIP_TRY(hipMemcpy(sp.data(), p->sptr_w, sp.size() * sizeof(int), hipMemcpyDeviceToHost));
+    }
+    long long sum_max = 0, n_long = 0;
+    for (int b = 0; b < nblk; ++b)
+        for (int c = 0; c < nch; ++c) {
+            int mx = 0;
+            for (int w = 0; w < tcsc::kWaves; ++w) {
+                const int g = b * tcsc::kWaves + w;
+                const size_t i = (size_t)g * nch + c;
+                const int n = g < Gw ? sp[i + 1] - sp[i] - tcsc::kHdr : 0;
+                if (periods) periods[((size_t)b * nch + c) * tcsc::kWaves + w] = n;
+                mx = std::max(mx, n);
+                n_long += n > tcsc::kWideCap ? 1 : 0;
+            }
+            sum_max += mx;
+        }
+    if (stats) {
+        stats[0] = tcsc::kWideRingRows;
+        stats[1] = tcsc::kWideDeferRows;
+        stats[2] = sum_max;
+        stats[3] = n_long;
     }
     return TCSC_OK;
 }
diff --git a/sparse-matrix-multiplication-benchmark_amd/csrc/tcsc_internal.h b/sparse-matrix-multiplication-benchmark_amd/csrc/tcsc_internal.h
--- a/sparse-matrix-multiplication-benchmark_amd/csrc/tcsc_internal.h
+++ b/sparse-matrix-multiplication-benchmark_amd/csrc/tcsc_internal.h
@@ -93,7 +93,17 @@
 
 constexpr int kWideCW = 22;
 constexpr int kWideBatch = 3;
+constexpr int kWideCap = 30;
 constexpr int kWideWgCols = kWaves * kWideCW;
+#ifndef TCSC_WIDE_RING_ROWS
+#define TCSC_WIDE_RING_ROWS 152
+#endif
+constexpr int kWideRingRows = TCSC_WIDE_RING_ROWS;
+constexpr int kWideDeferRows = kWideRingRows - 3 * kTK;
+constexpr int kWideRingBytes = (kWideRingRows + 1) * kRowBytes;
+static_assert(kWideRingRows % 2 == 0 && kTK % 2 == 0, "a DMA row pair never straddles the ring's wrap");
+static_assert(kWideDeferRows >= 0 && kWideDeferRows <= 16 && kWideDeferRows < kTK, "the tail rows fit a 16-bit mask");
+static_assert(kWideRingBytes + kPfScratch <= 160 * 1024, "LDS");
 __host__ __device__ constexpr int wide_group_col0(int g) { return (g / kWaves) * kWideWgCols + (g % kWaves) * kWideCW; }
 __host__ __device__ constexpr int wide_groups_for(int ncols) {
     return (ncols / kWideWgCols) * kWaves + (ncols % kWideWgCols + kWideCW - 1) / kWideCW;
@@ -190,11 +200,13 @@
 size_t workspace_bytes(int M, int ncols, int slices);
 size_t xt_bytes(int M, int K);
 hipError_t launch_gemm(const GemmArgs& g, hipStream_t st);
-hipError_t wide_counts(const int2* ent, const int* sptr, int G, int nch, int ncols, int Gw, int balance, int* cnt,
-                       int* cptr, int* gcnt, int* sptr_w, int* loads, unsigned short* wperm, unsigned short* winv,
-                       unsigned long long* wstats, void* tmp, size_t tmp_bytes, hipStream_t st);
-hipError_t wide_fill(const int2* ent, const int* sptr, int G, int nch, int ncols, int Gw, const int* cptr,
-                     const unsigned short* winv, const int* sptr_w, int2* ent_w, long long n_entries, hipStream_t st);
+hipError_t wide_counts(const int2* ent, const int* sptr, int G, int nch, int ncols, int Gw, int balance, int defer,
+                       int* cnt, int* cptr, int* gcnt, int* sptr_w, int* loads, unsigned short* wperm,
+                       unsigned short* winv, unsigned long long* wstats, unsigned short* tail, int* lev, int* def,
+                       void* tmp, size_t tmp_bytes, hipStream_t st);
+hipError_t wide_fill(const int2* ent, const int* sptr, int G, int nch, int ncols, int Gw, const int* cnt,
+                     const int* def, const int* cptr, const unsigned short* winv, const int* sptr_w, int2* ent_w,
+                     long long n_entries, hipStream_t st);
 hipError_t launch_stream_wide(const GemmArgs& g, hipStream_t st);
 int dense_tile_rows(int rows);
 hipError_t dense_to_tcsc_counts(const float* D, int rows, int cols, int* cp, int* cn, int* totp, int* totn,
diff --git a/sparse-matrix-multiplication-benchmark_amd/csrc/tcsc_wide.hip b/sparse-matrix-multiplication-benchmark_amd/csrc/tcsc_wide.hip
--- a/sparse-matrix-multiplication-benchmark_amd/csrc/tcsc_wide.hip
+++ b/sparse-matrix-multiplication-benchmark_amd/csrc/tcsc_wide.hip
@@ -8,14 +8,15 @@
 
 #include "gather_asm_w22.inc"
 
-static_assert(TCSCW_GEN_CW == kWideCW && TCSCW_GEN_BATCH == kWideBatch, "generated loop geometry");
+static_assert(TCSCW_GEN_CW == kWideCW && TCSCW_GEN_BATCH == kWideBatch && TCSCW_GEN_CAP == kWideCap,
+              "generated loop geometry");
 static_assert(TCSCW_GEN_CAP + kHdr <= kEntGuard, "stream prefetch stays inside the entry guard");
 static_assert(TCSCW_GEN_HDR == 2 * kHdr, "generated loop and plan agree on the chunk header");
 static_assert(TCSCW_GEN_BUDGET == (512 / kWavesPerSimd) / 8 * 8, "generated loop VGPR budget");
 static_assert(TCSCW_GEN_TAIL == 1, "the wide streams are unpadded");
 static_assert(TCSCW_GEN_TOUCH == 0 && TCSCW_GEN_PF == 0, "no scalar-cache touches in the wide loop");
 static_assert(4 * kWideCW <= 255, "slot index must fit the 8-bit gpr_idx field");
-static_assert(kWaves == 16 && kTK % 16 == 0 && kNBuf >= 3, "the wide kernel's DMA split and ring");
+static_assert(kWaves == 16 && kTK % 16 == 0 && kNBuf == 3, "the wide kernel's DMA split and ring");
 
 namespace {
 
@@ -71,29 +72,36 @@
 
 struct DmaW {
     const char* next;
-    unsigned lds_wave;
+    unsigned ring;
     unsigned chunk_bytes;
     unsigned row_bytes;
 };
 static_assert(kDmaPerWave % 2 == 0, "whole pairs of DMA rows");
-
-__device__ __forceinline__ void dma_next_chunk_w(DmaW& d, int buf, unsigned lane16) {
-    const unsigned m0base = d.lds_wave + (unsigned)(buf * (kBufRows * kRowBytes));
+constexpr unsigned kRingWrapW = (unsigned)kWideRingRows * kRowBytes;
+
+__device__ __forceinline__ void dma_next_chunk_w(DmaW& d, unsigned lds_base, unsigned lane16) {
     const char* row = d.next;
 #pragma unroll
     for (int i0 = 0; i0 < kDmaPerWave; i0 += 2) {
         const char* s0 = row;
         const char* s1 = row + (d.row_bytes - 1 * kRowBytes);
+        unsigned off = d.ring + (unsigned)(i0 * kRowBytes);
+        off = off >= kRingWrapW ? off - kRingWrapW : off;
         unsigned sv;
         asm volatile("s_mov_b32 %[sv], m0\n\ts_mov_b32 m0, %1\n\ts_nop 0\n\tglobal_load_lds_dwordx4 %2, %3\n\t"
                      "global_load_lds_dwordx4 %2, %4 offset:1024\n\ts_mov_b32 m0, %[sv]"
                      : [sv] "=&s"(sv)
-                     : "s"(m0base + i0 * kRowBytes), "v"(lane16), "s"(s0), "s"(s1)
+                     : "s"(lds_base + off), "v"(lane16), "s"(s0), "s"(s1)
                      : "memory");
         row += 2u * d.row_bytes;
     }
     d.next += d.chunk_bytes;
-}
+    d.ring += (unsigned)(kTK * kRowBytes);
+    d.ring = d.ring >= kRingWrapW ? d.ring - kRingWrapW : d.ring;
+}
+constexpr int ring_gcd(int a, int b) { return b == 0 ? a : ring_gcd(b, a % b); }
+constexpr int kRingTurnW = kWideRingRows / ring_gcd(kTK, kWideRingRows);
+static_assert((kTK * kRingTurnW) % kWideRingRows == 0, "the ring's period in chunks (k_wide_scatter)");
 static_assert(kRowBytes == 1024, "the DMA's instruction offsets are whole 1-KiB rows");
 
 __device__ __forceinline__ void pf_touch_w(unsigned m0, unsigned voff, const char* base) {
@@ -116,8 +124,8 @@
 
 constexpr int kEpiRowsW = 64;
 constexpr int kStrideW = kWideWgCols * 4 + 16;
-constexpr int kLdsBytesW = kRingBytes + kPfScratch;
-static_assert(kEpiRowsW * kStrideW <= kRingBytes, "the epilogue staging fits below the ring's end");
+constexpr int kLdsBytesW = kWideRingBytes + kPfScratch;
+static_assert(kEpiRowsW * kStrideW <= kWideRingRows * kRowBytes, "the epilogue staging fits below the ring's end");
 static_assert(kLdsBytesW <= 160 * 1024, "LDS");
 static_assert(kWideCW <= 64 && kWideWgCols <= 65535, "one lane per slot reads its 16-bit column position");
 static_assert(kWideWgCols % 4 == 0 && kWideWgCols / 4 > 64 && kWideWgCols / 4 <= 128,
@@ -167,24 +175,23 @@
         }
     }
 
-    if (threadIdx.x < 64 * kNBuf) {
-        const int b = threadIdx.x >> 6;
-        reinterpret_cast<float4*>(lds + (b * kBufRows + kTK) * kRowBytes)[lane] = make_float4(-0.f, -0.f, -0.f, -0.f);
-    }
+    if (threadIdx.x < 64)
+        reinterpret_cast<float4*>(lds + kWideRingRows * kRowBytes)[lane] = make_float4(-0.f, -0.f, -0.f, -0.f);
 
     if (nch > 0) {
         DmaW dma;
         dma.row_bytes = (unsigned)ldxt * 4u;
         dma.chunk_bytes = (unsigned)kTK * (unsigned)ldxt * 4u;
         dma.next = reinterpret_cast<const char*>(XT + m0) + (size_t)(wave * kDmaPerWave) * dma.row_bytes;
-        dma.lds_wave = (unsigned)reinterpret_cast<uintptr_t>(lds) + (unsigned)(wave * kDmaPerWave * kRowBytes);
+        dma.ring = (unsigned)(wave * kDmaPerWave * kRowBytes);
+        const unsigned lds_base = (unsigned)reinterpret_cast<uintptr_t>(lds);
         const bool dma_wave = wave < kDmaWaves;
-        const unsigned pf_m0 = (unsigned)reinterpret_cast<uintptr_t>(lds) + kRingBytes + 256u * wave;
+        const unsigned pf_m0 = lds_base + kWideRingBytes + 256u * wave;
         const unsigned pf_s_off = (unsigned)pf_dist + 128u * (unsigned)(lane * pf_lines >> 6);
         auto pf_issue = [&](unsigned long long p) {
             if (kPfS) pf_touch_w(pf_m0, pf_s_off, reinterpret_cast<const char*>(p));
         };
-        if (dma_wave) dma_next_chunk_w(dma, 0, lane16);
+        if (dma_wave) dma_next_chunk_w(dma, lds_base, lane16);
         unsigned long long cur =
             reinterpret_cast<unsigned long long>(ent + (active ? (long long)sptr[(long long)g * nch] : n_entries));
         i32x16 sb[TCSCW_SBUF_VECS];
@@ -193,20 +200,18 @@
         pf_issue(cur);
 #pragma unroll
         for (int i = 1; i + 1 < kNBuf; ++i) {
-            if (dma_wave) dma_next_chunk_w(dma, i % kNBuf, lane16);
+            if (dma_wave) dma_next_chunk_w(dma, lds_base, lane16);
             pf_issue(cur);
         }
         asm volatile("s_waitcnt lgkmcnt(0)" ::: "memory");
         const unsigned mask = 0x3ffu;
-        int dbuf = kNBuf - 1;
         for (int c = 0; c < nch; ++c) {
             asm volatile("s_waitcnt vmcnt(%0)" ::"n"((kNBuf - 2) * kDmaPerWave + (kPfS ? 2 : 0)) : "memory");
             __builtin_amdgcn_s_barrier();
-            if (dma_wave) dma_next_chunk_w(dma, dbuf, lane16);
+            if (dma_wave) dma_next_chunk_w(dma, lds_base, lane16);
             gather_stream_w(sb, sbt, cur, lane16, mask, acc);
             load_stream_w(sb, sbt, reinterpret_cast<const char*>(cur));
             pf_issue(cur);
-            dbuf = dbuf == kNBuf - 1 ? 0 : dbuf + 1;
         }
         asm volatile("s_waitcnt vmcnt(0) lgkmcnt(0)" ::: "memory");
     }
@@ -303,7 +308,7 @@
 __device__ __forceinline__ bool is_pad(int word) { return ((word >> 10) % kBufRows) == kTK; }
 
 __global__ void k_wide_col_counts(const int2* __restrict__ ent, const int* __restrict__ sptr, int G, int nch, int ncols,
-                                  int* __restrict__ cnt) {
+                                  int* __restrict__ cnt, unsigned short* __restrict__ tail) {
     const long long total = (long long)G * nch;
     for (long long i = blockIdx.x * (long long)blockDim.x + threadIdx.x; i < total;
          i += (long long)gridDim.x * blockDim.x) {
@@ -312,18 +317,24 @@
         const int n = stream_range(sptr, i, &first);
         const int n0 = group_col0(g);
         int run = 0, slot = -1;
+        unsigned bits = 0;
         for (int e = 0; e < n; ++e) {
             const int w = ent[first + e].y;
             if (is_pad(w)) continue;
             const int s = (w & 0x3ff) >> 2;
             if (s != slot) {
                 if (run) cnt[(long long)c * ncols + n0 + slot] = run;
+                if (bits) tail[(long long)c * ncols + n0 + slot] = (unsigned short)bits;
                 slot = s;
                 run = 0;
+                bits = 0;
             }
             ++run;
+            const int r = (w >> 10) % kBufRows - (kTK - kWideDeferRows);
+            if (r >= 0) bits |= 1u << r;
         }
         if (run) cnt[(long long)c * ncols + n0 + slot] = run;
+        if (bits) tail[(long long)c * ncols + n0 + slot] = (unsigned short)bits;
     }
 }
 
@@ -470,6 +481,111 @@
     }
 }
 
+constexpr int kLevelTaus = 5;
+
+__device__ __forceinline__ int max16(int v) {
+#pragma unroll
+    for (int o = 8; o > 0; o >>= 1) v = max(v, __shfl_xor(v, o));
+    return v;
+}
+
+__device__ __forceinline__ unsigned long long level_walk(const int* L, const int* D, int nch,
+                                                         int w, int tau, int* out) {
+    unsigned long long sum = 0;
+    int carry = 0;
+    for (int c = 0; c < nch; ++c) {
+        const int have = carry + L[(size_t)w * nch + c];
+        const int T = max(tau, max16(have - D[(size_t)w * nch + c]));
+        const int P = min(have, T);
+        carry = have - P;
+        if (out) out[(size_t)w * nch + c] = carry;
+        sum += (unsigned long long)max16(P);
+    }
+    return sum;
+}
+
+__global__ void __launch_bounds__(128)
+k_wide_level(const int* __restrict__ cnt, const unsigned short* __restrict__ tail,
+             const unsigned short* __restrict__ wperm, int ncols, int nch, int defer, int* lev) {
+    __shared__ unsigned long long sums[8], base_s, tot_s[2];
+    __shared__ int tau_s;
+    const int tid = threadIdx.x, lane = tid & 63;
+    const int c0 = blockIdx.x * kWideWgCols;
+    const unsigned short* perm = wperm + (size_t)blockIdx.x * kWideWgCols;
+    const size_t plane = (size_t)gridDim.x * kWaves * nch;
+    int* L = lev + (size_t)blockIdx.x * kWaves * nch;
+    int* D = L + plane;
+    int* carry = D + plane;
+    unsigned long long tot = 0;
+    for (int i = tid; i < kWaves * nch; i += blockDim.x) {
+        const int w = i / nch, c = i % nch;
+        int l = 0, d = 0;
+        for (int j = 0; j < kWideCW; ++j) {
+            const int col = c0 + perm[w * kWideCW + j];
+            if (col < ncols) {
+                l += cnt[(size_t)c * ncols + col];
+                d += __popc((unsigned)tail[(size_t)c * ncols + col]);
+            }
+        }
+        L[i] = l;
+        D[i] = c + 1 < nch ? d : 0;
+        carry[i] = 0;
+        tot += (unsigned long long)l;
+    }
+    if (!defer) return;
+    tot = wave_sum(tot);
+    if (lane == 0) tot_s[tid >> 6] = tot;
+    __syncthreads();
+    const unsigned long long den = (unsigned long long)kWaves * nch;
+    const int tau0 = (int)((tot_s[0] + tot_s[1] + den - 1) / den);
+    const int w = tid & 15, ti = tid >> 4;
+    const unsigned long long sum = level_walk(L, D, nch, w, tau0 + ti, nullptr);
+    if (w == 0) sums[ti] = sum;
+    if (ti == 0) {
+        unsigned long long b = 0;
+        for (int c = 0; c < nch; ++c) b += (unsigned long long)max16(L[(size_t)w * nch + c]);
+        if (w == 0) base_s = b;
+    }
+    __syncthreads();
+    if (tid == 0) {
+        int best = 0;
+        for (int t = 1; t < kLevelTaus; ++t)
+            if (sums[t] < sums[best]) best = t;
+        tau_s = sums[best] < base_s ? tau0 + best : -1;
+    }
+    __syncthreads();
+    if (tau_s >= 0 && tid < 64) (void)level_walk(L, D, nch, w, tau_s, tid < 16 ? carry : nullptr);
+}
+static_assert(kLevelTaus <= 8, "k_wide_level walks one candidate per 16 lanes of its 128");
+
+__global__ void k_wide_defer_cols(const unsigned short* __restrict__ tail, const unsigned short* __restrict__ wperm,
+                                  const int* __restrict__ lev, int ncols, int nch, int nblk, int* __restrict__ def) {
+    const long long total = (long long)nblk * kWaves * nch;
+    const int* carry = lev + 2 * total;
+    for (long long i = blockIdx.x * (long long)blockDim.x + threadIdx.x; i < total;
+         i += (long long)gridDim.x * blockDim.x) {
+        int left = carry[i];
+        if (left <= 0) continue;
+        const int gw = (int)(i / nch), c = (int)(i % nch);
+        const int p0 = wide_group_col0(gw), c0 = gw / kWaves * kWideWgCols;
+        for (int r = kWideDeferRows - 1; r >= 0 && left > 0; --r)
+            for (int j = 0; j < kWideCW && left > 0; ++j) {
+                const int col = c0 + wperm[p0 + j];
+                if (col < ncols && ((tail[(size_t)c * ncols + col] >> r) & 1)) {
+                    ++def[(size_t)c * ncols + p0 + j];
+                    --left;
+                }
+            }
+    }
+}
+
+__global__ void k_wide_apply_defer(const int* __restrict__ def, int ncols, int nch, int* __restrict__ cntp) {
+    const long long total = (long long)nch * ncols;
+    for (long long i = blockIdx.x * (long long)blockDim.x + threadIdx.x; i < total;
+         i += (long long)gridDim.x * blockDim.x)
+        cntp[i] += (i >= ncols ? def[i - ncols] : 0) - def[i];
+}
+
 __global__ void k_wide_group_counts(const int* __restrict__ cptr, int ncols, int nch, int Gw, int* __restrict__ gcnt) {
     const long long total = (long long)nch * Gw;
     for (long long i = blockIdx.x * (long long)blockDim.x + threadIdx.x; i < total;
@@ -481,6 +597,7 @@
 }
 
 __global__ void k_wide_scatter(const int2* __restrict__ ent, const int* __restrict__ sptr, int G, int nch, int ncols,
+                               const int* __restrict__ cnt, const int* __restrict__ def,
                                const int* __restrict__ cptr, const unsigned short* __restrict__ winv,
                                const int* __restrict__ sptr_w, int2* __restrict__ ent_w) {
     const long long total = (long long)G * nch;
@@ -490,7 +607,8 @@
         int first;
         const int n = stream_range(sptr, i, &first);
         const int n0 = group_col0(g);
-        int rank = 0, slot = -1, base = 0, jw = 0;
+        int rank = 0, slot = -1, base = 0, jw = 0, stay = 0, base_n = 0;
+        const int ring0 = (c % kRingTurnW) * kTK;
         for (int e = 0; e < n; ++e) {
             const int2 v = ent[first + e];
             if (is_pad(v.y)) continue;
@@ -502,10 +620,20 @@
                 const int p = col / kWideWgCols * kWideWgCols + winv[col];
                 const int gw = (p / kWideWgCols) * kWaves + (p % kWideWgCols) / kWideCW;
                 jw = p - wide_group_col0(gw);
+                const int p0 = wide_group_col0(gw);
+                const int d = def[(long long)c * ncols + p];
                 base = sptr_w[(long long)gw * nch + c] + kHdr +
-                       (cptr[(long long)c * ncols + p] - cptr[(long long)c * ncols + wide_group_col0(gw)]);
+                       (cptr[(long long)c * ncols + p] - cptr[(long long)c * ncols + p0]) +
+                       (c > 0 ? def[(long long)(c - 1) * ncols + p] : 0);
+                stay = cnt[(long long)c * ncols + col] - d;
+                base_n = d ? sptr_w[(long long)gw * nch + c + 1] + kHdr +
+                                 (cptr[(long long)(c + 1) * ncols + p] - cptr[(long long)(c + 1) * ncols + p0])
+                           : 0;
             }
-            ent_w[base + rank++] = make_int2(v.x, (v.y & ~0x3ff) | (4 * jw));
+            const int ring = (ring0 + (v.y >> 10) % kBufRows) % kWideRingRows;
+            const int at = rank < stay ? base + rank : base_n + (rank - stay);
+            ++rank;
+            ent_w[at] = make_int2(v.x, (ring << 10) | (4 * jw));
         }
     }
 }
@@ -522,7 +650,7 @@
     }
     if (blockIdx.x == 0)
         for (int i = threadIdx.x; i < kEntGuard; i += blockDim.x)
-            ent_w[n_entries + i] = i < kHdr ? make_int2(0, 0) : make_int2(0x3f800000, kTK << 10);
+            ent_w[n_entries + i] = i < kHdr ? make_int2(0, 0) : make_int2(0x3f800000, kWideRingRows << 10);
 }
 
 inline int grid_for(long long n, int block) {
@@ -534,17 +662,20 @@
 
 }
 
-hipError_t wide_counts(const int2* ent, const int* sptr, int G, int nch, int ncols, int Gw, int balance, int* cnt,
-                       int* cptr, int* gcnt, int* sptr_w, int* loads, unsigned short* wperm, unsigned short* winv,
-                       unsigned long long* wstats, void* tmp, size_t tmp_bytes, hipStream_t st) {
+hipError_t wide_counts(const int2* ent, const int* sptr, int G, int nch, int ncols, int Gw, int balance, int defer,
+                       int* cnt, int* cptr, int* gcnt, int* sptr_w, int* loads, unsigned short* wperm,
+                       unsigned short* winv, unsigned long long* wstats, unsigned short* tail, int* lev, int* def,
+                       void* tmp, size_t tmp_bytes, hipStream_t st) {
     hipError_t e;
     const long long nc = (long long)nch * ncols, ng = (long long)nch * Gw;
     const int nblk = wide_blocks_for(ncols);
     if ((e = hipMemsetAsync(cnt, 0, (size_t)(nc + 1) * sizeof(int), st)) != hipSuccess) return e;
     if ((e = hipMemsetAsync(gcnt + ng, 0, sizeof(int), st)) != hipSuccess) return e;
+    if ((e = hipMemsetAsync(tail, 0, (size_t)nc * sizeof(unsigned short), st)) != hipSuccess) return e;
+    if ((e = hipMemsetAsync(def, 0, (size_t)nc * sizeof(int), st)) != hipSuccess) return e;
     if ((e = hipMemsetAsync(wstats, 0, 4 * sizeof(unsigned long long), st)) != hipSuccess) return e;
     hipLaunchKernelGGL(k_wide_col_counts, dim3(grid_for((long long)G * nch, 128)), dim3(128), 0, st, ent, sptr, G, nch,
-                       ncols, cnt);
+                       ncols, cnt, tail);
     if ((e = hipGetLastError()) != hipSuccess) return e;
     hipLaunchKernelGGL(k_wide_balance, dim3(nblk), dim3(kWaves * 64), 0, st, cnt, ncols, nch, balance, loads, wperm,
                        winv);
@@ -554,6 +685,15 @@
     hipLaunchKernelGGL(k_wide_permute_counts, dim3(grid_for(nc + 1, 256)), dim3(256), 0, st, cnt, wperm, ncols, nch,
                        cptr);
     if ((e = hipGetLastError()) != hipSuccess) return e;
+    hipLaunchKernelGGL(k_wide_level, dim3(nblk), dim3(128), 0, st, cnt, tail, wperm, ncols, nch, defer, lev);
+    if ((e = hipGetLastError()) != hipSuccess) return e;
+    if (defer) {
+        hipLaunchKernelGGL(k_wide_defer_cols, dim3(grid_for((long long)nblk * kWaves * nch, 128)), dim3(128), 0, st, tail,
+                           wperm, lev, ncols, nch, nblk, def);
+        if ((e = hipGetLastError()) != hipSuccess) return e;
+        hipLaunchKernelGGL(k_wide_apply_defer, dim3(grid_for(nc, 256)), dim3(256), 0, st, def, ncols, nch, cptr);
+        if ((e = hipGetLastError()) != hipSuccess) return e;
+    }
     size_t tb = tmp_bytes;
     if ((e = hipcub::DeviceScan::ExclusiveSum(tmp, tb, cptr, cptr, (int)(nc + 1), st)) != hipSuccess) return e;
     hipLaunchKernelGGL(k_wide_group_counts, dim3(grid_for(ng, 256)), dim3(256), 0, st, cptr, ncols, nch, Gw, gcnt);
@@ -562,10 +702,11 @@
     return hipcub::DeviceScan::ExclusiveSum(tmp, tb, gcnt, sptr_w, (int)(ng + 1), st);
 }
 
-hipError_t wide_fill(const int2* ent, const int* sptr, int G, int nch, int ncols, int Gw, const int* cptr,
-                     const unsigned short* winv, const int* sptr_w, int2* ent_w, long long n_entries, hipStream_t st) {
+hipError_t wide_fill(const int2* ent, const int* sptr, int G, int nch, int ncols, int Gw, const int* cnt,
+                     const int* def, const int* cptr, const unsigned short* winv, const int* sptr_w, int2* ent_w,
+                     long long n_entries, hipStream_t st) {
     hipLaunchKernelGGL(k_wide_scatter, dim3(grid_for((long long)G * nch, 128)), dim3(128), 0, st, ent, sptr, G, nch,
-                       ncols, cptr, winv, sptr_w, ent_w);
+                       ncols, cnt, def, cptr, winv, sptr_w, ent_w);
     hipError_t e = hipGetLastError();
     if (e != hipSuccess) return e;
     hipLaunchKernelGGL(k_wide_headers, dim3(grid_for((long long)nch * Gw, 256)), dim3(256), 0, st, sptr_w, nch, Gw,
diff --git a/sparse-matrix-multiplication-benchmark_amd/tcsc_amd/__init__.py b/sparse-matrix-multiplication-benchmark_amd/tcsc_amd/__init__.py
--- a/sparse-matrix-multiplication-benchmark_amd/tcsc_amd/__init__.py
+++ b/sparse-matrix-multiplication-benchmark_amd/tcsc_amd/__init__.py
@@ -30,7 +30,7 @@
     "tcsc_gpu_plan_enable_i8", "tcsc_gpu_plan_has_i8", "tcsc_gpu_sgemm_i8", "tcsc_gpu_launch_info_i8",
     "tcsc_gpu_quantize_rows_i8", "tcsc_gpu_workspace_bound_i8",
     "tcsc_gpu_plan_enable_w2", "tcsc_gpu_plan_has_w2", "tcsc_gpu_w2_image_bytes", "tcsc_gpu_decode_pays",
-    "tcsc_gpu_launch_geometry", "tcsc_gpu_wide_pays", "tcsc_gpu_plan_wide_stats",
+    "tcsc_gpu_launch_geometry", "tcsc_gpu_wide_pays", "tcsc_gpu_plan_wide_stats", "tcsc_gpu_plan_wide_defer_stats",
     "tcsc_gpu_plan_create_packed", "tcsc_gpu_plan_create_packed_device", "tcsc_gpu_plan_is_packed",
     "tcsc_gpu_plan_copy_w2",
     "tcsc_gpu_plan_create_packed_image", "tcsc_gpu_plan_create_packed_image_device", "tcsc_gpu_w2_to_tcsc",
@@ -118,6 +118,7 @@
     L.tcsc_gpu_launch_geometry.argtypes = [vp, i, C.POINTER(i)]
     L.tcsc_gpu_wide_pays.argtypes = [i, i, i]
     L.tcsc_gpu_plan_wide_stats.argtypes = [vp, C.POINTER(C.c_longlong), vp, C.c_size_t]
+    L.tcsc_gpu_plan_wide_defer_stats.argtypes = [vp, C.POINTER(C.c_longlong), vp, C.c_size_t]
     L.tcsc_gpu_plan_reserve.argtypes = [vp, i]
     L.tcsc_gpu_plan_workspace.argtypes = [vp, i, i, C.POINTER(C.c_size_t), C.POINTER(C.c_size_t)]
     L.tcsc_gpu_plan_destroy.argtypes = [vp]
@@ -565,6 +566,14 @@
                "tcsc_gpu_plan_wide_stats")
         return dict(max_identity=st[0], max_balanced=st[1], long_identity=st[2], long_balanced=st[3], map=m)
 
+    def wide_defer_stats(self) -> dict:
+        st = (C.c_longlong * 4)()
+        inf = self.info()
+        P = np.empty(((inf["cols"] + 351) // 352, inf["n_chunks"], 16), np.int32)
+        _check(lib().tcsc_gpu_plan_wide_defer_stats(self.handle, st, C.c_void_p(P.ctypes.data), P.size),
+               "tcsc_gpu_plan_wide_defer_stats")
+        return dict(ring_rows=st[0], defer_rows=st[1], max_deferred=st[2], long_deferred=st[3], periods=P)
+
     def reserve(self, max_M: int) -> None:
         _check(lib().tcsc_gpu_plan_reserve(self.handle, int(max_M)), "tcsc_gpu_plan_reserve")
 
```

Measured after the change: 19460 G-add-ops/s, median of 6. Within noise of the previous version (+0.7%).
